# GRAPH-0/JODO

Hardware: AMD Instinct MI355X
Metric: molecules/sec (1000-step ancestral) (higher is better)
Workload: dtype f32

## Files before the change

### include/jodo_hip.h

```cpp
#ifndef JODO_HIP_H
#define JODO_HIP_H
#include <stddef.h>
#include <stdint.h>
#ifdef __cplusplus
extern "C" {
#endif

#define JODO_OK 0
#define JODO_ERR_ARG (-1)
#define JODO_ERR_LAUNCH (-2)
#define JODO_ERR_UNSUPPORTED (-3)

typedef struct {
    int32_t nf;
    int32_t n_layers;
    int32_t n_heads;
    int32_t n_extra;
    int32_t mlp_ratio;
    int32_t in_node_dim;
    int32_t edge_ch;
    int32_t cond_ch;
    float spatial_cut_off;
    float edge_quan_th;
    int32_t layout;
} jodo_cfg;

enum jodo_wslot_global {
    JW_TIME_FREQ = 0, JW_TIME_W1, JW_TIME_B1, JW_TIME_W3, JW_TIME_B3,
    JW_COND_W0, JW_COND_B0, JW_COND_W2, JW_COND_B2, JW_COND_LIN_W, JW_COND_LIN_B,
    JW_MOD_W, JW_MOD_B,
    JW_NODE_EMB_W, JW_NODE_EMB_B, JW_EDGE_EMB_W, JW_EDGE_EMB_B, JW_GBF_TOP,
    JW_NH1_W, JW_NH1_B, JW_NH2_W, JW_NH2_B, JW_NH3_W, JW_NH3_B,
    JW_EH1_W, JW_EH1_B, JW_EH2_W, JW_EH2_B, JW_EH3_W, JW_EH3_B,
    JW_GLOBAL_COUNT
};
enum jodo_wslot_block {
    JB_WQ = 0, JB_BQ, JB_WK, JB_BK, JB_WV, JB_BV,
    JB_EE_W, JB_EE_B, JB_LE0_W, JB_LE1_W, JB_N2E_W, JB_N2E_B,
    JB_FF1_W, JB_FF1_B, JB_FF2_W, JB_FF2_B, JB_FF3_W, JB_FF3_B, JB_FF4_W, JB_FF4_B,
    JB_INE_W, JB_ROW_W, JB_COL_W, JB_IN_B, JB_C0_W, JB_C0_B, JB_C2_W, JB_CSCALE,
    JB_NRO_W, JB_NRO_B, JB_ERO_W, JB_ERO_B, JB_GBF,
    JB_ROWQ_W, JB_COLQ_W, JB_INQ_B, JB_LQ_W, JB_INEC_W, JB_QT_W,
    JB_BLOCK_COUNT
};

typedef struct {
    const char* name;
    const float* data;
    const int64_t* shape;
    int32_t ndim;
} jodo_tensor;
int jodo_dgt_packed_size(const jodo_cfg* cfg, const jodo_tensor* tensors, int n_tensors, size_t* n_floats, int* n_woff);
int jodo_dgt_pack_weights_host(const jodo_cfg* cfg, const jodo_tensor* tensors, int n_tensors, float* packed_host,
                               size_t cap_floats, int64_t* woff_out, int n_woff);
int jodo_dgt_pack_weights(const jodo_cfg* cfg, const jodo_tensor* tensors, int n_tensors, void* packed_dev,
                          size_t cap_floats, int64_t* woff_out, int n_woff, void* stream);

typedef struct jodo_plan jodo_plan;

int jodo_plan_create(const jodo_cfg* cfg, int B, int N, const int32_t* n_nodes_host, int max_chunk,
                     jodo_plan** out);
void jodo_plan_destroy(jodo_plan* plan);
size_t jodo_plan_desc_bytes(const jodo_plan* plan);
size_t jodo_plan_workspace_bytes(const jodo_plan* plan);
int64_t jodo_plan_mod_len(const jodo_plan* plan);
int jodo_plan_upload(jodo_plan* plan, void* desc_dev, void* stream);
int jodo_plan_stats(const jodo_plan* plan, int64_t* out6);

int jodo_dgt_forward(jodo_plan* plan, const void* desc_dev, const float* packed_w, const int64_t* woff,
                     int n_woff, const float* xh, const float* edge_x, const float* cond_x,
                     const float* cond_edge_x, const float* noise_level, const float* context,
                     float* out_xh, float* out_edge, int32_t* flags_dev, void* workspace, void* stream);

int jodo_plan_work(const jodo_plan* plan, int uniform_t, int symmetric, double* mfma_flops_per_class);

enum jodo_plan_option {
    JODO_OPT_FUSE_NEXT_QKV = 0,
    JODO_OPT_DIR_SPLIT = 1,
    JODO_OPT_NODE_POST_WAVES = 2,
    JODO_OPT_ATTN_VARIANT = 3,
    JODO_OPT_PIN_SYMMETRIC = 4,
    JODO_OPT_PIN_UNIFORM_T = 5,
    JODO_OPT_ROT_STATS = 6,
    JODO_OPT_NODE_MIX = 7,
    JODO_OPT_HEADS_MIX = 8,
    JODO_OPT_HALF_ROWS = 9,
    JODO_OPT_PRE_EMBED = 10,
    JODO_OPT_AB_PRE = 11,
    JODO_OPT_Z_SPLIT = 12,
    JODO_OPT_SPLIT_BF16 = 13,
    JODO_OPT_COUNT
};
int jodo_plan_set_option(jodo_plan* plan, int option, int value);

int jodo_debug_attn_schedule(const jodo_plan* plan, int64_t* out8);

int jodo_debug_fetch(jodo_plan* plan, const void* workspace, int what, float* dst_dev, int64_t* count,
                     void* stream);
int jodo_debug_set_max_blocks(jodo_plan* plan, int max_blocks);
int jodo_debug_set_force_directed(jodo_plan* plan, int on);
int jodo_debug_set_timing_buffer(jodo_plan* plan, void* dev16xu64);

enum jodo_prof_class {
    JODO_PROF_PROLOGUE = 0, JODO_PROF_NODE_PRE, JODO_PROF_EDGE_ATTN, JODO_PROF_RESERVED3, JODO_PROF_RESERVED4,
    JODO_PROF_NODE_POST, JODO_PROF_EDGE_UPDATE, JODO_PROF_EPILOGUE, JODO_PROF_COUNT
};
int jodo_profile_enable(jodo_plan* plan, int enable);
int jodo_profile_read(jodo_plan* plan, float* ms_sum, int32_t* launches);

int jodo_sampler_step(int B, int N, int node_feats, int edge_ch, const int32_t* n_nodes_dev, float c_x, float c_pred,
                      float sigma, const float* x, const float* edge_x, const float* pred, const float* edge_pred,
                      const float* eps_pos, const float* eps_feat, const float* eps_edge, float* x_next,
                      float* edge_next, float* x_mean, float* edge_mean, void* stream);
int jodo_sampler_step_tab(int B, int N, int node_feats, int edge_ch, const int32_t* n_nodes_dev, const float* coef_tab_dev,
                          const int32_t* step_dev, const float* x, const float* edge_x, const float* pred,
                          const float* edge_pred, const float* eps_pos, const float* eps_feat, const float* eps_edge,
                          float* x_next, float* edge_next, float* x_mean, float* edge_mean, void* stream);
int jodo_sampler_step_rng(int B, int N, int node_feats, int edge_ch, const int32_t* n_nodes_dev, float c_x, float c_pred,
                          float sigma, const float* coef_tab_dev, const int32_t* step_dev, uint64_t seed, uint32_t draw,
                          const float* x, const float* edge_x, const float* pred, const float* edge_pred, float* x_next,
                          float* edge_next, float* x_mean, float* edge_mean, void* stream);
int jodo_step_begin(int B, const float* coef_tab_dev, const int32_t* step_dev, float* noise_level_out, void* stream);
int jodo_step_end(int32_t* step_dev, void* stream);
int jodo_dpm_update(int B, int N, int node_feats, int edge_ch, const int32_t* n_nodes_dev, const float* coef8_host,
                    const float* coef_tab_dev, const int32_t* step_dev, int tab_stride, int tab_col, const float* x_pos,
                    const float* x_base, const float* edge_base, const float* P, const float* eP, const float* DA, const float* eDA,
                    const float* DB, const float* eDB, const float* PP, const float* eps_pos, float* x_out, float* edge_out,
                    void* stream);
int jodo_dpm_update_rng(int B, int N, int node_feats, int edge_ch, const int32_t* n_nodes_dev, const float* coef8_host,
                        const float* coef_tab_dev, const int32_t* step_dev, int tab_stride, int tab_col, uint64_t seed,
                        uint32_t draw, uint32_t draw_mul, const float* x_pos, const float* x_base, const float* edge_base,
                        const float* P, const float* eP, const float* DA, const float* eDA, const float* DB, const float* eDB,
                        const float* PP, float* x_out, float* edge_out, void* stream);
int jodo_step_begin_at(int B, const float* coef_tab_dev, const int32_t* step_dev, int tab_stride, int tab_col,
                       float* noise_level_out, void* stream);
int jodo_decode(int B, int N, int atom_types, int include_fc, int edge_ch, int compress_edge, int centered,
                float pos_norm, float atom_norm, float fc_norm, float edge_norm, const int32_t* n_nodes_dev,
                const float* xh, const float* edge_x, float* pos_out, uint8_t* atom_type_out, int8_t* fc_out,
                uint8_t* edge_type_out, void* stream);

typedef struct jodo_train jodo_train;
int jodo_train_create(const jodo_cfg* cfg, int B, int N, const int32_t* n_nodes_host, const jodo_tensor* params, int n_params,
                      jodo_train** out);
void jodo_train_destroy(jodo_train* t);
size_t jodo_train_desc_bytes(const jodo_train* t);
size_t jodo_train_workspace_bytes(const jodo_train* t);
int jodo_train_set_option(jodo_train* t, int option, int value);
int jodo_train_debug_locate(const jodo_train* t, int what, int layer, size_t* byte_offset, size_t* count);
int jodo_train_upload(jodo_train* t, void* desc_dev, void* stream);
const void* jodo_train_desc_host(const jodo_train* t);
int jodo_train_forward(jodo_train* t, const void* desc_dev, const float* const* params_dev, int n_params, const float* xh,
                       const float* edge_x, const float* cond_x, const float* cond_edge_x, const float* noise_level,
                       const float* context, float dropout_p, uint64_t seed, float* out_xh, float* out_edge, int32_t* flags_out,
                       void* workspace, void* stream);
int jodo_train_backward(jodo_train* t, const void* desc_dev, const float* const* params_dev, float* const* grads_dev, int n_params,
                        const float* noise_level, const float* d_out_xh, const float* d_out_edge, float dropout_p, uint64_t seed,
                        void* workspace, void* stream);
int jodo_train_gemm(int tA, int tB, int M, int N, int K, const float* A, int lda, const float* B, int ldb, float* C, int ldc,
                    const float* bias, int acc, float* ws, size_t ws_floats, void* stream);
int jodo_train_gemm_ex(int tA, int tB, int M, int N, int K, const float* A, int lda, const float* B, int ldb, float* C, int ldc,
                       const float* bias, int act, float* out2, float* dbias, float* ws, size_t ws_floats, void* stream);

int jodo_adam_step(int64_t n, float* p, const float* g, float* m, float* v, float* vmax, double lr, double beta1, double beta2, double eps,
                   double weight_decay, int64_t step, int decoupled, int amsgrad, void* stream);
int jodo_gradnorm_clip(const float* norm_dev, double* state_dev, double max_grad, float* coef_dev, float* allowed_dev, void* stream);
int jodo_kabsch_rotations(int B, const float* A_dev, float* R_dev, void* stream);

typedef struct {
    int32_t nf, n_layers, n_heads, n_extra, mlp_ratio, in_node_dim, edge_ch;
    float edge_quan_th;
} jodo_cfg2d;
enum jodo2d_wslot_global {
    J2_TIME_FREQ = 0, J2_TIME_W1, J2_TIME_B1, J2_TIME_W3, J2_TIME_B3, J2_MOD_W, J2_MOD_B,
    J2_NODE_EMB_W, J2_NODE_EMB_B, J2_EDGE_EMB_W, J2_EDGE_EMB_B,
    J2_NH1_W, J2_NH1_B, J2_NH2_W, J2_NH2_B, J2_NH3_W, J2_NH3_B,
    J2_EH1_W, J2_EH1_B, J2_EH2_W, J2_EH2_B, J2_EH3_W, J2_EH3_B,
    J2_GLOBAL_COUNT
};
enum jodo2d_wslot_block {
    J2B_QKV_W = 0, J2B_QKV_B, J2B_LE_W, J2B_N2E_W, J2B_N2E_B, J2B_FF1_W, J2B_FF1_B, J2B_FF2_W, J2B_FF2_B,
    J2B_FF3_W, J2B_FF3_B, J2B_FF4_W, J2B_FF4_B, J2B_NRO_W, J2B_NRO_B, J2B_ERO_W, J2B_ERO_B,
    J2B_BLOCK_COUNT
};
int jodo_dgt2d_check_cfg(const jodo_cfg2d* cfg);
int jodo_dgt2d_packed_size(const jodo_cfg2d* cfg, size_t* n_floats, int* n_woff);
int jodo_dgt2d_pack_weights_host(const jodo_cfg2d* cfg, const jodo_tensor* tensors, int n_tensors, float* packed_host,
                                 size_t cap_floats, int64_t* woff_out, int n_woff);
int jodo_dgt2d_layout(const jodo_cfg2d* cfg, int B, int N, const int32_t* n_nodes_host, int64_t* out8);
int jodo_dgt2d_fill_desc(const jodo_cfg2d* cfg, int B, int N, const int32_t* n_nodes_host, int32_t* desc_host, int64_t n_words);
int jodo_dgt2d_forward(const jodo_cfg2d* cfg, int B, int N, const int32_t* n_nodes_host, const void* desc_dev, const float* packed_w,
                       const int64_t* woff, int n_woff, const float* xh, const float* edge_x, const float* cond_x,
                       const float* cond_edge_x, const float* noise_level, float* out_xh, float* out_edge, int32_t* flags_dev,
                       void* workspace, int force_directed, int max_blocks, void* stream);
enum jodo2d_walk { JODO_2D_WALK_DIRECTED = 0, JODO_2D_WALK_PAIR = 1 };
int jodo_dgt2d_pair_layout(const jodo_cfg2d* cfg, int B, int N, const int32_t* n_nodes_host, int64_t* out8);
int jodo_dgt2d_pair_fill_desc(const jodo_cfg2d* cfg, int B, int N, const int32_t* n_nodes_host, int32_t* desc_host, int64_t n_words);
int jodo_dgt2d_forward_walk(const jodo_cfg2d* cfg, int B, int N, const int32_t* n_nodes_host, const void* desc_dev,
                            const void* pair_desc_dev, int walk, const float* packed_w, const int64_t* woff, int n_woff, const float* xh,
                            const float* edge_x, const float* cond_x, const float* cond_edge_x, const float* noise_level, float* out_xh,
                            float* out_edge, int32_t* flags_dev, void* workspace, int force_directed, int max_blocks, void* stream);
int jodo_sampler_step_2d(int B, int N, int node_feats, int edge_ch, const int32_t* n_nodes_dev, float cx, float cp, float sigma,
                         const float* x, const float* edge_x, const float* pred, const float* edge_pred, const float* eps_node,
                         const float* eps_edge, float* x_next, float* edge_next, float* x_mean, float* edge_mean, void* stream);
int jodo_sampler_step_2d_rng(int B, int N, int node_feats, int edge_ch, const int32_t* n_nodes_dev, float c_x, float c_pred, float sigma,
                             const float* coef_tab_dev, const int32_t* step_dev, uint64_t seed, uint32_t draw, const float* x,
                             const float* edge_x, const float* pred, const float* edge_pred, float* x_next, float* edge_next,
                             float* x_mean, float* edge_mean, void* stream);
int jodo_decode_2d(int B, int N, int atom_types, int include_fc, int edge_ch, int compress_edge, int centered, float atom_norm,
                   float fc_norm, float edge_norm, const int32_t* n_nodes_dev, const float* xh, const float* edge_x,
                   uint8_t* atom_type_out, int8_t* fc_out, uint8_t* edge_type_out, void* stream);

typedef struct jodo_train2d jodo_train2d;
int jodo_train2d_create(const jodo_cfg2d* cfg, int B, int N, const int32_t* n_nodes_host, const jodo_tensor* params, int n_params,
                        jodo_train2d** out);
void jodo_train2d_destroy(jodo_train2d* t);
size_t jodo_train2d_desc_bytes(const jodo_train2d* t);
size_t jodo_train2d_workspace_bytes(const jodo_train2d* t);
const void* jodo_train2d_desc_host(const jodo_train2d* t);
int jodo_train2d_upload(jodo_train2d* t, void* desc_dev, void* stream);
int jodo_train2d_set_option(jodo_train2d* t, int option, int value);
int jodo_train2d_debug_locate(const jodo_train2d* t, int what, int layer, size_t* byte_offset, size_t* count);
int jodo_train2d_forward(jodo_train2d* t, const void* desc_dev, const float* const* params_dev, int n_params, const float* xh,
                         const float* edge_x, const float* cond_x, const float* cond_edge_x, const float* noise_level,
                         const float* context, float dropout_p, uint64_t seed, float* out_xh, float* out_edge, int32_t* flags_out,
                         void* workspace, void* stream);
int jodo_train2d_backward(jodo_train2d* t, const void* desc_dev, const float* const* params_dev, float* const* grads_dev, int n_params,
                          const float* noise_level, const float* d_out_xh, const float* d_out_edge, float dropout_p, uint64_t seed,
                          void* workspace, void* stream);

const char* jodo_last_error(void);

int jodo_debug_mfma_peak(int iters, int chains, int waves_per_simd, float* sink_dev, float* tflops_out);

int jodo_debug_mfma_valu(int iters, int nv, int nt, int waves_per_simd, float* sink_dev, float* tflops_out);

int jodo_dgt_split_size(const jodo_cfg* cfg, size_t* total_bytes, size_t* pair_block_bytes, size_t* node_block_bytes, size_t* attn_block_bytes);
int jodo_dgt_pack_split_host(const jodo_cfg* cfg, const jodo_tensor* tensors, int n_tensors, void* host, size_t cap_bytes);
int jodo_plan_set_split_weights(jodo_plan* plan, const void* tape_dev, size_t bytes);
int jodo_dgt_split_cond_size(const jodo_cfg* cfg, size_t* total_bytes, size_t* pair_block_bytes);
int jodo_dgt_pack_split_cond_host(const jodo_cfg* cfg, const jodo_tensor* tensors, int n_tensors, void* host, size_t cap_bytes);

int jodo_debug_mfma_bf16_valu(int iters, int nv, int chains, int waves_per_simd, float* sink_dev, float* tflops_out);
int jodo_debug_pack_split(const float* W, int n_out, int n_in, float* f32_packed_host, void* split_packed_host);
int jodo_debug_chain(int mode, int K, int tiles, const float* x, int rows, const float* wf, const void* wsp, float* y, int iters,
                     float* ms_out, void* stream);

// ... 8 lines not shown
```

### jodo_amd/csrc/dgt_forward.hip

```cpp
#include "dgt_kernels_pre.h"
#include "dgt_kernels_node.h"
#include "dgt_kernels_split_node.h"
#include "dgt_kernels_post.h"
#include "dgt_kernels_wide.h"
#include "jodo_hip_internal.h"
#include "dgt_launch.h"
#include <memory>
#include <utility>

using namespace jd;

namespace {

PlanDev make_plan_dev(const jodo_plan* p, const void* desc_dev) {
    const int* base = static_cast<const int*>(desc_dev);
    PlanDev d;
    d.node_b = base + p->off_node_b; d.node_i = base + p->off_node_i; d.node_n = base + p->off_node_n;
    d.node_noff = base + p->off_node_noff; d.node_eoff = base + p->off_node_eoff;
    d.orig_n = base + p->off_orig_n; d.orig_noff = base + p->off_orig_noff; d.orig_eoff = base + p->off_orig_eoff;
    d.item_strip = base + p->off_item_strip; d.item_t0 = base + p->off_item_t0; d.item_t1 = base + p->off_item_t1;
    d.item_part = base + p->off_item_part; d.strip_parts = base + p->off_strip_parts;
    d.pitem_strip = base + p->off_pitem_strip; d.pitem_t0 = base + p->off_pitem_t0; d.pitem_t1 = base + p->off_pitem_t1;
    d.n_pitems = p->n_pitems;
    d.ag_node = base + p->off_ag_node; d.ai_group = base + p->off_ai_group; d.ai_t0 = base + p->off_ai_t0; d.ai_t1 = base + p->off_ai_t1;
    d.ai_part = base + p->off_ai_part; d.ai_dir = base + p->off_ai_dir; d.ad_group = base + p->off_ad_group; d.ad_t0 = base + p->off_ad_t0; d.ad_t1 = base + p->off_ad_t1;
    d.ad_part = base + p->off_ad_part; d.ad_big = base + p->off_ad_big; d.anode_parts = base + p->off_anode_parts;
    d.aw_off = base + p->off_aw_off; d.a_persist = p->a_persist;
    d.n_agroups = p->n_agroups; d.n_aitems = p->n_aitems; d.n_aditems = p->n_aditems; d.amax_parts = p->amax_parts;
    d.Nn = p->Nn; d.Nn_pad = p->Nn_pad; d.n_strips = p->n_strips; d.n_items = p->n_items; d.B = p->B; d.N = p->N;
    d.max_parts = p->max_parts; d.rows = p->rows;
    d.ut_rows = base + p->off_ut_rows; d.n_ut_pad = p->n_ut_pad;
    d.gt_sa = base + p->off_gt_sa; d.gt_sc = base + p->off_gt_sc; d.n_gtiles = p->n_gtiles;
    return d;
}

template <typename T>
T* ws_ptr(void* ws, size_t off) { return reinterpret_cast<T*>(static_cast<char*>(ws) + off); }

void fill_ws(KArgs& A, const jodo_plan* p, void* ws) {
    const WsLayout& w = p->ws;
    A.hid1 = ws_ptr<float>(ws, w.hid1); A.temb = ws_ptr<float>(ws, w.temb); A.mods = ws_ptr<float>(ws, w.mods);
    A.condh = ws_ptr<float>(ws, w.condh); A.condh2 = ws_ptr<float>(ws, w.condh2);
    A.dpos = ws_ptr<float>(ws, w.dpos); A.cpos = ws_ptr<float>(ws, w.cpos); A.feat = ws_ptr<float>(ws, w.feat);
    A.h = ws_ptr<float>(ws, w.h); A.hhat = ws_ptr<float>(ws, w.hhat); A.astat = ws_ptr<float>(ws, w.astat); A.q = ws_ptr<float>(ws, w.q);
    A.k = ws_ptr<float>(ws, w.k); A.v = ws_ptr<float>(ws, w.v); A.n2e = ws_ptr<float>(ws, w.n2e);
    A.wrow = ws_ptr<float>(ws, w.wrow); A.wcol = ws_ptr<float>(ws, w.wcol); A.ua = ws_ptr<float>(ws, w.ua); A.ub = ws_ptr<float>(ws, w.ub);
    A.rmean = ws_ptr<float>(ws, w.rmean); A.mfold = ws_ptr<float>(ws, w.mfold); A.ffold = ws_ptr<float>(ws, w.ffold); A.ahid = ws_ptr<float>(ws, w.ahid);
    A.apred = ws_ptr<float>(ws, w.apred);
    A.eflag = ws_ptr<int>(ws, w.eflag); A.e = ws_ptr<float>(ws, w.e);
    A.ehid = ws_ptr<float>(ws, w.ehid); A.epred = ws_ptr<float>(ws, w.epred);
    A.e_out = ws_ptr<float>(ws, w.e2);
    A.dposE = ws_ptr<float>(ws, w.dposE); A.gramE = ws_ptr<float>(ws, w.gramE);
    A.wsplit = nullptr; A.wsplit_node = nullptr; A.wsplit_attn = nullptr; A.mfold_s = nullptr; A.ffold_s = nullptr; A.split_cond = 0;
}

int rowgemm(hipStream_t st, const float* X, int64_t ldx, float* Y, int64_t ldy, const float* Wp, const float* bias,
            int rows, int K, int NB, int in_act, int accumulate, const int* uniform_flag, float* Ysilu = nullptr) {
    if (K % 64 != 0) return jodo_set_error(JODO_ERR_ARG, "rowgemm: K=%d not a multiple of 64", K);
    const int nob = (rows <= 64 || uniform_flag) ? 1 : 4;
    const int gx = uniform_flag ? 1 : 0;
    RowGemmArgs G{X, ldx, Y, ldy, Wp, bias, rows, K, NB, in_act, accumulate, uniform_flag, nob, gx, Ysilu};
    dim3 grid((rows + 31) / 32, (NB + nob - 1) / nob);
    if (gx) grid = dim3(grid.y, grid.x);
    hipLaunchKernelGGL(k_rowgemm, grid, dim3(64), 0, st, G);
    return jodo_check_launch("k_rowgemm");
}

struct ProfScope {
    jodo_plan* p; hipStream_t st; int cls; bool on;
    static hipEvent_t get(jodo_plan* p) {
        if (!p->prof_pool.empty()) { hipEvent_t e = (hipEvent_t)p->prof_pool.back(); p->prof_pool.pop_back(); return e; }
        hipEvent_t e; (void)hipEventCreate(&e); return e;
    }
    ProfScope(jodo_plan* p_, hipStream_t st_, int cls_)
        : p(p_), st(st_), cls(cls_), on(p_->prof_enabled == 1 || (p_->prof_enabled == 2 && cls_ == JODO_PROF_EDGE_UPDATE) || p_->prof_enabled == 16 + cls_) {
        if (on) { hipEvent_t e = get(p); (void)hipEventRecord(e, st); p->prof_ev.push_back(e); }
    }
    ~ProfScope() {
        if (on) { hipEvent_t e = get(p); (void)hipEventRecord(e, st); p->prof_ev.push_back(e); p->prof_cls.push_back(cls); }
    }
};

template <int D, int KQ>
int launch_embed_nodes(hipStream_t st, const KArgs& A) {
    LAUNCH((wide::k_embed_nodes<D, KQ>), A.pd.n_strips, 64, A);
    return JODO_OK;
}
template <int D, int NBK>
int launch_edge_head(hipStream_t st, const KArgs& A, bool merged) {
    if (merged) {
        LAUNCH((wide::k_heads_sym<D, NBK>), (unsigned)(A.pd.n_strips + A.pd.n_ut_pad / 32), 64, A);
        return JODO_OK;
    }
    LAUNCH((wide::k_node_head<D>), A.pd.n_strips, 64, A);
    if (A.pd.n_ut_pad > 0 && A.pin_sym != 2) LAUNCH((wide::k_edge_head<D, NBK, true>), (unsigned)(A.pd.n_ut_pad / 32), 64, A);
    if (A.pin_sym != 1) LAUNCH((wide::k_edge_head<D, NBK, false>), (unsigned)((A.pd.rows + 31) / 32), 64, A);
    return JODO_OK;
}

__global__ __launch_bounds__(64, 1) void k_pre_embed(KArgs A) {
    const int npre = A.pd.n_strips * 3;
    if ((int)blockIdx.x < npre) node_pre_body<false>(A, (int)blockIdx.x);
    else wide::embed_edges_body<256>(A, (int)blockIdx.x - npre);
}


__global__ __launch_bounds__(64, 1) void k_node_ab_pre(KArgs A) {
    const int npre = A.mix_nw, nab = A.ab1 - A.ab0;
    const int b = (int)blockIdx.x;
    if (b < npre) node_pre_body<true>(A, b);
    else if (b < npre + nab) wide::node_ab_body<256>(A, A.ab0 + b - npre);
    else wide::node_gram_body<256>(A, A.g0 + b - npre - nab);
}

template <int D>
__global__ __launch_bounds__(64, 1) void k_node_ab_pre_w(KArgs A) {
    const int npre = A.mix_nw, nab = A.ab1 - A.ab0;
    const int b = (int)blockIdx.x;
    if (b < npre) wide::node_pre_body<D, true>(A, b);
    else if (b < npre + nab) wide::node_ab_body<D>(A, A.ab0 + b - npre);
    else wide::node_gram_body<D>(A, A.g0 + b - npre - nab);
}
template <int D>
__global__ __launch_bounds__(64, 1) void k_pre_embed_w(KArgs A) {
    const int npre = A.pd.n_strips * 3;
    if ((int)blockIdx.x < npre) wide::node_pre_body<D, false>(A, (int)blockIdx.x);
    else wide::embed_edges_body<D>(A, (int)blockIdx.x - npre);
}

template <int R, int NW>
__global__ __launch_bounds__(NW * 64, 1) void k_node_mix(KArgs A) {
    __shared__ float4 part[NW * 8 * 4 * 64];
    const int wg = blockIdx.x, wave = threadIdx.x >> 6;
    if (wg < A.mix_nw) { node_postw_body<R, NW>(A, wg + A.strip0, part); return; }
    const int nab = (A.ab1 - A.ab0 + NW - 1) / NW;
    if (wg < A.mix_nw + nab) {
        const int it = A.ab0 + (wg - A.mix_nw) * NW + wave;
        if (it < A.ab1) wide::node_ab_body<256>(A, it);
        return;
    }
    const int t = A.g0 + (wg - A.mix_nw - nab) * NW + wave;
    if (t < A.g1) wide::node_gram_body<256>(A, t);
}

int launch_node_post_256(jodo_plan* p, hipStream_t st, KArgs& A, bool with_ab, bool next_pre) {
    const DgtDims& d = p->dims;
    const int force = p->opt[JODO_OPT_NODE_POST_WAVES];
    const bool rem_only = force >= 10;
    const int full = (force && !rem_only) ? (force == 1 ? p->n_strips : 0) : (p->n_strips / 1024) * 1024;
    const int rem = p->n_strips - full;
    const int nw = rem_only ? force - 10 : (force ? force : (rem <= 256 ? 4 : (rem <= 512 ? 2 : 1)));
    const bool split_node = A.wsplit_node != nullptr && A.rot == 1;
    if (split_node) {
        A.strip0 = 0;
        const int wgs = (p->n_strips + 3) / 4;
        if (d.r == 2) { LAUNCH((split::k_node_post_split<2, 1>), wgs, split::SPLIT_WAVES * 64, A); LAUNCH((split::k_node_post_split<2, 2>), wgs, split::SPLIT_WAVES * 64, A); }
        else { LAUNCH((split::k_node_post_split<4, 1>), wgs, split::SPLIT_WAVES * 64, A); LAUNCH((split::k_node_post_split<4, 2>), wgs, split::SPLIT_WAVES * 64, A); }
    }
    const bool split_ab = split_node && with_ab && A.ffold_s != nullptr && !next_pre;
    if (split_ab) {
        A.ab0 = 0; A.ab1 = 2 * p->n_strips;
        LAUNCH(split::k_node_ab_split, (2 * p->n_strips + split::SPLIT_WAVES - 1) / split::SPLIT_WAVES, split::SPLIT_WAVES * 64, A);
    }
    if (full > 0 && !split_node) {
        A.strip0 = 0;
        if (d.r == 2) LAUNCH(k_node_post<2>, full, 64, A); else LAUNCH(k_node_post<4>, full, 64, A);
    }
    A.ab0 = 0; A.ab1 = 2 * p->n_strips; A.g0 = 0; A.g1 = A.rot ? p->n_gtiles : 0; A.mix_nw = 0;
    const bool mix = !split_node && with_ab && full > 0 && rem > 0 && nw >= 2 && p->opt[JODO_OPT_NODE_MIX] != 0;
    if (mix) {
        if (p->gt_cache_full != full) {
            const int32_t* sa = p->desc.data() + p->off_gt_sa, *sc = p->desc.data() + p->off_gt_sc;
            int c = 0;
            while (c < p->n_gtiles && sa[c] < full && sc[c] < full) ++c;
            p->gt_cache_full = full; p->gt_cache_count = c;
        }
        const int gpre = A.rot ? p->gt_cache_count : 0;
        A.strip0 = full; A.mix_nw = rem; A.ab0 = 0; A.ab1 = 2 * full; A.g0 = 0; A.g1 = gpre;
        const int g1 = rem + (A.ab1 - A.ab0 + nw - 1) / nw + (A.g1 - A.g0 + nw - 1) / nw;
        if (nw == 2) { if (d.r == 2) LAUNCH((k_node_mix<2, 2>), g1, 128, A); else LAUNCH((k_node_mix<4, 2>), g1, 128, A); }
        else { if (d.r == 2) LAUNCH((k_node_mix<2, 4>), g1, 256, A); else LAUNCH((k_node_mix<4, 4>), g1, 256, A); }
        A.strip0 = 0; A.mix_nw = 0; A.ab0 = 2 * full; A.ab1 = 2 * p->n_strips; A.g0 = gpre; A.g1 = A.rot ? p->n_gtiles : 0;
        const int g2 = (A.ab1 - A.ab0 + 1) / 2 + (A.g1 - A.g0 + 1) / 2;
        if (d.r == 2) LAUNCH((k_node_mix<2, 2>), g2, 128, A); else LAUNCH((k_node_mix<4, 2>), g2, 128, A);
        A.ab0 = 0; A.g0 = 0;
        return JODO_OK;
    }
    if (rem > 0 && !split_node) {
        A.strip0 = full;
        if (nw == 1) { if (d.r == 2) LAUNCH(k_node_post<2>, rem, 64, A); else LAUNCH(k_node_post<4>, rem, 64, A); }
        else if (nw == 2) { if (d.r == 2) LAUNCH((k_node_postw<2, 2>), rem, 128, A); else LAUNCH((k_node_postw<4, 2>), rem, 128, A); }
        else { if (d.r == 2) LAUNCH((k_node_postw<2, 4>), rem, 256, A); else LAUNCH((k_node_postw<4, 4>), rem, 256, A); }
    }
    A.strip0 = 0;
    if (next_pre) {
        A.mix_nw = 3 * p->n_strips;
        if (!with_ab) { A.ab1 = A.ab0; A.g1 = A.g0; }
        LAUNCH(k_node_ab_pre, A.mix_nw + (A.ab1 - A.ab0) + (A.g1 - A.g0), 64, A);
        A.mix_nw = 0;
        return JODO_OK;
    }
    if (with_ab) {
        if (!split_ab) LAUNCH((wide::k_node_ab<256>), p->n_strips * 2, 64, A);
        if (A.rot && p->n_gtiles > 0) LAUNCH((wide::k_node_gram<256>), p->n_gtiles, 64, A);
    }
    return JODO_OK;
}

template <int D, bool TUNED>
int forward_blocks(jodo_plan* p, hipStream_t st, KArgs& A, const int64_t* woff, float* const posbuf[2], std::unique_ptr<ProfScope>& pro) {
    const DgtDims& d = p->dims;
    int rc = JODO_OK;
    LAUNCH(k_pack_nodes, (p->Nn_pad + 255) / 256, 256, A);
    switch (d.ndp / 8) {
        case 1: rc = launch_embed_nodes<D, 1>(st, A); break;
        case 2: rc = launch_embed_nodes<D, 2>(st, A); break;
        case 3: rc = launch_embed_nodes<D, 3>(st, A); break;
        case 4: rc = launch_embed_nodes<D, 4>(st, A); break;
        case 5: rc = launch_embed_nodes<D, 5>(st, A); break;
        case 6: rc = launch_embed_nodes<D, 6>(st, A); break;
        case 7: rc = launch_embed_nodes<D, 7>(st, A); break;
        case 8: rc = launch_embed_nodes<D, 8>(st, A); break;
        default: return jodo_set_error(JODO_ERR_UNSUPPORTED, "node input width %d", d.ndp);
    }
    if (rc) return rc;
    const bool embed_merged = p->n_items > 0 && p->opt[JODO_OPT_PRE_EMBED] != 0 && ((p->max_blocks >= 0 && p->max_blocks < d.L) ? p->max_blocks : d.L) > 0;
    if (p->n_items > 0 && !embed_merged) LAUNCH((wide::k_embed_edges<D>), p->n_items, 64, A);
    const bool pin_pair = p->opt[JODO_OPT_PIN_SYMMETRIC] == 1 && !p->force_directed, pin_dir = p->opt[JODO_OPT_PIN_SYMMETRIC] == 2 || p->force_directed;
    const bool can_fold = p->n_pitems > 0 && !pin_dir && p->opt[JODO_OPT_PIN_UNIFORM_T] != 2 && d.cond_ch == 0;
    A.rot = can_fold ? p->opt[JODO_OPT_ROT_STATS] : 0;
    if (can_fold) {
        if (d.L > 16) return jodo_set_error(JODO_ERR_UNSUPPORTED, "more than 16 blocks");
        FoldOffs F;
        for (int l = 0; l < 16; ++l) {
            F.c0[l] = l < d.L ? woff[JW_GLOBAL_COUNT + l * JB_BLOCK_COUNT + JB_C0_W] : 0;
            F.ine[l] = l < d.L ? woff[JW_GLOBAL_COUNT + l * JB_BLOCK_COUNT + (A.rot ? JB_INEC_W : JB_INE_W)] : 0;
        }
        LAUNCH((wide::k_fold_coord<D, D / 16>), d.L * (D / 32) * (d.De / 4), 64, A, F, A.mfold, 0, A.mfold_s);
        if (A.rot) {
            for (int l = 0; l < d.L; ++l) F.ine[l] = woff[JW_GLOBAL_COUNT + l * JB_BLOCK_COUNT + JB_QT_W];
            LAUNCH((wide::k_fold_coord<D, D / 8>), d.L * (D / 32) * (D / 8), 64, A, F, A.ffold, 1, A.ffold_s);
        }
    }
    pro.reset();
    const int nblocks = (p->max_blocks >= 0 && p->max_blocks < d.L) ? p->max_blocks : d.L;
    const bool fuse_pre = TUNED && p->opt[JODO_OPT_FUSE_NEXT_QKV] != 0 && nblocks > 1 && p->n_strips >= 1024;
    const bool ab_pre = !fuse_pre && p->opt[JODO_OPT_AB_PRE] != 0 && nblocks > 1 && (!TUNED || (p->n_strips < 1024 && p->opt[JODO_OPT_NODE_POST_WAVES] == 0));
    int cur = 0;
    for (int l = 0; l < nblocks; ++l) {
        A.layer = l;
        A.mod_base = 32 + (int64_t)l * d.MB;
        for (int i = 0; i < JB_BLOCK_COUNT; ++i) A.wb[i] = woff[JW_GLOBAL_COUNT + l * JB_BLOCK_COUNT + i];
        A.wsplit = nullptr; A.wsplit_node = nullptr; A.wsplit_attn = nullptr;
        if (A.mfold_s) {
            size_t total = 0, pair_block = 0, node_block = 0, attn_block = 0;
            (void)jodo_dgt_split_size(&p->cfg, &total, &pair_block, &node_block, &attn_block);
            const char* base = static_cast<const char*>(p->split_w);
            A.wsplit = reinterpret_cast<const unsigned short*>(base + (size_t)l * pair_block);
            if (node_block > 0) A.wsplit_node = reinterpret_cast<const unsigned short*>(base + (size_t)d.L * pair_block + (size_t)l * node_block);
            if (attn_block > 0 && p->opt[JODO_OPT_SPLIT_BF16] == 2) A.wsplit_attn = reinterpret_cast<const unsigned short*>(base + (size_t)d.L * (pair_block + node_block) + (size_t)l * attn_block);
        } else if (A.split_cond) {
            size_t total = 0, pair_block = 0;
            (void)jodo_dgt_split_cond_size(&p->cfg, &total, &pair_block);
            A.wsplit = reinterpret_cast<const unsigned short*>(static_cast<const char*>(p->split_w) + (size_t)l * pair_block);
        }
        A.pos_in = posbuf[cur]; A.pos_out = posbuf[cur ^ 1];
        {
            ProfScope ps(p, st, JODO_PROF_NODE_PRE);
            if constexpr (TUNED) {
                if (!fuse_pre && !ab_pre) {
                    A.pre_mode = 0;
                    if (l == 0 && embed_merged) LAUNCH(k_pre_embed, p->n_strips * 3 + p->n_items, 64, A);
                    else LAUNCH(k_node_pre, p->n_strips * 3, 64, A);
                } else {
                    LAUNCH(k_pos_final, (p->Nn_pad + 255) / 256, 256, A);
                    if (l == 0) {
                        A.pre_mode = 1;
                        if (embed_merged) LAUNCH(k_pre_embed, p->n_strips * 3 + p->n_items, 64, A);
                        else LAUNCH(k_node_pre, p->n_strips * 3, 64, A);
                    }
                }
            } else if (!ab_pre) {
                A.pre_mode = 0;
                if (l == 0 && embed_merged) LAUNCH((k_pre_embed_w<D>), p->n_strips * 3 + p->n_items, 64, A);
                else LAUNCH((wide::k_node_pre<D>), p->n_strips * 3, 64, A);
            } else {
                LAUNCH(k_pos_final, (p->Nn_pad + 255) / 256, 256, A);
                if (l == 0) {
                    A.pre_mode = 1;
                    if (embed_merged) LAUNCH((k_pre_embed_w<D>), p->n_strips * 3 + p->n_items, 64, A);
                    else LAUNCH((wide::k_node_pre<D>), p->n_strips * 3, 64, A);
                }
            }
        }
        cur ^= 1;
        {
            ProfScope ps(p, st, JODO_PROF_EDGE_ATTN);
            rc = jd_launch_edge_attn(p, st, A, D, TUNED, pin_pair, pin_dir);
            if (rc) return rc;
        }
        {
            ProfScope ps(p, st, JODO_PROF_NODE_POST);
            if constexpr (TUNED) {
                A.fuse_next = (fuse_pre && l + 1 < nblocks) ? 1 : 0;
                const bool next_pre = ab_pre && l + 1 < nblocks;
                if (A.fuse_next || next_pre) {
                    static const int slots[6] = {JB_WQ, JB_BQ, JB_WK, JB_BK, JB_WV, JB_BV};
                    for (int i = 0; i < 6; ++i) A.wbn[i] = woff[JW_GLOBAL_COUNT + (l + 1) * JB_BLOCK_COUNT + slots[i]];
                    A.mod_base_next = 32 + (int64_t)(l + 1) * d.MB;
                }
                rc = launch_node_post_256(p, st, A, p->n_pitems > 0 && !pin_dir, next_pre);
                if (rc) return rc;
            } else {
                if (d.r == 2) LAUNCH((wide::k_node_post<D, 2>), p->n_strips, 64, A); else LAUNCH((wide::k_node_post<D, 4>), p->n_strips, 64, A);
                A.ab0 = 0; A.g0 = 0;
                const bool with_ab = p->n_pitems > 0 && !pin_dir;
                if (ab_pre && l + 1 < nblocks) {
                    static const int slots[6] = {JB_WQ, JB_BQ, JB_WK, JB_BK, JB_WV, JB_BV};
                    for (int i = 0; i < 6; ++i) A.wbn[i] = woff[JW_GLOBAL_COUNT + (l + 1) * JB_BLOCK_COUNT + slots[i]];
                    A.mod_base_next = 32 + (int64_t)(l + 1) * d.MB;
                    A.mix_nw = 3 * p->n_strips;
                    A.ab1 = with_ab ? 2 * p->n_strips : 0;
                    A.g1 = (with_ab && A.rot) ? p->n_gtiles : 0;
                    LAUNCH((k_node_ab_pre_w<D>), A.mix_nw + A.ab1 + A.g1, 64, A);
                    A.mix_nw = 0;
                } else {
                    if (with_ab) LAUNCH((wide::k_node_ab<D>), p->n_strips * 2, 64, A);
                    if (A.rot && p->n_gtiles > 0) LAUNCH((wide::k_node_gram<D>), p->n_gtiles, 64, A);
                }
            }
        }
        if (p->n_items > 0) {
            ProfScope ps(p, st, JODO_PROF_EDGE_UPDATE);
            rc = jd_launch_edge_update(p, st, A, D, pin_pair, pin_dir);
            if (rc) return rc;
            std::swap(A.e, A.e_out);
            p->last_e_buf ^= 1;
        }
    }
    ProfScope epi(p, st, JODO_PROF_EPILOGUE);
    A.pos_in = posbuf[cur]; A.pos_out = posbuf[cur ^ 1];
    A.layer = nblocks;
    LAUNCH(k_pos_final, (p->Nn_pad + 255) / 256, 256, A);
    p->last_pos_buf = cur ^ 1;
    const bool heads_mix = A.pin_sym == 1 && A.pd.n_ut_pad > 0 && p->opt[JODO_OPT_HEADS_MIX] != 0;
    switch (d.KEH / 32) {
        case 3: rc = launch_edge_head<D, 3>(st, A, heads_mix); break;
        case 4: rc = launch_edge_head<D, 4>(st, A, heads_mix); break;
        case 5: rc = launch_edge_head<D, 5>(st, A, heads_mix); break;
        case 6: rc = launch_edge_head<D, 6>(st, A, heads_mix); break;
        case 7: rc = launch_edge_head<D, 7>(st, A, heads_mix); break;
        case 8: rc = launch_edge_head<D, 8>(st, A, heads_mix); break;
        case 9: rc = launch_edge_head<D, 9>(st, A, heads_mix); break;
        case 10: rc = launch_edge_head<D, 10>(st, A, heads_mix); break;
        case 11: rc = launch_edge_head<D, 11>(st, A, heads_mix); break;
        case 12: rc = launch_edge_head<D, 12>(st, A, heads_mix); break;
        case 13: rc = launch_edge_head<D, 13>(st, A, heads_mix); break;
        case 15: rc = launch_edge_head<D, 15>(st, A, heads_mix); break;
        default: return jodo_set_error(JODO_ERR_UNSUPPORTED, "edge head width %d", d.KEH);
    }
    if (rc) return rc;
    LAUNCH(k_finalize_nodes, (p->B * p->N + 255) / 256, 256, A);
    {
        const size_t tot = (size_t)p->B * p->N * p->N;
        LAUNCH(k_finalize_edges, (unsigned)((tot + 255) / 256), 256, A);
    }
    return JODO_OK;
}

}

extern "C" int jodo_dgt_forward(jodo_plan* p, const void* desc_dev, const float* packed_w, const int64_t* woff,
                                int n_woff, const float* xh, const float* edge_x, const float* cond_x,
                                const float* cond_edge_x, const float* noise_level, const float* context,
                                float* out_xh, float* out_edge, int32_t* flags_dev, void* workspace, void* stream) {
    if (!p || !desc_dev || !packed_w || !woff || !xh || !edge_x || !noise_level || !out_xh || !out_edge || !flags_dev ||
        !workspace)
        return jodo_set_error(JODO_ERR_ARG, "dgt_forward: null argument");
    const DgtDims& d = p->dims;
    if (n_woff != JW_GLOBAL_COUNT + d.L * JB_BLOCK_COUNT)
        return jodo_set_error(JODO_ERR_ARG, "dgt_forward: weight table has %d slots, expected %d", n_woff,
                              JW_GLOBAL_COUNT + d.L * JB_BLOCK_COUNT);
    if ((cond_x == nullptr) != (cond_edge_x == nullptr))
        return jodo_set_error(JODO_ERR_ARG, "dgt_forward: cond_x and cond_edge_x must both be given or both NULL");
    if (d.cond_ch > 0 && !context) return jodo_set_error(JODO_ERR_ARG, "dgt_forward: conditional model needs context");
    hipStream_t st = (hipStream_t)stream;

    KArgs A;
    A.pd = make_plan_dev(p, desc_dev);
    A.d = d;
    A.W = packed_w;
    for (int i = 0; i < JW_GLOBAL_COUNT; ++i) A.wg[i] = woff[i];
    for (int i = 0; i < JB_BLOCK_COUNT; ++i) A.wb[i] = 0;
    A.mod_base = 0; A.layer = 0; A.force_directed = p->force_directed; A.pin_sym = p->force_directed ? 0 : p->opt[JODO_OPT_PIN_SYMMETRIC];
    A.half_rows = (A.pin_sym == 1 && p->n_pitems > 0 && p->opt[JODO_OPT_HALF_ROWS] != 0) ? 1 : 0;
    A.pin_uni = p->opt[JODO_OPT_PIN_UNIFORM_T]; A.pre_mode = 0; A.strip0 = 0; A.item0 = 0; A.dir_split = 0; A.rot = 0; A.mix_nw = 0; A.ab0 = 0; A.ab1 = 0; A.g0 = 0; A.g1 = 0; A.fuse_next = 0; A.mod_base_next = 0;
    for (int i = 0; i < 6; ++i) A.wbn[i] = 0;
    fill_ws(A, p, workspace);
    if (p->opt[JODO_OPT_SPLIT_BF16] >= 1 && p->split_w && (d.D == 256 || d.D == 384) && d.cond_ch == 0 && !p->force_directed && p->n_pitems > 0 && p->pitems_single &&
        p->opt[JODO_OPT_PIN_SYMMETRIC] == 1 && p->opt[JODO_OPT_PIN_UNIFORM_T] == 1 && p->opt[JODO_OPT_ROT_STATS] == 1) {
        size_t total = 0, per_block = 0, node_block = 0, attn_block = 0;
        if (jodo_dgt_split_size(&p->cfg, &total, &per_block, &node_block, &attn_block) == JODO_OK && total == p->split_bytes)
            A.mfold_s = ws_ptr<unsigned short>(workspace, p->ws.mfold_s);
        if (A.mfold_s && node_block > 0) A.ffold_s = ws_ptr<unsigned short>(workspace, p->ws.ffold_s);
    }
    if (p->opt[JODO_OPT_SPLIT_BF16] >= 1 && p->split_w && d.D == 256 && d.cond_ch > 0 && !p->force_directed && p->n_pitems > 0 && p->pitems_single &&
        p->opt[JODO_OPT_PIN_SYMMETRIC] == 1 && p->opt[JODO_OPT_PIN_UNIFORM_T] == 2) {
        size_t total = 0, per_block = 0;
        if (jodo_dgt_split_cond_size(&p->cfg, &total, &per_block) == JODO_OK && total == p->split_bytes) A.split_cond = 1;
    }
    float* posbuf[2] = {ws_ptr<float>(workspace, p->ws.pos0), ws_ptr<float>(workspace, p->ws.pos1)};
    A.pos_in = posbuf[0]; A.pos_out = posbuf[1];
    A.flags = flags_dev;
    A.dbgt = static_cast<unsigned long long*>(p->dbg_timing);
    A.xh = xh; A.edge_x = edge_x; A.cond_x = cond_x; A.cond_edge_x = cond_edge_x; A.noise = noise_level; A.context = context;
    A.out_xh = out_xh; A.out_edge = out_edge;
    const float* W = packed_w;
    int rc;

    p->last_e_buf = 0;
    std::unique_ptr<ProfScope> pro(new ProfScope(p, st, JODO_PROF_PROLOGUE));
    LAUNCH(k_flags_init, 1, 256, A);
    { const size_t tot = (size_t)p->B * p->N * p->N; LAUNCH(k_check_sym, (unsigned)((tot + 255) / 256), 256, A); }
    LAUNCH(k_time1, p->B, 256, A);
    const int* uflag = d.cond_ch > 0 ? nullptr : flags_dev + FLAG_UNIFORM_T;
    float* tembs = ws_ptr<float>(workspace, p->ws.tembs);
    rc = rowgemm(st, A.hid1, d.T, A.temb, d.T, W + A.wg[JW_TIME_W3], W + A.wg[JW_TIME_B3], p->B, d.T, d.T / 32, 0, 0, uflag,
                 d.cond_ch > 0 ? nullptr : tembs);
    if (rc) return rc;
    if (d.cond_ch > 0) {
        LAUNCH(k_cond1, p->B * d.cond_ch, 256, A);
        rc = rowgemm(st, A.condh, d.D, A.condh2, d.D, W + A.wg[JW_COND_W2], W + A.wg[JW_COND_B2], p->B * d.cond_ch, d.D,
                     d.D / 32, 0, 0, nullptr);
        if (rc) return rc;
        rc = rowgemm(st, A.condh2, (int64_t)d.cond_ch * d.D, A.temb, d.T, W + A.wg[JW_COND_LIN_W], W + A.wg[JW_COND_LIN_B],
                     p->B, d.cond_ch * d.D, d.T / 32, 0, 1, nullptr, tembs);
        if (rc) return rc;
    }
    rc = rowgemm(st, tembs, d.T, A.mods, d.Mtot, W + A.wg[JW_MOD_W], W + A.wg[JW_MOD_B], p->B, d.T, (int)(d.Mtot / 32), 0, 0,
                 uflag);
    if (rc) return rc;
    if (!d.wide) return forward_blocks<256, true>(p, st, A, woff, posbuf, pro);
    if (d.D == 128) return forward_blocks<128, false>(p, st, A, woff, posbuf, pro);
    return d.D == 256 ? forward_blocks<256, false>(p, st, A, woff, posbuf, pro) : forward_blocks<384, false>(p, st, A, woff, posbuf, pro);
}

extern "C" int jodo_debug_fetch(jodo_plan* p, const void* workspace, int what, float* dst, int64_t* count, void* stream) {
    if (!p || !workspace || !dst || !count) return jodo_set_error(JODO_ERR_ARG, "debug_fetch: null");
    const char* ws = static_cast<const char*>(workspace);
    const void* src = nullptr;
    int64_t n = 0;
    switch (what) {
        case 0: src = ws + p->ws.h; n = (int64_t)p->Nn * p->dims.D; break;
        case 1: src = ws + (p->last_e_buf ? p->ws.e2 : p->ws.e); n = p->rows * p->dims.De; break;
        case 2: src = ws + (p->last_pos_buf ? p->ws.pos1 : p->ws.pos0); n = (int64_t)p->Nn * 4; break;
        case 3: src = ws + p->ws.hhat; n = (int64_t)p->Nn * p->amax_parts * p->dims.D; break;
        case 5: src = ws + p->ws.mods; n = p->dims.Mtot; break;
        case 6: src = ws + p->ws.q; n = (int64_t)p->Nn * p->dims.QKP; break;
        default: return jodo_set_error(JODO_ERR_ARG, "debug_fetch: unknown selector %d", what);
    }
    hipError_t e = hipMemcpyAsync(dst, src, (size_t)n * sizeof(float), hipMemcpyDeviceToDevice, (hipStream_t)stream);
    if (e != hipSuccess) return jodo_set_error(JODO_ERR_LAUNCH, "debug_fetch: %s", hipGetErrorString(e));
    *count = n;
    return JODO_OK;
}
```

### jodo_amd/csrc/dgt_kernels_common.h

```cpp
#pragma once
#include "dgt_device.h"
#include "dgt_plan.h"

enum { FLAG_NAN = 0, FLAG_FIRST = 1, FLAG_UNIFORM_T = 2, FLAG_COND_NONZERO = 3, FLAG_ASYM = 4, FLAG_NAN_COUNT = 5, FLAG_PIN_VIOLATED = 6 };

struct KArgs {
    PlanDev pd;
    DgtDims d;
    const float* W;
    int64_t wg[JW_GLOBAL_COUNT];
    int64_t wb[JB_BLOCK_COUNT];
    int64_t mod_base;
    int layer;
    int force_directed;
    int pin_sym, pin_uni;
    int strip0;
    int half_rows;
    int item0, dir_split;
    int mix_nw, ab0, ab1, g0, g1;
    int rot;
    int fuse_next;
    int64_t wbn[6];
    int64_t mod_base_next;
    int pre_mode;
    float *hid1, *temb, *mods, *condh, *condh2;
    float *pos_in, *pos_out, *dpos, *cpos, *feat, *h, *hhat, *astat, *q, *k, *v, *n2e, *wrow, *wcol, *ua, *ub, *rmean, *mfold, *ffold, *ahid, *apred;
    int* eflag;
    float *e, *ehid, *epred, *dposE, *gramE;
    float* e_out;
    const unsigned short* wsplit;
    const unsigned short* wsplit_attn;
    const unsigned short* wsplit_node;
    unsigned short* mfold_s;
    unsigned short* ffold_s;
    int split_cond;
    int* flags;
    unsigned long long* dbgt;
    const float *xh, *edge_x, *cond_x, *cond_edge_x, *noise, *context;
    float *out_xh, *out_edge;
};

struct FoldOffs { int64_t c0[16], ine[16]; };

namespace jd {

constexpr int PAIR_GROUP_LANES = 128;

__device__ __forceinline__ bool rot_active(const KArgs& A) { return A.rot && A.flags[FLAG_UNIFORM_T] && !A.flags[FLAG_ASYM]; }
}

namespace jd {

__device__ __forceinline__ const float4* wq(const KArgs& A, int64_t off, int lane) {
    return reinterpret_cast<const float4*>(A.W + off) + lane;
}

__device__ __forceinline__ const float* mod_row(const KArgs& A, int node_b) {
    const int trow = A.flags[FLAG_UNIFORM_T] ? 0 : node_b;
    return A.mods + (size_t)trow * A.d.Mtot;
}

struct LaneNode {
    int v, b, i, n, noff, eoff;
    bool valid;
};

__device__ __forceinline__ LaneNode lane_node(const KArgs& A, int strip, int j) {
    LaneNode L;
    L.v = strip * 32 + j;
    L.b = A.pd.node_b[L.v];
    L.i = A.pd.node_i[L.v];
    L.n = A.pd.node_n[L.v];
    L.noff = A.pd.node_noff[L.v];
    L.eoff = A.pd.node_eoff[L.v];
    L.valid = L.n > 0;
    return L;
}

__device__ __forceinline__ float4 advance_position(const KArgs& A, float4 p, int v, int strip, int n, int i, int eoff) {
    double sx = 0., sy = 0., sz = 0.;
    if (A.flags[FLAG_ASYM]) {
        const int parts = A.pd.strip_parts[strip];
        for (int q = 0; q < parts; ++q) {
            const float4 dp = reinterpret_cast<const float4*>(A.dpos)[(size_t)v * A.pd.max_parts + q];
            sx += dp.x; sy += dp.y; sz += dp.z;
        }
    } else {
        const float4* row = reinterpret_cast<const float4*>(A.dposE) + (size_t)eoff + (size_t)i * n;
        int c = 0;
        for (; c + 8 <= n; c += 8) {
            float4 d[8];
#pragma unroll
            for (int u = 0; u < 8; ++u) d[u] = row[c + u];
#pragma unroll
            for (int u = 0; u < 8; ++u)
                if (c + u != i) { sx += d[u].x; sy += d[u].y; sz += d[u].z; }
        }
        for (; c + 4 <= n; c += 4) {
            const float4 d0 = row[c], d1 = row[c + 1], d2 = row[c + 2], d3 = row[c + 3];
            if (c != i) { sx += d0.x; sy += d0.y; sz += d0.z; }
            if (c + 1 != i) { sx += d1.x; sy += d1.y; sz += d1.z; }
            if (c + 2 != i) { sx += d2.x; sy += d2.y; sz += d2.z; }
            if (c + 3 != i) { sx += d3.x; sy += d3.y; sz += d3.z; }
        }
        for (; c < n; ++c) {
            if (c == i) continue;
            const float4 dp = row[c];
            sx += dp.x; sy += dp.y; sz += dp.z;
        }
    }
    p.x += (float)sx; p.y += (float)sy; p.z += (float)sz;
    return p;
}

__device__ __forceinline__ float gelu_erf(float x) { return 0.5f * x * (1.f + erff(x * 0.70710678118654752f)); }

}
```

### jodo_amd/csrc/dgt_kernels_node.h

```cpp
#pragma once
#include "dgt_kernels_attn.h"

namespace jd {

template <bool NEXT = false>
__device__ __forceinline__ void node_pre_body(const KArgs& A, int blk) {
    const int lane = threadIdx.x & 63, j = lane & 31, half = lane >> 5;
    const int strip = blk / 3, piece = blk % 3;
    const LaneNode L = lane_node(A, strip, j);
    if (!NEXT && piece == 0 && A.pre_mode == 0) {
        float4 p = reinterpret_cast<const float4*>(A.pos_in)[L.v];
        if (A.layer > 0) p = advance_position(A, p, L.v, strip, L.n, L.i, L.eoff);
        if (half == 0) reinterpret_cast<float4*>(A.pos_out)[L.v] = p;
    }
    const float* mr = mod_row(A, L.b) + (NEXT ? A.mod_base_next : A.mod_base);
    float hx[128];
    load_nat<8>(A.h + (size_t)L.v * 256, half, hx);
    layer_norm<128>(hx);
    modulate<8>(hx, mr, mr + 256, half);
    const WSrc ws = make_wsrc(A.W, lane);
    const unsigned woff = (unsigned)((NEXT ? A.wbn[2 * piece] : A.wb[piece == 0 ? JB_WQ : (piece == 1 ? JB_WK : JB_WV)]) * 4);
    const float* bias = A.W + (NEXT ? A.wbn[2 * piece + 1] : A.wb[piece == 0 ? JB_BQ : (piece == 1 ? JB_BK : JB_BV)]);
    float* outp = piece == 0 ? A.q : (piece == 1 ? A.k : A.v);
    WPipe<8> wp;
    wpipe_prime(wp, ws, woff);
#pragma unroll 1
    for (int b = 0; b < 8; ++b) {
        const unsigned cur = woff + (unsigned)b * 32 * 1024;
        const unsigned nxt = b < 7 ? cur + 32 * 1024 : woff;
        float bb[16], r[16];
        load16(bias + b * 32 + half * 16, bb);
        f32x16 acc = mfma_block_p<32>(wp, ws, cur, nxt, hx, zero16());
#pragma unroll
        for (int s = 0; s < 16; ++s) r[s] = acc[s] + bb[s];
        store16T(outp, 8, L.v, half, b, r);
    }
}
__global__ __launch_bounds__(64, 1) void k_node_pre(KArgs A) { node_pre_body<false>(A, (int)blockIdx.x); }
__device__ __forceinline__ void node_load_hh(const KArgs& A, const LaneNode& L, int half, float (&hh)[128]) {
    attn_merge<256>(A, L.v, half, hh);
}

__device__ __forceinline__ void node_residual_ln(const KArgs& A, const LaneNode& L, int half, const float* mr, float (&x)[128]) {
    const float* ng1 = mr + 2 * 256, *ns2 = mr + 3 * 256, *nc2 = mr + 4 * 256;
    const float* hrow = A.h + (size_t)L.v * 256;
#pragma unroll
    for (int b = 0; b < 8; ++b) {
        float g[16], h0[16];
        load16(ng1 + b * 32 + half * 16, g);
        load16(hrow + b * 32 + half * 16, h0);
#pragma unroll
        for (int s = 0; s < 16; ++s) x[b * 16 + s] = fmaf(g[s], x[b * 16 + s], h0[s]);
    }
    layer_norm<128>(x);
    modulate<8>(x, ns2, nc2, half);
}

__device__ __forceinline__ void node_next_ln(const KArgs& A, const LaneNode& L, int half, float (&x)[128]) {
    const float* mr = mod_row(A, L.b) + A.mod_base_next;
    layer_norm<128>(x);
    modulate<8>(x, mr, mr + 256, half);
}
__device__ __forceinline__ void node_next_qkv(const KArgs& A, const LaneNode& L, int half, const float (&x)[128], const WSrc& ws,
                                              WPipe<8>& wp, int g0, int g1) {
#pragma unroll 1
    for (int g = g0; g < g1; ++g) {
        const int piece = g >> 3, b = g & 7;
        const unsigned cur = (unsigned)(A.wbn[2 * piece] * 4) + (unsigned)b * 32 * 1024;
        const int gn = g + 1 < g1 ? g + 1 : g0;
        const unsigned nxt = (unsigned)(A.wbn[2 * (gn >> 3)] * 4) + (unsigned)(gn & 7) * 32 * 1024;
        const float* bias = A.W + A.wbn[2 * piece + 1];
        float* outp = piece == 0 ? A.q : (piece == 1 ? A.k : A.v);
        float bb[16], r[16];
        load16(bias + b * 32 + half * 16, bb);
        f32x16 acc = mfma_block_p<32>(wp, ws, cur, nxt, x, zero16());
#pragma unroll
        for (int s = 0; s < 16; ++s) r[s] = acc[s] + bb[s];
        store16T(outp, 8, L.v, half, b, r);
    }
}

template <int R>
__global__ __launch_bounds__(64, 1) void k_node_post(KArgs A) {
    const int lane = threadIdx.x & 63, j = lane & 31, half = lane >> 5;
    const int strip = blockIdx.x + A.strip0;
    const LaneNode L = lane_node(A, strip, j);
    const float* mr = mod_row(A, L.b) + A.mod_base;
    const float* ng2 = mr + 5 * 256;
    const WSrc ws = make_wsrc(A.W, lane);
    const unsigned oN2E = (unsigned)(A.wb[JB_N2E_W] * 4), oF1 = (unsigned)(A.wb[JB_FF1_W] * 4), oF2 = (unsigned)(A.wb[JB_FF2_W] * 4);
    const bool rot = rot_active(A);
    const unsigned oRow = (unsigned)(A.wb[rot ? JB_ROWQ_W : JB_ROW_W] * 4), oCol = (unsigned)(A.wb[rot ? JB_COLQ_W : JB_COL_W] * 4), oNro = (unsigned)(A.wb[JB_NRO_W] * 4);
    WPipe<8> wp;
    wpipe_prime(wp, ws, oN2E);
    float hx[128];
    node_load_hh(A, L, half, hx);
#pragma unroll
    for (int b = 0; b < 2; ++b) {
        const unsigned cur = oN2E + (unsigned)b * 32 * 1024;
        f32x16 acc = mfma_block_p<32>(wp, ws, cur, b == 0 ? cur + 32 * 1024 : oF1, hx, zero16());
        float r[16];
#pragma unroll
        for (int s = 0; s < 16; ++s) r[s] = acc[s];
        store16T(A.n2e, 2, L.v, half, b, r);
    }
    node_residual_ln(A, L, half, mr, hx);
    f32x16 o[8];
#pragma unroll
    for (int b = 0; b < 8; ++b) o[b] = zero16();
    {
        const float* b1 = A.W + A.wb[JB_FF1_B];
        constexpr int KQ2 = R * 256 / 8;
#pragma unroll 1
        for (int c = 0; c < R * 4; ++c) {
            float hid[32];
#pragma unroll
            for (int b2 = 0; b2 < 2; ++b2) {
                const unsigned cur = oF1 + (unsigned)(c * 2 + b2) * 32 * 1024;
                const unsigned nxt = b2 == 0 ? cur + 32 * 1024 : oF2 + (unsigned)(c * 8) * 1024;
                float bb[16];
                load16(b1 + (c * 2 + b2) * 32 + half * 16, bb);
                f32x16 acc = mfma_block_p<32>(wp, ws, cur, nxt, hx, zero16());
                silu_bias16(acc, bb, hid + b2 * 16);
            }
#pragma unroll
            for (int ob = 0; ob < 8; ++ob) {
                const unsigned cur = oF2 + (unsigned)(ob * KQ2 + c * 8) * 1024;
                const unsigned nxt = ob < 7 ? oF2 + (unsigned)((ob + 1) * KQ2 + c * 8) * 1024
                                            : (c + 1 < R * 4 ? oF1 + (unsigned)((c + 1) * 2) * 32 * 1024 : oRow);
                o[ob] = mfma_block_p<8>(wp, ws, cur, nxt, hid, o[ob]);
            }
        }
    }
    {
        const float* b2 = A.W + A.wb[JB_FF2_B];
#pragma unroll
        for (int b = 0; b < 8; ++b) {
            float bb[16], g[16];
            load16(b2 + b * 32 + half * 16, bb);
            load16(ng2 + b * 32 + half * 16, g);
#pragma unroll
            for (int s = 0; s < 16; ++s) hx[b * 16 + s] = fmaf(g[s], o[b][s] + bb[s], hx[b * 16 + s]);
        }
    }
    store_nat<8>(A.h + (size_t)L.v * 256, half, hx);
    {
        const float* bin = A.W + A.wb[rot ? JB_INQ_B : JB_IN_B];
#pragma unroll 1
        for (int b = 0; b < 8; ++b) {
            const unsigned cr = oRow + (unsigned)b * 32 * 1024, cc = oCol + (unsigned)b * 32 * 1024;
            float bb[16], r[16];
            load16(bin + b * 32 + half * 16, bb);
            f32x16 acc = mfma_block_p<32>(wp, ws, cr, cc, hx, zero16());
#pragma unroll
            for (int s = 0; s < 16; ++s) r[s] = acc[s] + bb[s];
            store16T(A.wrow, 8, L.v, half, b, r);
            acc = mfma_block_p<32>(wp, ws, cc, b < 7 ? cr + 32 * 1024 : oNro, hx, zero16());
#pragma unroll
            for (int s = 0; s < 16; ++s) r[s] = acc[s];
            store16T(A.wcol, 8, L.v, half, b, r);
        }
    }
    {
        const float* bias = A.W + A.wb[JB_NRO_B];
#pragma unroll
        for (int b = 0; b < 2; ++b) {
            const unsigned cur = oNro + (unsigned)b * 32 * 1024;
            float bb[16], r[16];
            load16(bias + b * 32 + half * 16, bb);
            f32x16 acc = mfma_block_p<32>(wp, ws, cur, b == 0 ? cur + 32 * 1024 : (A.fuse_next ? (unsigned)(A.wbn[0] * 4) : oNro), hx, zero16());
// ... 162 lines not shown
```

### jodo_amd/csrc/dgt_kernels_post.h

```cpp
#pragma once
#include "dgt_kernels_common.h"

namespace jd {

__global__ void k_pos_final(KArgs A) {
    const int v = blockIdx.x * blockDim.x + threadIdx.x;
    if (v >= A.pd.Nn_pad) return;
    float4 p = reinterpret_cast<const float4*>(A.pos_in)[v];
    if (v < A.pd.Nn) {
        if (A.layer > 0)
            p = advance_position(A, p, v, v >> 5, A.pd.node_n[v], A.pd.node_i[v], A.pd.node_eoff[v]);
        if (isnan(p.x) || isnan(p.y) || isnan(p.z)) atomicOr(&A.flags[FLAG_NAN], 1);
    }
    reinterpret_cast<float4*>(A.pos_out)[v] = p;
}

__global__ void k_finalize_nodes(KArgs A) {
    const int idx = blockIdx.x * blockDim.x + threadIdx.x;
    if (idx >= A.pd.B * A.pd.N) return;
    if (idx == 0 && A.flags[FLAG_NAN] != 0) A.flags[FLAG_NAN_COUNT] += 1;
    if (idx == 0) {
        int bad = 0;
        if (A.pin_sym == 1 && A.flags[FLAG_ASYM]) bad |= 1;
        if ((A.pin_uni == 1 && !A.flags[FLAG_UNIFORM_T]) || (A.pin_uni == 2 && A.flags[FLAG_UNIFORM_T])) bad |= 2;
        if (bad) A.flags[FLAG_PIN_VIOLATED] |= bad;
    }
    const int b = idx / A.pd.N, i = idx % A.pd.N;
    const int n = A.pd.orig_n[b], nd = A.d.nd;
    float* o = A.out_xh + (size_t)idx * (3 + nd);
    if (i >= n) {
        for (int f = 0; f < 3 + nd; ++f) o[f] = 0.f;
        return;
    }
    const int v0 = A.pd.orig_noff[b];
    const bool nan = A.flags[FLAG_NAN] != 0;
    double mx = 0., my = 0., mz = 0.;
    for (int k = 0; k < n; ++k) {
        const float4 p = reinterpret_cast<const float4*>(A.pos_out)[v0 + k];
        mx += p.x; my += p.y; mz += p.z;
    }
    const float4 p = reinterpret_cast<const float4*>(A.pos_out)[v0 + i];
    const double inv = 1.0 / (double)n;
    o[0] = nan ? 0.f : p.x - (float)(mx * inv);
    o[1] = nan ? 0.f : p.y - (float)(my * inv);
    o[2] = nan ? 0.f : p.z - (float)(mz * inv);
    const float* ap = A.apred + (size_t)(v0 + i) * 32;
    for (int f = 0; f < nd; ++f) o[3 + f] = ap[f];
}

__global__ void k_finalize_edges(KArgs A) {
    const size_t idx = (size_t)blockIdx.x * blockDim.x + threadIdx.x;
    const size_t NN = (size_t)A.pd.N * A.pd.N;
    if (idx >= (size_t)A.pd.B * NN) return;
    const int b = (int)(idx / NN);
    const int a = (int)((idx % NN) / A.pd.N), c = (int)(idx % A.pd.N);
    const int n = A.pd.orig_n[b], ch = A.d.ch;
    float* o = A.out_edge + idx * ch;
    if (a >= n || c >= n || a == c) {
        for (int f = 0; f < ch; ++f) o[f] = 0.f;
        return;
    }
    const size_t e0 = (size_t)A.pd.orig_eoff[b];
    const float4 p = reinterpret_cast<const float4*>(A.epred)[e0 + (size_t)a * n + c];
    const float4 q = reinterpret_cast<const float4*>(A.epred)[e0 + (size_t)c * n + a];
    const float pp[4] = {p.x, p.y, p.z, p.w}, qq[4] = {q.x, q.y, q.z, q.w};
    for (int f = 0; f < ch; ++f) o[f] = 0.5f * (pp[f] + qq[f]);
}

}
```

### jodo_amd/csrc/dgt_kernels_pre.h

```cpp
#pragma once
#include "dgt_kernels_common.h"

namespace jd {

__global__ void k_flags_init(KArgs A) {
    __shared__ int differs;
    if (threadIdx.x == 0) differs = 0;
    __syncthreads();
    const float x0 = A.noise[0];
    int d = 0;
    for (int b = threadIdx.x; b < A.pd.B; b += blockDim.x) d |= (A.noise[b] != x0);
    if (d) atomicOr(&differs, 1);
    __syncthreads();
    if (threadIdx.x == 0) {
        A.flags[FLAG_NAN] = 0;
        A.flags[FLAG_FIRST] = 0;
        A.flags[FLAG_COND_NONZERO] = 0;
        A.flags[FLAG_ASYM] = (A.force_directed || A.pin_sym == 2) ? 1 : 0;
        A.flags[FLAG_UNIFORM_T] = (A.d.cond_ch == 0 && !differs) ? 1 : 0;
    }
}

__global__ void k_check_sym(KArgs A) {
    const size_t idx = (size_t)blockIdx.x * blockDim.x + threadIdx.x;
    const size_t NN = (size_t)A.pd.N * A.pd.N;
    if (idx >= (size_t)A.pd.B * NN) return;
    const int b = (int)(idx / NN);
    const int a = (int)((idx % NN) / A.pd.N), c = (int)(idx % A.pd.N);
    const int n = A.pd.orig_n[b], ch = A.d.ch;
    if (a >= n || c >= n || a >= c) return;
    const size_t r1 = idx * ch, r2 = ((size_t)b * NN + (size_t)c * A.pd.N + a) * ch;
    bool diff = false;
    for (int f = 0; f < ch; ++f) {
        const float x1 = A.edge_x[r1 + f], x2 = A.edge_x[r2 + f];
        diff |= !(x1 == x2 || (x1 != x1 && x2 != x2));
        if (A.cond_edge_x) {
            const float c1 = A.cond_edge_x[r1 + f], c2 = A.cond_edge_x[r2 + f];
            diff |= !(c1 == c2 || (c1 != c1 && c2 != c2));
        }
    }
    if (diff) atomicOr(&A.flags[FLAG_ASYM], 1);
}

__global__ void k_time1(KArgs A) {
    const int b = blockIdx.x;
    if (A.flags[FLAG_UNIFORM_T] && b > 0) return;
    __shared__ float ft[17];
    const float x = A.noise[b];
    if (threadIdx.x < 8) {
        const float fr = x * A.W[A.wg[JW_TIME_FREQ] + threadIdx.x] * 2.f * 3.14159265358979323846f;
        ft[1 + threadIdx.x] = sinf(fr);
        ft[9 + threadIdx.x] = cosf(fr);
    }
    if (threadIdx.x == 0) ft[0] = x;
    __syncthreads();
    const float* W1 = A.W + A.wg[JW_TIME_W1];
    const float* b1 = A.W + A.wg[JW_TIME_B1];
    for (int f = threadIdx.x; f < A.d.T; f += blockDim.x) {
        float acc = b1[f];
#pragma unroll
        for (int k = 0; k < 17; ++k) acc = fmaf(W1[f * 17 + k], ft[k], acc);
        A.hid1[(size_t)b * A.d.T + f] = gelu_erf(acc);
    }
}

__global__ void k_cond1(KArgs A) {
    const int row = blockIdx.x;
    const float x = A.context[row];
    const float* w0 = A.W + A.wg[JW_COND_W0];
    const float* b0 = A.W + A.wg[JW_COND_B0];
    for (int f = threadIdx.x; f < A.d.D; f += blockDim.x)
        A.condh[(size_t)row * A.d.D + f] = gelu_erf(fmaf(w0[f], x, b0[f]));
}

struct RowGemmArgs {
    const float* X; int64_t ldx;
    float* Y; int64_t ldy;
    const float* Wp; const float* bias;
    int rows, K, NB;
    int in_act;
    int accumulate;
    const int* uniform_flag;
    int nob;
    int groups_in_x;
    float* Ysilu;
};

__global__ __launch_bounds__(64) __attribute__((amdgpu_waves_per_eu(2))) void k_rowgemm(RowGemmArgs G) {
    const int lane = threadIdx.x & 63, j = lane & 31, half = lane >> 5;
    const int rows = (G.uniform_flag && *G.uniform_flag) ? 1 : G.rows;
    const int r0 = (G.groups_in_x ? blockIdx.y : blockIdx.x) * 32;
    if (r0 >= rows) return;
    const int row = r0 + j;
    const int rowc = row < rows ? row : rows - 1;
    const int ob0 = (G.groups_in_x ? blockIdx.x : blockIdx.y) * G.nob;
    const int nv = G.NB - ob0 < G.nob ? G.NB - ob0 : G.nob;
    const int kq = G.K / 8, nch = G.K / 64;
    f32x16 acc[4];
#pragma unroll
    for (int o = 0; o < 4; ++o) acc[o] = zero16();
    const WSrc ws = make_wsrc(G.Wp, lane);
    auto woff = [&](int o, int c) { return (unsigned)(((size_t)(ob0 + o) * kq + (size_t)c * 8) * 1024); };
    WPipe<8> wp;
    wpipe_prime(wp, ws, woff(0, 0));
    const float* xrow = G.X + (size_t)rowc * G.ldx;
    float xn[32];
    load_nat<2>(xrow, half, xn);
    for (int c = 0; c < nch; ++c) {
        float x[32];
#pragma unroll
        for (int s = 0; s < 32; ++s) x[s] = xn[s];
        if (c + 1 < nch) load_nat<2>(xrow + (c + 1) * 64, half, xn);
        if (G.in_act == 1) {
#pragma unroll
            for (int s = 0; s < 32; ++s) x[s] = silu_f(x[s]);
        }
#pragma unroll
        for (int o = 0; o < 4; ++o) {
            if (o < nv) {
                const bool last_o = o + 1 >= nv;
                const unsigned nxt = !last_o ? woff(o + 1, c) : (c + 1 < nch ? woff(0, c + 1) : woff(0, 0));
                acc[o] = mfma_block_p<8>(wp, ws, woff(o, c), nxt, x, acc[o]);
            }
        }
    }
    if (row >= rows) return;
#pragma unroll
    for (int o = 0; o < 4; ++o) {
        if (o < nv) {
            float r[16];
            acc_bias(acc[o], G.bias + (ob0 + o) * 32 + half * 16, r);
            float* yp = G.Y + (size_t)row * G.ldy + (ob0 + o) * 32 + half * 16;
            if (G.accumulate) {
                float old[16];
                load16(yp, old);
#pragma unroll
                for (int s = 0; s < 16; ++s) r[s] += old[s];
            }
            store16(yp, r);
            if (G.Ysilu) {
#pragma unroll
                for (int s = 0; s < 16; ++s) r[s] = silu_f(r[s]);
                store16(G.Ysilu + (size_t)row * G.ldy + (ob0 + o) * 32 + half * 16, r);
            }
        }
    }
}

__global__ void k_pack_nodes(KArgs A) {
    const int v = blockIdx.x * blockDim.x + threadIdx.x;
    if (v >= A.pd.Nn_pad) return;
    const int nd = A.d.nd, ndp = A.d.ndp, dims = 3 + nd;
    float4 p = make_float4(0.f, 0.f, 0.f, 0.f), cp = p;
    float* ft = A.feat + (size_t)v * ndp;
    for (int f = 0; f < ndp; ++f) ft[f] = 0.f;
    if (v < A.pd.Nn) {
        const int b = A.pd.node_b[v], i = A.pd.node_i[v];
        const float* x = A.xh + ((size_t)b * A.pd.N + i) * dims;
        p = make_float4(x[0], x[1], x[2], 0.f);
        for (int f = 0; f < nd; ++f) ft[f] = x[3 + f];
        if (A.cond_x) {
            const float* c = A.cond_x + ((size_t)b * A.pd.N + i) * dims;
            cp = make_float4(c[0], c[1], c[2], 0.f);
            for (int f = 0; f < nd; ++f) ft[nd + f] = c[3 + f];
            const float* c0 = A.cond_x + ((size_t)b * A.pd.N) * dims;
            if (c[0] != c0[0] || c[1] != c0[1] || c[2] != c0[2]) atomicOr(&A.flags[FLAG_COND_NONZERO], 1);
        }
    }
    reinterpret_cast<float4*>(A.pos_in)[v] = p;
    reinterpret_cast<float4*>(A.cpos)[v] = cp;
}

}
```

### jodo_amd/csrc/dgt_kernels_wide.h

```cpp
#pragma once
#include "dgt_kernels_common.h"
#include "dgt_kernels_attn.h"

namespace jd {
namespace wide {

constexpr int NHEAD_BLOCKS = 14;

template <int D_>
struct Dim {
    static constexpr int D = D_, De = D_ / 4, ND = D_ / 32, NE = D_ / 128;
    static constexpr int HD = D_ / 2, HE = D_ / 8;
    static constexpr int KQD = D_ / 8, KQE = D_ / 32;
    static constexpr int PG = (D_ % 256 == 0) ? 8 : 4;
    static constexpr int C = D_ / 16;
    static constexpr float INV_SQRT_C = D_ == 256 ? 0.25f : (D_ == 384 ? 0.20412414523193150f : (D_ == 128 ? 0.35355339059327379f : 0.f));
    static constexpr int M_EDGE = 6 * D_, M_EQUI = 6 * D_ + 6 * (D_ / 4), M_GBF = 6 * D_ + 6 * (D_ / 4) + 2 * D_;
    static constexpr int M_WG = M_GBF + 32, M_BS = M_WG + D_;
};

template <int D, int KQ>
__global__ __launch_bounds__(64) void k_embed_nodes(KArgs A) {
    using X = Dim<D>;
    const int lane = threadIdx.x & 63, j = lane & 31, half = lane >> 5;
    const int v = blockIdx.x * 32 + j;
    float x[KQ * 4];
    const float4* src = reinterpret_cast<const float4*>(A.feat + (size_t)v * (KQ * 8) + half * (KQ * 4));
#pragma unroll
    for (int q = 0; q < KQ; ++q) {
        const float4 t = src[q];
        x[q * 4 + 0] = t.x; x[q * 4 + 1] = t.y; x[q * 4 + 2] = t.z; x[q * 4 + 3] = t.w;
    }
    const float4* w = wq(A, A.wg[JW_NODE_EMB_W], lane);
    const float* bias = A.W + A.wg[JW_NODE_EMB_B];
#pragma unroll
    for (int b = 0; b < X::ND; ++b) {
        f32x16 acc = mfma_block<KQ>(w + (size_t)b * KQ * 64, x, zero16());
        float r[16];
        acc_bias(acc, bias + b * 32 + half * 16, r);
        store16(A.h + (size_t)v * D + b * 32 + half * 16, r);
        store16(A.ahid + (size_t)v * A.d.KNH + b * 32 + half * 16, r);
    }
}

template <int D>
__device__ __forceinline__ void embed_edges_body(const KArgs& A, int it) {
    using X = Dim<D>;
    const int lane = threadIdx.x & 63, j = lane & 31, half = lane >> 5;
    const int strip = A.pd.item_strip[it], t0 = A.pd.item_t0[it], t1 = A.pd.item_t1[it];
    const LaneNode L = lane_node(A, strip, j);
    const int ch = A.d.ch;
    const bool first = A.flags[FLAG_COND_NONZERO] == 0;
    const float* mr = mod_row(A, L.b);
    const float gscale = mr[0], gshift = mr[1];
    const float4 pc = reinterpret_cast<const float4*>(A.cpos)[L.v];
    const float* tab = A.W + A.wg[JW_GBF_TOP];
    const float4* w = wq(A, A.wg[JW_EDGE_EMB_W], lane);
    const float* bias = A.W + A.wg[JW_EDGE_EMB_B];
    for (int t = t0; t < t1; ++t) {
        const bool ok = L.valid && t < L.n;
        const int tc = ok ? t : 0;
        const int u = L.noff + tc;
        const size_t r = (size_t)L.eoff + (size_t)L.i * L.n + tc;
        int dd = tc - L.i;
        if (dd < 0) dd += L.n;
        const bool wr = ok && (!A.half_rows || L.n > PAIR_GROUP_LANES || (dd != 0 && (2 * dd < L.n || (2 * dd == L.n && 2 * L.i < L.n))));
        const float4 pu = reinterpret_cast<const float4*>(A.cpos)[u];
        const float dx = pc.x - pu.x, dy = pc.y - pu.y, dz = pc.z - pu.z;
        const float d2c = dx * dx + dy * dy + dz * dz;
        const size_t din = (((size_t)L.b * A.pd.N + L.i) * A.pd.N + tc) * ch;
        float ein[4];
#pragma unroll
        for (int s = 0; s < 4; ++s) {
            const int f = half * 4 + s;
            float val = 0.f;
            if (f < ch) val = A.edge_x[din + f];
            else if (f < 2 * ch && A.cond_edge_x) val = A.cond_edge_x[din + (f - ch)];
            ein[s] = val;
        }
        int adj2d = 1;
        if (A.cond_edge_x) adj2d = A.cond_edge_x[din] >= A.d.edge_th ? 1 : 0;
        const int adjsp = d2c <= A.d.cutoff ? 1 : 0;
        float G[X::HE];
        if (first) {
#pragma unroll
            for (int s = 0; s < X::HE; ++s) G[s] = 0.f;
        } else {
            gbf_n<X::NE>(d2c, gscale, gshift, tab, half, G);
        }
#pragma unroll
        for (int b = 0; b < X::NE; ++b) {
            f32x16 acc = mfma_block<X::KQE>(w + (size_t)(b * (X::KQE + 1)) * 64, G, zero16());
            acc = mfma_block<1>(w + (size_t)(b * (X::KQE + 1) + X::KQE) * 64, ein, acc);
            float rr[16];
            acc_bias(acc, bias + b * 32 + half * 16, rr);
            if (wr) {
                store16(A.e + r * X::De + b * 32 + half * 16, rr);
                store16(A.ehid + r * A.d.KEH + b * 32 + half * 16, rr);
            }
        }
        if (ok && half == 0) A.eflag[r] = adj2d | (adjsp << 1);
    }
}
template <int D>
__global__ __launch_bounds__(64) void k_embed_edges(KArgs A) { embed_edges_body<D>(A, (int)blockIdx.x); }

template <int D, bool NEXT = false>
__device__ __forceinline__ void node_pre_body(const KArgs& A, int blk) {
    using X = Dim<D>;
    const int lane = threadIdx.x & 63, j = lane & 31, half = lane >> 5;
    const int strip = blk / 3, piece = blk % 3;
    const LaneNode L = lane_node(A, strip, j);
    if (!NEXT && piece == 0 && A.pre_mode == 0) {
        float4 p = reinterpret_cast<const float4*>(A.pos_in)[L.v];
        if (A.layer > 0) p = advance_position(A, p, L.v, strip, L.n, L.i, L.eoff);
        if (half == 0) reinterpret_cast<float4*>(A.pos_out)[L.v] = p;
    }
    const float* mr = mod_row(A, L.b) + (NEXT ? A.mod_base_next : A.mod_base);
    float hx[X::HD];
    load_nat<X::ND>(A.h + (size_t)L.v * D, half, hx);
    layer_norm<X::HD>(hx);
    modulate<X::ND>(hx, mr, mr + D, half);
    const WSrc ws = make_wsrc(A.W, lane);
    const unsigned woff = (unsigned)((NEXT ? A.wbn[2 * piece] : A.wb[piece == 0 ? JB_WQ : (piece == 1 ? JB_WK : JB_WV)]) * 4);
    const float* bias = A.W + (NEXT ? A.wbn[2 * piece + 1] : A.wb[piece == 0 ? JB_BQ : (piece == 1 ? JB_BK : JB_BV)]);
    float* outp = piece == 0 ? A.q : (piece == 1 ? A.k : A.v);
    const int nb = piece == 2 ? X::ND : NHEAD_BLOCKS;
    WPipe<X::PG> wp;
    wpipe_prime(wp, ws, woff);
#pragma unroll 1
    for (int b = 0; b < nb; ++b) {
        const unsigned cur = woff + (unsigned)b * X::KQD * 1024;
        const unsigned nxt = b + 1 < nb ? cur + X::KQD * 1024 : woff;
        float bb[16], r[16];
        load16(bias + b * 32 + half * 16, bb);
        f32x16 acc = mfma_block_p<X::KQD>(wp, ws, cur, nxt, hx, zero16());
#pragma unroll
        for (int s = 0; s < 16; ++s) r[s] = acc[s] + bb[s];
        store16T(outp, nb, L.v, half, b, r);
    }
}
template <int D>
__global__ __launch_bounds__(64, 1) void k_node_pre(KArgs A) { node_pre_body<D, false>(A, (int)blockIdx.x); }

template <int D, int R>
__global__ __launch_bounds__(64, 1) void k_node_post(KArgs A) {
    using X = Dim<D>;
    constexpr int NPASS = 1, NOB = X::ND / NPASS;
    constexpr int NCH = R * D / 64;
    constexpr int KQ2 = R * D / 8;
    const int lane = threadIdx.x & 63, j = lane & 31, half = lane >> 5;
    const int strip = blockIdx.x;
    const LaneNode L = lane_node(A, strip, j);
    const float* mr = mod_row(A, L.b) + A.mod_base;
    const float* ng1 = mr + 2 * D, *ns2 = mr + 3 * D, *nc2 = mr + 4 * D, *ng2 = mr + 5 * D;
    const WSrc ws = make_wsrc(A.W, lane);
    const unsigned oN2E = (unsigned)(A.wb[JB_N2E_W] * 4), oF1 = (unsigned)(A.wb[JB_FF1_W] * 4), oF2 = (unsigned)(A.wb[JB_FF2_W] * 4);
    const bool rot = rot_active(A);
    const unsigned oRow = (unsigned)(A.wb[rot ? JB_ROWQ_W : JB_ROW_W] * 4), oCol = (unsigned)(A.wb[rot ? JB_COLQ_W : JB_COL_W] * 4), oNro = (unsigned)(A.wb[JB_NRO_W] * 4);
    WPipe<X::PG> wp;
    wpipe_prime(wp, ws, oN2E);
    float hx[X::HD];
    attn_merge<D>(A, L.v, half, hx);
#pragma unroll
    for (int b = 0; b < X::NE; ++b) {
        const unsigned cur = oN2E + (unsigned)b * X::KQD * 1024;
        f32x16 acc = mfma_block_p<X::KQD>(wp, ws, cur, b + 1 < X::NE ? cur + X::KQD * 1024 : oF1, hx, zero16());
        float r[16];
#pragma unroll
        for (int s = 0; s < 16; ++s) r[s] = acc[s];
        store16T(A.n2e, X::NE, L.v, half, b, r);
    }
    {
        const float* hrow = A.h + (size_t)L.v * D;
#pragma unroll
        for (int b = 0; b < X::ND; ++b) {
            float g[16], h0[16];
            load16(ng1 + b * 32 + half * 16, g);
            load16(hrow + b * 32 + half * 16, h0);
#pragma unroll
            for (int s = 0; s < 16; ++s) hx[b * 16 + s] = fmaf(g[s], hx[b * 16 + s], h0[s]);
        }
        layer_norm<X::HD>(hx);
        modulate<X::ND>(hx, ns2, nc2, half);
    }
    {
        const float* b1 = A.W + A.wb[JB_FF1_B];
        const float* b2 = A.W + A.wb[JB_FF2_B];
        float* hrow = A.h + (size_t)L.v * D;
#pragma unroll
        for (int ps = 0; ps < NPASS; ++ps) {
            f32x16 o[NOB];
#pragma unroll
            for (int b = 0; b < NOB; ++b) o[b] = zero16();
#pragma unroll 1
// ... 12 lines not shown
                for (int ob = 0; ob < NOB; ++ob) {
                    const unsigned cur = oF2 + (unsigned)((ps * NOB + ob) * KQ2 + c * 8) * 1024;
                    const unsigned nxt = ob + 1 < NOB ? oF2 + (unsigned)((ps * NOB + ob + 1) * KQ2 + c * 8) * 1024
                                                      : (c + 1 < NCH ? oF1 + (unsigned)((c + 1) * 2) * X::KQD * 1024
                                                                     : (ps + 1 < NPASS ? oF1 : oRow));
                    o[ob] = mfma_block_p<8>(wp, ws, cur, nxt, hid, o[ob]);
                }
            }
#pragma unroll
            for (int ob = 0; ob < NOB; ++ob) {
                const int b = ps * NOB + ob;
                float bb[16], g[16], r[16];
                load16(b2 + b * 32 + half * 16, bb);
                load16(ng2 + b * 32 + half * 16, g);
#pragma unroll
                for (int s = 0; s < 16; ++s) r[s] = fmaf(g[s], o[ob][s] + bb[s], hx[b * 16 + s]);
                store16(hrow + b * 32 + half * 16, r);
            }
        }
        load_nat<X::ND>(hrow, half, hx);
    }
    {
        const float* bin = A.W + A.wb[rot ? JB_INQ_B : JB_IN_B];
#pragma unroll 1
        for (int b = 0; b < X::ND; ++b) {
            const unsigned cr = oRow + (unsigned)b * X::KQD * 1024, cc = oCol + (unsigned)b * X::KQD * 1024;
            float bb[16], r[16];
            load16(bin + b * 32 + half * 16, bb);
            f32x16 acc = mfma_block_p<X::KQD>(wp, ws, cr, cc, hx, zero16());
#pragma unroll
            for (int s = 0; s < 16; ++s) r[s] = acc[s] + bb[s];
            store16T(A.wrow, X::ND, L.v, half, b, r);
            acc = mfma_block_p<X::KQD>(wp, ws, cc, b + 1 < X::ND ? cr + X::KQD * 1024 : oNro, hx, zero16());
#pragma unroll
            for (int s = 0; s < 16; ++s) r[s] = acc[s];
            store16T(A.wcol, X::ND, L.v, half, b, r);
        }
    }
    {
        const float* bias = A.W + A.wb[JB_NRO_B];
        const int nro = A.d.cnp / 32;
#pragma unroll 1
        for (int b = 0; b < nro; ++b) {
            const unsigned cur = oNro + (unsigned)b * X::KQD * 1024;
            float bb[16], r[16];
            load16(bias + b * 32 + half * 16, bb);
            f32x16 acc = mfma_block_p<X::KQD>(wp, ws, cur, b + 1 < nro ? cur + X::KQD * 1024 : oNro, hx, zero16());
#pragma unroll
            for (int s = 0; s < 16; ++s) r[s] = acc[s] + bb[s];
            store16(A.ahid + (size_t)L.v * A.d.KNH + D + A.layer * A.d.cnp + b * 32 + half * 16, r);
        }
    }
}

template <int D>
__device__ __forceinline__ void node_ab_body(const KArgs& A, int item) {
    if (D != 256 && !A.flags[FLAG_UNIFORM_T]) return;
    using X = Dim<D>;
    const int lane = threadIdx.x & 63, j = lane & 31, half = lane >> 5;
    const int strip = item >> 1, piece = item & 1;
    const LaneNode L = lane_node(A, strip, j);
    const bool rot = rot_active(A);
    const float* qsc = mod_row(A, L.b) + A.mod_base + X::M_EQUI + D;
    const TRow src = trow(piece == 0 ? A.wrow : A.wcol, X::ND, L.v, half);
    float x[X::HD];
    float sum = 0.f;
    if (rot) {
#pragma unroll
        for (int b = 0; b < X::ND; ++b) {
            float t[16];
            load16T(src, b, t);
#pragma unroll
            for (int s = 0; s < 16; ++s) x[b * 16 + s] = t[s];
        }
    } else {
#pragma unroll
        for (int b = 0; b < X::ND; ++b) {
            float t[16], g[16];
            load16T(src, b, t);
            load16(qsc + b * 32 + half * 16, g);
#pragma unroll
            for (int s = 0; s < 16; ++s) { sum += t[s]; x[b * 16 + s] = t[s] * (1.f + g[s]); }
        }
    }
    if (!rot) {
        const float red = pair_sum(sum);
        if (half == 0) A.rmean[(size_t)L.v * 2 + piece] = red * (1.f / D);
    }
    const float* wbase = rot ? A.ffold + (size_t)A.layer * D * D : A.W;
    const WSrc ws = make_wsrc(wbase, lane);
    const unsigned o0 = rot ? 0u : (unsigned)(A.wb[JB_C0_W] * 4);
    WPipe<X::PG> wp;
    wpipe_prime(wp, ws, o0);
    float* dst = piece == 0 ? A.ua : A.ub;
#pragma unroll 1
    for (int b = 0; b < X::ND; ++b) {
        const unsigned cur = o0 + (unsigned)b * X::KQD * 1024;
        f32x16 acc = mfma_block_p<X::KQD>(wp, ws, cur, b + 1 < X::ND ? cur + X::KQD * 1024 : o0, x, zero16());
        float r[16];
#pragma unroll
        for (int s = 0; s < 16; ++s) r[s] = acc[s];
        store16T(dst, X::ND, L.v, half, b, r);
    }
}
template <int D>
__global__ __launch_bounds__(64, 1) void k_node_ab(KArgs A) { node_ab_body<D>(A, A.ab0 + (int)blockIdx.x); }

template <int D>
__device__ __forceinline__ void node_gram_body(const KArgs& A, int tile) {
    if (!rot_active(A)) return;
    using X = Dim<D>;
    const int lane = threadIdx.x & 63, j = lane & 31, half = lane >> 5;
    const int sa = A.pd.gt_sa[tile], sc = A.pd.gt_sc[tile];
    const float4* ra = reinterpret_cast<const float4*>(A.wrow) + (size_t)sa * X::ND * 256 + lane;
    const float4* cc = reinterpret_cast<const float4*>(A.wcol) + (size_t)sc * X::ND * 256 + lane;
    const int vc = sc * 32 + j, val = sa * 32 + j;
    const int nc = A.pd.node_n[vc], noffc = A.pd.node_noff[vc], ic = A.pd.node_i[vc];
    const bool centre = A.rot != 2;
    const int refa = (centre && A.pd.node_n[val] > 0) ? A.pd.node_noff[val] : val, refc = (centre && nc > 0) ? noffc : vc;
    const float4* ma = reinterpret_cast<const float4*>(A.wcol) + (size_t)(refa >> 5) * X::ND * 256 + (refa & 31) + 32 * half;
    const float4* mc = reinterpret_cast<const float4*>(A.wcol) + (size_t)(refc >> 5) * X::ND * 256 + (refc & 31) + 32 * half;
    const float sgn = centre ? 1.f : 0.f;
    f32x16 acc = zero16();
    float na[4] = {0.f, 0.f, 0.f, 0.f}, nc4[4] = {0.f, 0.f, 0.f, 0.f};
#pragma unroll
    for (int b = 2 * X::NE; b < X::ND; ++b)
#pragma unroll
        for (int q = 0; q < 4; ++q) {
            const float4 a0 = ra[(b * 4 + q) * 64], c0 = cc[(b * 4 + q) * 64], pa = ma[(b * 4 + q) * 64], pc = mc[(b * 4 + q) * 64];
            const float4 a = make_float4(fmaf(sgn, pa.x, a0.x), fmaf(sgn, pa.y, a0.y), fmaf(sgn, pa.z, a0.z), fmaf(sgn, pa.w, a0.w));
            const float4 c = make_float4(fmaf(-sgn, pc.x, c0.x), fmaf(-sgn, pc.y, c0.y), fmaf(-sgn, pc.z, c0.z), fmaf(-sgn, pc.w, c0.w));
            acc = __builtin_amdgcn_mfma_f32_32x32x2f32(a.x, c.x, acc, 0, 0, 0);
            acc = __builtin_amdgcn_mfma_f32_32x32x2f32(a.y, c.y, acc, 0, 0, 0);
            acc = __builtin_amdgcn_mfma_f32_32x32x2f32(a.z, c.z, acc, 0, 0, 0);
            acc = __builtin_amdgcn_mfma_f32_32x32x2f32(a.w, c.w, acc, 0, 0, 0);
            na[0] = fmaf(a.x, a.x, na[0]); na[1] = fmaf(a.y, a.y, na[1]); na[2] = fmaf(a.z, a.z, na[2]); na[3] = fmaf(a.w, a.w, na[3]);
            nc4[0] = fmaf(c.x, c.x, nc4[0]); nc4[1] = fmaf(c.y, c.y, nc4[1]); nc4[2] = fmaf(c.z, c.z, nc4[2]); nc4[3] = fmaf(c.w, c.w, nc4[3]);
        }
    const float nR = pair_sum((na[0] + na[1]) + (na[2] + na[3]));
    const float nC = pair_sum((nc4[0] + nc4[1]) + (nc4[2] + nc4[3]));
    const size_t eoffc = (size_t)A.pd.node_eoff[vc];
#pragma unroll
    for (int s = 0; s < 16; ++s) {
        const int m = 8 * (s >> 2) + 4 * half + (s & 3), va = sa * 32 + m;
        const float nRa = __shfl(nR, m);
        if (nc > 0 && A.pd.node_n[va] > 0 && A.pd.node_noff[va] == noffc)
            A.gramE[eoffc + (size_t)A.pd.node_i[va] * nc + ic] = nRa + nC + 2.f * acc[s];
    }
}
template <int D>
__global__ __launch_bounds__(64) void k_node_gram(KArgs A) { node_gram_body<D>(A, A.g0 + (int)blockIdx.x); }

template <int D, int KQI>
__global__ __launch_bounds__(64) void k_fold_coord(KArgs A, FoldOffs F, float* out, int need_rot, unsigned short* out_s = nullptr) {
    if (!A.flags[FLAG_UNIFORM_T] || (need_rot && !rot_active(A))) return;
    using X = Dim<D>;
    constexpr int PER_L = X::ND * KQI;
    const int l = blockIdx.x / PER_L, r = blockIdx.x % PER_L, nb = r / KQI, q = r % KQI;
    const int lane = threadIdx.x & 63, i = lane & 31, kh = lane >> 5;
    const float* sc = A.mods + 32 + (size_t)l * A.d.MB + X::M_EQUI + D;
    const float4* c0 = reinterpret_cast<const float4*>(A.W + F.c0[l]) + (size_t)nb * X::KQD * 64;
    const float4* ine = reinterpret_cast<const float4*>(A.W + F.ine[l]);
    double a0 = 0., a1 = 0., a2 = 0., a3 = 0.;
#pragma unroll 2
    for (int qj = 0; qj < X::KQD; ++qj) {
#pragma unroll
        for (int khj = 0; khj < 2; ++khj) {
            const float4 w = c0[qj * 64 + i + 32 * khj];
            const float wv[4] = {w.x, w.y, w.z, w.w};
#pragma unroll
            for (int cj = 0; cj < 4; ++cj) {
                const int m = 4 * qj + cj, j = (m >> 4) * 32 + khj * 16 + (m & 15);
                const int s_ = j & 15, h_ = (j >> 4) & 1, ij = (s_ & 3) + 4 * h_ + 8 * (s_ >> 2);
                const float4 v = ine[((size_t)(j >> 5) * KQI + q) * 64 + ij + 32 * kh];
                const double f = (double)wv[cj] * (1.0 + (double)sc[j]);
                a0 += f * v.x; a1 += f * v.y; a2 += f * v.z; a3 += f * v.w;
            }
        }
    }
    const float m4[4] = {(float)a0, (float)a1, (float)a2, (float)a3};
    reinterpret_cast<float4*>(out)[((size_t)l * PER_L + r) * 64 + lane] = make_float4(m4[0], m4[1], m4[2], m4[3]);
    if (out_s) {
        unsigned short t[3][4];
#pragma unroll
        for (int c = 0; c < 4; ++c) {
            const __bf16 h = (__bf16)m4[c];
            const float r1 = m4[c] - (float)h;
            const __bf16 m = (__bf16)r1;
            const __bf16 lo = (__bf16)(r1 - (float)m);
            t[0][c] = __builtin_bit_cast(unsigned short, h); t[1][c] = __builtin_bit_cast(unsigned short, m); t[2][c] = __builtin_bit_cast(unsigned short, lo);
        }
        constexpr int NS = KQI / 2;
        const size_t stepbase = (((size_t)l * X::ND + nb) * NS + (q >> 1)) * 3;
#pragma unroll
        for (int term = 0; term < 3; ++term) {
            unsigned short* dst = out_s + ((stepbase + term) * 64 + lane) * 8 + 4 * (q & 1);
            *reinterpret_cast<uint2*>(dst) = make_uint2((unsigned)t[term][0] | ((unsigned)t[term][1] << 16), (unsigned)t[term][2] | ((unsigned)t[term][3] << 16));
        }
    }
}

template <int D, int R>
__global__ __launch_bounds__(64, 1) void k_edge_update(KArgs A) {
    if (!A.flags[FLAG_ASYM]) return;
    using X = Dim<D>;
    constexpr int NCH = R * X::De / 64;
    constexpr int KQ4 = R * X::De / 8;
    const int lane = threadIdx.x & 63, j = lane & 31, half = lane >> 5;
    const int it = blockIdx.x;
    const int strip = A.pd.item_strip[it], t0 = A.pd.item_t0[it], t1 = A.pd.item_t1[it], part = A.pd.item_part[it];
    const LaneNode L = lane_node(A, strip, j);
    const float* mrow = mod_row(A, L.b) + A.mod_base;
    const float* eg1 = mrow + X::M_EDGE + 2 * X::De;
    const float* qsh = mrow + X::M_EQUI;
    const float gscale = mrow[X::M_GBF + 0], gshift = mrow[X::M_GBF + 1];
    const float4 pv = reinterpret_cast<const float4*>(A.pos_out)[L.v];
    const float cscale = A.W[A.wb[JB_CSCALE]];
    const WSrc ws = make_wsrc(A.W, lane);
    const unsigned o3 = (unsigned)(A.wb[JB_FF3_W] * 4), o4 = (unsigned)(A.wb[JB_FF4_W] * 4);
    const unsigned oro = (unsigned)(A.wb[JB_ERO_W] * 4), oi = (unsigned)(A.wb[JB_INE_W] * 4), o0 = (unsigned)(A.wb[JB_C0_W] * 4);
    WPipe<X::PG> wp;
    wpipe_prime(wp, ws, o3);
    float dax = 0.f, day = 0.f, daz = 0.f;
    for (int t = t0; t < t1; ++t) {
        const bool inr = L.valid && t < L.n;
        const bool ok = inr && t != L.i;
        const int tc = inr ? t : 0;
        const int u = L.noff + tc;
        const size_t r = (size_t)L.eoff + (size_t)L.i * L.n + tc;
        const float* eg1_ = launder(eg1);
        const float* es2_ = eg1_ + X::De, *ec2_ = es2_ + X::De, *eg2_ = ec2_ + X::De;
        const float* qsh_ = launder(qsh);
        const float* qsc_ = qsh_ + D;
        const float* cst = launder(A.W);
        const float* n2bias_ = cst + A.wb[JB_N2E_B], *b3_ = cst + A.wb[JB_FF3_B], *b4_ = cst + A.wb[JB_FF4_B];
        const float* b0_ = cst + A.wb[JB_C0_B], *w2_ = cst + A.wb[JB_C2_W], *tab_ = cst + A.wb[JB_GBF];
        const float* bro_ = cst + A.wb[JB_ERO_B];
        TRow wrow = trow(A.wrow, X::ND, L.v, half);
        wrow.p = launder(wrow.p);
        const TRow wcol = trow(A.wcol, X::ND, u, half);
        const float4 pu = reinterpret_cast<const float4*>(A.pos_out)[u];
        const float dx = pv.x - pu.x, dy = pv.y - pu.y, dz = pv.z - pu.z;
        const float d2 = dx * dx + dy * dy + dz * dz;
        float G[X::HE];
        gbf_n<X::NE>(d2, gscale, gshift, tab_, half, G);
        float en[X::HE];
        {
            const TRow ra = trow(A.n2e, X::NE, L.v, half), rc = trow(A.n2e, X::NE, u, half);
#pragma unroll
            for (int b = 0; b < X::NE; ++b) {
                float e[16], ta[16], tc2[16], g[16], bb[16];
                load16(A.e + r * X::De + b * 32 + half * 16, e);
                load16T(ra, b, ta);
                load16T(rc, b, tc2);
                load16(eg1_ + b * 32 + half * 16, g);
                load16(n2bias_ + b * 32 + half * 16, bb);
#pragma unroll
                for (int s = 0; s < 16; ++s) en[b * 16 + s] = fmaf(g[s], ta[s] + tc2[s] + bb[s], e[s]);
            }
        }
        layer_norm<X::HE>(en);
        modulate<X::NE>(en, es2_, ec2_, half);
        {
            f32x16 o[X::NE];
#pragma unroll
            for (int b = 0; b < X::NE; ++b) o[b] = zero16();
#pragma unroll
            for (int c = 0; c < NCH; ++c) {
                float hid[32];
#pragma unroll
                for (int b2 = 0; b2 < 2; ++b2) {
                    const unsigned wcur = o3 + (unsigned)(c * 2 + b2) * X::KQE * 1024;
                    const unsigned wnx = b2 == 0 ? wcur + X::KQE * 1024 : o4 + (unsigned)(c * 8) * 1024;
                    float bb[16];
                    load16(b3_ + (c * 2 + b2) * 32 + half * 16, bb);
                    f32x16 acc = mfma_block_p<X::KQE>(wp, ws, wcur, wnx, en, zero16());
                    silu_bias16(acc, bb, hid + b2 * 16);
                }
#pragma unroll
                for (int ob = 0; ob < X::NE; ++ob) {
                    const unsigned wcur = o4 + (unsigned)(ob * KQ4 + c * 8) * 1024;
                    const unsigned wnx = ob + 1 < X::NE ? o4 + (unsigned)((ob + 1) * KQ4 + c * 8) * 1024
                                                        : (c + 1 < NCH ? o3 + (unsigned)((c + 1) * 2) * X::KQE * 1024 : oro);
                    o[ob] = mfma_block_p<8>(wp, ws, wcur, wnx, hid, o[ob]);
                }
            }
#pragma unroll
            for (int b = 0; b < X::NE; ++b) {
                float ob4[16], og2[16];
                load16(b4_ + b * 32 + half * 16, ob4);
                load16(eg2_ + b * 32 + half * 16, og2);
#pragma unroll
                for (int s = 0; s < 16; ++s) en[b * 16 + s] = fmaf(og2[s], o[b][s] + ob4[s], en[b * 16 + s]);
            }
        }
        if (inr) store_nat<X::NE>(A.e_out + r * X::De, half, en);
        {
            float bb[16];
            load16(bro_ + half * 16, bb);
            f32x16 acc = mfma_block_p<X::KQE>(wp, ws, oro, oi, en, zero16());
            float rr[16];
#pragma unroll
            for (int s = 0; s < 16; ++s) rr[s] = acc[s] + bb[s];
            if (inr && (half == 0 || A.d.cep == 32)) store16(A.ehid + r * A.d.KEH + X::De + A.layer * A.d.cep + half * 16, rr);
        }
        float uu[X::HD];
#pragma unroll
        for (int b = 0; b < X::ND; ++b) {
            const unsigned we = oi + (unsigned)(b * 2 * X::KQE) * 1024, wg_ = we + X::KQE * 1024;
            float a1[16], a2[16];
            load16T(wrow, b, a1);
            load16T(wcol, b, a2);
            f32x16 acc = mfma_block_p<X::KQE>(wp, ws, we, wg_, en, zero16());
            acc = mfma_block_p<X::KQE>(wp, ws, wg_, b + 1 < X::ND ? wg_ + X::KQE * 1024 : o0, G, acc);
#pragma unroll
            for (int s = 0; s < 16; ++s) uu[b * 16 + s] = acc[s] + a1[s] + a2[s];
        }
        layer_norm<X::HD>(uu);
        modulate<X::ND>(uu, qsh_, qsc_, half);
        float c0 = 0.f, c1 = 0.f, c2 = 0.f;
#pragma unroll 1
        for (int b = 0; b < X::ND; ++b) {
            const unsigned wcur = o0 + (unsigned)b * X::KQD * 1024;
            const unsigned wnx = b + 1 < X::ND ? wcur + X::KQD * 1024 : o3;
            float bb[16], k0[16], k1[16], k2[16];
            load16(b0_ + b * 32 + half * 16, bb);
            load16(w2_ + b * 32 + half * 16, k0);
            load16(w2_ + D + b * 32 + half * 16, k1);
            load16(w2_ + 2 * D + b * 32 + half * 16, k2);
            f32x16 acc = mfma_block_p<X::KQD>(wp, ws, wcur, wnx, uu, zero16());
#pragma unroll
            for (int s = 0; s < 16; ++s) {
                const float ys = silu_f(acc[s] + bb[s]);
                c0 = fmaf(ys, k0[s], c0);
                c1 = fmaf(ys, k1[s], c1);
                c2 = fmaf(ys, k2[s], c2);
            }
        }
        c0 = tanh_f(pair_sum(c0));
        c1 = tanh_f(pair_sum(c1));
        c2 = tanh_f(pair_sum(c2));
        const int fl = A.eflag[r];
        const float iota = (c0 + ((fl & 1) ? c1 : 0.f) + ((fl & 2) ? c2 : 0.f)) * (1.f / 3.f);
        const float nrm = fmaxf(sqrtf(d2), 1e-8f);
        const float f = ok ? cscale * iota / nrm : 0.f;
        dax = fmaf(dx, f, dax);
        day = fmaf(dy, f, day);
        daz = fmaf(dz, f, daz);
    }
    if (half == 0)
        reinterpret_cast<float4*>(A.dpos)[(size_t)L.v * A.pd.max_parts + part] = make_float4(dax, day, daz, 0.f);
}
// ... 336 lines not shown
                const unsigned we = oi + (unsigned)(b * 2 * X::KQE) * 1024, wg_ = we + X::KQE * 1024;
                f32x16 acc = mfma_block_p<X::KQE>(wp, ws, we, wg_, en, zero16());
                acc = mfma_block_p<X::KQE>(wp, ws, wg_, b + 1 < X::ND ? wg_ + X::KQE * 1024 : o0, G, acc);
    #pragma unroll
                for (int s = 0; s < 16; ++s) {
                    if (b < X::ND - PLB) park[(b < X::ND - PLB ? b : 0) * 16 + s] = acc[s];
                }
                if (b >= X::ND - PLB) {
    #pragma unroll
                    for (int q = 0; q < 4; ++q)
                        pl[((b - (X::ND - PLB)) * 4 + q) * 64 + lane] = make_float4(acc[q * 4 + 0], acc[q * 4 + 1], acc[q * 4 + 2], acc[q * 4 + 3]);
                }
            }
            PT(3);
    #pragma unroll 1
            for (int dir = 0; dir < 2; ++dir) {
                if (dsel >= 0 && dir != dsel) continue;
                BRow ra = wrow_i, rc = wcol_j;
                if (dir == 1) { ra.voff = wrow_j.voff; rc.voff = wcol_i.voff; }
                float uu[X::HD];
                constexpr int GB = D == 256 ? 4 : 2;
    #pragma unroll
                for (int g = 0; g < X::ND / GB; ++g) {
                    float a1[GB * 16], a2[GB * 16];
    #pragma unroll
                    for (int k = 0; k < GB; ++k) {
                        float t1[16], t2[16];
                        bload16(ra, g * GB + k, t1);
                        bload16(rc, g * GB + k, t2);
    #pragma unroll
                        for (int s = 0; s < 16; ++s) { a1[k * 16 + s] = t1[s]; a2[k * 16 + s] = t2[s]; }
                    }
                    pipeline_fence();
    #pragma unroll
                    for (int k = 0; k < GB; ++k) {
                        const int b = g * GB + k;
                        float pk[16];
                        if (b < X::ND - PLB) {
    #pragma unroll
                            for (int s = 0; s < 16; ++s) pk[s] = park[(b < X::ND - PLB ? b : 0) * 16 + s];
                        } else {
    #pragma unroll
                            for (int q = 0; q < 4; ++q) {
                                const float4 t = pl[((b - (X::ND - PLB)) * 4 + q) * 64 + lane];
                                pk[q * 4 + 0] = t.x; pk[q * 4 + 1] = t.y; pk[q * 4 + 2] = t.z; pk[q * 4 + 3] = t.w;
                            }
                        }
    #pragma unroll
                        for (int s = 0; s < 16; ++s) uu[b * 16 + s] = pk[s] + (a1[k * 16 + s] + a2[k * 16 + s]);
                    }
                }
                PT(6);
                layer_norm<X::HD>(uu);
                modulate<X::ND>(uu, qsh_, qsc_, half);
                PT(4);
                float c0 = 0.f, c1 = 0.f, c2 = 0.f;
    #pragma unroll 1
                for (int b = 0; b < X::ND; ++b) {
                    const unsigned wcur = o0 + (unsigned)b * X::KQD * 1024;
                    const unsigned wnx = b + 1 < X::ND ? wcur + X::KQD * 1024 : ((dir == 0 && dsel < 0) ? o0 : o3);
                    float bb[16], k0[16], k1[16], k2[16];
                    load16(b0_ + b * 32 + half * 16, bb);
                    load16(w2_ + b * 32 + half * 16, k0);
                    load16(w2_ + D + b * 32 + half * 16, k1);
                    load16(w2_ + 2 * D + b * 32 + half * 16, k2);
                    f32x16 acc = mfma_block_p<X::KQD>(wp, ws, wcur, wnx, uu, zero16());
    #pragma unroll
                    for (int s = 0; s < 16; ++s) {
                        const float ys = silu_f(acc[s] + bb[s]);
                        c0 = fmaf(ys, k0[s], c0);
                        c1 = fmaf(ys, k1[s], c1);
                        c2 = fmaf(ys, k2[s], c2);
                    }
                }
                PT(dir == 0 ? 5 : 7);
                c0 = tanh_f(pair_sum(c0));
                c1 = tanh_f(pair_sum(c1));
                c2 = tanh_f(pair_sum(c2));
                const size_t rr = dir == 0 ? P.rij : P.rji;
                const int fl = A.eflag[rr];
                const float iota = (c0 + ((fl & 1) ? c1 : 0.f) + ((fl & 2) ? c2 : 0.f)) * (1.f / 3.f);
                const float nrm = fmaxf(sqrtf(d2), 1e-8f);
                const float f = cscale * iota / nrm;
                const float sgn = dir == 0 ? 1.f : -1.f;
                if (P.ok && half == 0)
                    reinterpret_cast<float4*>(A.dposE)[rr] = make_float4(sgn * dx * f, sgn * dy * f, sgn * dz * f, 0.f);
                PT(6);
            }
        }
    }
    PT_FLUSH;
}

template <int D>
__device__ __forceinline__ void node_head_body(const KArgs& A, int strip) {
    using X = Dim<D>;
    const int lane = threadIdx.x & 63, j = lane & 31, half = lane >> 5;
    const int v = strip * 32 + j;
    const int KNH = A.d.KNH;
    const WSrc ws = make_wsrc(A.W, lane);
    const unsigned o1 = (unsigned)(A.wg[JW_NH1_W] * 4), o2 = (unsigned)(A.wg[JW_NH2_W] * 4), o3 = (unsigned)(A.wg[JW_NH3_W] * 4);
    WPipe<4> wp;
    wpipe_prime(wp, ws, o1);
    f32x16 o[X::ND];
#pragma unroll
    for (int b = 0; b < X::ND; ++b) o[b] = zero16();
    {
        const int kq = KNH / 8, nch = KNH / 64;
#pragma unroll 1
        for (int c = 0; c < nch; ++c) {
            float x[32];
            load_nat<2>(A.ahid + (size_t)v * KNH + c * 64, half, x);
#pragma unroll
            for (int ob = 0; ob < X::ND; ++ob) {
                const unsigned cur = o1 + (unsigned)(ob * kq + c * 8) * 1024;
                const unsigned nxt = ob + 1 < X::ND ? o1 + (unsigned)((ob + 1) * kq + c * 8) * 1024
                                                    : (c + 1 < nch ? o1 + (unsigned)((c + 1) * 8) * 1024 : o2);
                o[ob] = mfma_block_p<8>(wp, ws, cur, nxt, x, o[ob]);
            }
        }
    }
    float a1[X::HD];
    {
        const float* bias = A.W + A.wg[JW_NH1_B];
#pragma unroll
        for (int b = 0; b < X::ND; ++b) {
            float r[16];
            acc_bias(o[b], bias + b * 32 + half * 16, r);
#pragma unroll
            for (int s = 0; s < 16; ++s) a1[b * 16 + s] = silu_f(r[s]);
        }
    }
    float a2[X::HD / 2];
    {
        const float* bias = A.W + A.wg[JW_NH2_B];
#pragma unroll
        for (int b = 0; b < X::ND / 2; ++b) {
            const unsigned cur = o2 + (unsigned)(b * X::KQD) * 1024;
            f32x16 acc = mfma_block_p<X::KQD>(wp, ws, cur, b + 1 < X::ND / 2 ? cur + X::KQD * 1024 : o3, a1, zero16());
            float r[16];
            acc_bias(acc, bias + b * 32 + half * 16, r);
#pragma unroll
            for (int s = 0; s < 16; ++s) a2[b * 16 + s] = silu_f(r[s]);
        }
    }
    {
        f32x16 acc = mfma_block_p<X::KQD / 2>(wp, ws, o3, o3, a2, zero16());
        float r[16];
        acc_bias(acc, A.W + A.wg[JW_NH3_B] + half * 16, r);
        store16(A.apred + (size_t)v * 32 + half * 16, r);
    }
}
template <int D>
__global__ __launch_bounds__(64, 1) void k_node_head(KArgs A) { node_head_body<D>(A, (int)blockIdx.x); }

template <int D, int NBK, bool SYM>
__device__ __forceinline__ void edge_head_body(const KArgs& A, int blk) {
    if ((A.flags[FLAG_ASYM] != 0) == SYM) return;
    using X = Dim<D>;
    const int lane = threadIdx.x & 63, j = lane & 31, half = lane >> 5;
    const int ur = SYM ? A.pd.ut_rows[((size_t)blk * 32 + j) * 2] : 0, um = SYM ? A.pd.ut_rows[((size_t)blk * 32 + j) * 2 + 1] : 0;
    const size_t r = SYM ? (size_t)(ur < 0 ? 0 : ur) : (size_t)blk * 32 + j;
    const WSrc ws = make_wsrc(A.W, lane);
    const unsigned o1 = (unsigned)(A.wg[JW_EH1_W] * 4), o2 = (unsigned)(A.wg[JW_EH2_W] * 4), o3 = (unsigned)(A.wg[JW_EH3_W] * 4);
    WPipe<4> wp;
    wpipe_prime(wp, ws, o1);
    float x[NBK * 16];
    load_nat<NBK>(A.ehid + r * (NBK * 32), half, x);
    float a1[X::De];
    {
        const float* bias = A.W + A.wg[JW_EH1_B];
#pragma unroll
        for (int b = 0; b < 2 * X::NE; ++b) {
            const unsigned cur = o1 + (unsigned)(b * NBK * 4) * 1024;
            f32x16 acc = mfma_block_p<NBK * 4>(wp, ws, cur, b + 1 < 2 * X::NE ? cur + (unsigned)(NBK * 4) * 1024 : o2, x, zero16());
            float rr[16];
            acc_bias(acc, bias + b * 32 + half * 16, rr);
#pragma unroll
            for (int s = 0; s < 16; ++s) a1[b * 16 + s] = silu_f(rr[s]);
        }
    }
    float a2[X::De / 2];
    {
        const float* bias = A.W + A.wg[JW_EH2_B];
#pragma unroll
        for (int b = 0; b < X::NE; ++b) {
            const unsigned cur = o2 + (unsigned)(b * (X::De / 4)) * 1024;
            f32x16 acc = mfma_block_p<X::De / 4>(wp, ws, cur, b + 1 < X::NE ? cur + (unsigned)(X::De / 4) * 1024 : o3, a1, zero16());
            float rr[16];
            acc_bias(acc, bias + b * 32 + half * 16, rr);
#pragma unroll
            for (int s = 0; s < 16; ++s) a2[b * 16 + s] = silu_f(rr[s]);
        }
    }
    {
        f32x16 acc = mfma_block_p<X::De / 8>(wp, ws, o3, o3, a2, zero16());
        float rr[16];
        acc_bias(acc, A.W + A.wg[JW_EH3_B] + half * 16, rr);
        if (SYM) {
            if (half == 0 && ur >= 0) {
                reinterpret_cast<float4*>(A.epred)[ur] = make_float4(rr[0], rr[1], rr[2], rr[3]);
                reinterpret_cast<float4*>(A.epred)[um] = make_float4(rr[0], rr[1], rr[2], rr[3]);
            }
        } else if (half == 0 && r < (size_t)A.pd.rows) {
            reinterpret_cast<float4*>(A.epred)[r] = make_float4(rr[0], rr[1], rr[2], rr[3]);
        }
    }
}
template <int D, int NBK, bool SYM>
__global__ __launch_bounds__(64, 1) void k_edge_head(KArgs A) { edge_head_body<D, NBK, SYM>(A, (int)blockIdx.x); }

template <int D, int NBK>
__global__ __launch_bounds__(64, 1) void k_heads_sym(KArgs A) {
    const int ns = A.pd.n_strips;
    if ((int)blockIdx.x < ns) node_head_body<D>(A, (int)blockIdx.x);
    else edge_head_body<D, NBK, true>(A, (int)blockIdx.x - ns);
}

}
}
```

### jodo_amd/csrc/dgt_plan.cpp

```cpp
#include <algorithm>
#include <numeric>
#include <utility>
#include <new>
#include "dgt_plan.h"
#include "jodo_hip_internal.h"

static size_t align_up(size_t x, size_t a) { return (x + a - 1) / a * a; }

static std::vector<int> xcd_order(const std::vector<int32_t>& strip, int group) {
    const int n = (int)strip.size();
    std::vector<std::vector<int>> q(8);
    for (int i = 0; i < n; ++i) q[strip[i] & 7].push_back(i);
    size_t pos[8] = {0, 0, 0, 0, 0, 0, 0, 0};
    std::vector<int> out;
    out.reserve(n);
    int wg = 0;
    while ((int)out.size() < n) {
        int c = wg & 7, tries = 0;
        while (pos[c] >= q[c].size() && tries < 8) { c = (c + 1) & 7; ++tries; }
        for (int k = 0; k < group && pos[c] < q[c].size(); ++k) out.push_back(q[c][pos[c]++]);
        ++wg;
    }
    return out;
}

static void permute(std::vector<int32_t>& a, const std::vector<int>& ord) {
    std::vector<int32_t> b(a.size());
    for (size_t i = 0; i < ord.size(); ++i) b[i] = a[ord[i]];
    a.swap(b);
}

int dgt_dims_from_cfg(const jodo_cfg* c, DgtDims* d) {
    if (c->nf != 128 && c->nf != 256 && c->nf != 384)
        return jodo_set_error(JODO_ERR_UNSUPPORTED, "nf=%d: kernels are built for nf=128, nf=256 and nf=384", c->nf);
    if (c->layout != 0 && c->layout != 1) return jodo_set_error(JODO_ERR_ARG, "layout=%d (0 or 1)", c->layout);
    if (c->n_heads != 16 || c->n_extra != 2)
        return jodo_set_error(JODO_ERR_UNSUPPORTED, "n_heads=%d n_extra_heads=%d: kernels are built for 16/2", c->n_heads, c->n_extra);
    if (c->mlp_ratio != 2 && c->mlp_ratio != 4)
        return jodo_set_error(JODO_ERR_UNSUPPORTED, "mlp_ratio=%d: supported 2, 4", c->mlp_ratio);
    if (c->n_layers < 1 || c->n_layers > 32) return jodo_set_error(JODO_ERR_ARG, "n_layers=%d", c->n_layers);
    if (c->in_node_dim < 1 || 2 * c->in_node_dim > 64) return jodo_set_error(JODO_ERR_ARG, "in_node_dim=%d", c->in_node_dim);
    if (c->edge_ch < 1 || c->edge_ch > 4) return jodo_set_error(JODO_ERR_ARG, "edge_ch=%d (1..4)", c->edge_ch);
    if (c->cond_ch < 0 || c->cond_ch > 8) return jodo_set_error(JODO_ERR_ARG, "cond_ch=%d", c->cond_ch);
    d->D = c->nf; d->De = c->nf / 4; d->T = c->nf * 4; d->L = c->n_layers; d->H = c->n_heads; d->XH = c->n_extra;
    d->SH = d->H - d->XH; d->C = d->D / d->H; d->SC = (d->H * d->C) / d->SH; d->r = c->mlp_ratio;
    d->nd = c->in_node_dim; d->ch = c->edge_ch; d->cond_ch = c->cond_ch;
    const int cn = (2 * d->D) / d->L, ce = (2 * d->De) / d->L;
    d->cnp = std::max(d->D / 4, (cn + 31) / 32 * 32);
    d->cep = std::max((d->D / 16 + 15) / 16 * 16, (ce + 15) / 16 * 16);
    if (d->cep > 32) return jodo_set_error(JODO_ERR_UNSUPPORTED, "n_layers=%d at nf=%d: edge readout width %d beyond one 32-row block", d->L, d->D, ce);
    d->wide = (c->nf != 256 || c->layout == 1 || d->cnp != 64) ? 1 : 0;
    int tail = d->SC - 16;
    d->QKP = d->wide ? d->SH * 32 : (d->SH / 2 + (tail + 1) / 2) * 32;
    d->ndp = (2 * d->nd + 7) / 8 * 8;
    d->einp = (2 * d->ch + 7) / 8 * 8;
    d->KNH = d->D + d->L * d->cnp; d->KEH = d->De + d->L * d->cep;
    if (d->KEH % 32 != 0) return jodo_set_error(JODO_ERR_UNSUPPORTED, "edge head width %d not a multiple of 32", d->KEH);
    d->MB = 6 * d->D + 6 * d->De + 2 * d->D + 32 + 2 * d->D;
    d->Mtot = 32 + (int64_t)d->L * d->MB;
    d->cutoff = c->spatial_cut_off; d->edge_th = c->edge_quan_th;
    return JODO_OK;
}

extern "C" int jodo_plan_create(const jodo_cfg* cfg, int B, int N, const int32_t* n_nodes, int max_chunk,
                                jodo_plan** out) {
    if (!cfg || !n_nodes || !out || B <= 0 || N <= 0) return jodo_set_error(JODO_ERR_ARG, "plan_create: bad argument");
    jodo_plan* p = new (std::nothrow) jodo_plan();
    if (!p) return jodo_set_error(JODO_ERR_ARG, "plan_create: out of host memory");
    p->cfg = *cfg;
    int rc = dgt_dims_from_cfg(cfg, &p->dims);
    if (rc != JODO_OK) { delete p; return rc; }
    for (int b = 0; b < B; ++b)
        if (n_nodes[b] < 1 || n_nodes[b] > N) {
            delete p;
            return jodo_set_error(JODO_ERR_ARG, "plan_create: n_nodes[%d]=%d outside [1,%d]", b, n_nodes[b], N);
        }
    int pair_chunk = (max_chunk >> 16) & 0xff, spair_chunk = (max_chunk >> 24) & 0xff;
    max_chunk &= 0xffff;
    if (max_chunk <= 0) {
        int64_t strip_nmax_sum = 0;
        {
            std::vector<int> sorted(n_nodes, n_nodes + B);
            std::sort(sorted.begin(), sorted.end(), [](int a, int b) { return a > b; });
            int64_t v = 0;
            int strip = -1;
            for (int m = 0; m < B; ++m) {
                const int first = (int)(v / 32), last = (int)((v + sorted[m] - 1) / 32);
                for (int s = std::max(first, strip + 1); s <= last; ++s) strip_nmax_sum += sorted[m];
                strip = std::max(strip, last);
                v += sorted[m];
            }
        }
        max_chunk = 8;
        while (max_chunk > 2 && strip_nmax_sum / max_chunk < 2048) --max_chunk;
    }
    if (pair_chunk <= 0) pair_chunk = 1;
    const bool spair_auto = spair_chunk <= 0;
    p->B = B; p->N = N; p->max_blocks = -1; p->last_pos_buf = 0; p->last_e_buf = 0;
    p->opt[JODO_OPT_FUSE_NEXT_QKV] = 1; p->opt[JODO_OPT_DIR_SPLIT] = 1; p->opt[JODO_OPT_NODE_POST_WAVES] = 0; p->opt[JODO_OPT_ATTN_VARIANT] = 0; p->opt[JODO_OPT_HEADS_MIX] = 1; p->opt[JODO_OPT_HALF_ROWS] = 1; p->opt[JODO_OPT_PRE_EMBED] = 1; p->opt[JODO_OPT_AB_PRE] = 1; p->opt[JODO_OPT_Z_SPLIT] = 1;
    p->opt[JODO_OPT_PIN_SYMMETRIC] = 0; p->opt[JODO_OPT_PIN_UNIFORM_T] = 0; p->opt[JODO_OPT_ROT_STATS] = 1; p->opt[JODO_OPT_NODE_MIX] = 1;
    p->opt[JODO_OPT_SPLIT_BF16] = 0; p->split_w = nullptr; p->split_bytes = 0;
    p->prof_enabled = 0; p->force_directed = 0; p->dbg_timing = nullptr;

    std::vector<int> order(B);
    std::iota(order.begin(), order.end(), 0);
    std::stable_sort(order.begin(), order.end(), [&](int a, int b) { return n_nodes[a] > n_nodes[b]; });

    int64_t Nn = 0, rows = 0, dir = 0;
    for (int b = 0; b < B; ++b) { Nn += n_nodes[b]; rows += (int64_t)n_nodes[b] * n_nodes[b]; dir += (int64_t)n_nodes[b] * (n_nodes[b] - 1); }
    if (rows >= (int64_t)1 << 31) { delete p; return jodo_set_error(JODO_ERR_UNSUPPORTED, "batch too large: %lld dense edge rows", (long long)rows); }
    p->Nn = (int)Nn; p->Nn_pad = (int)align_up((size_t)Nn, 32); p->n_strips = p->Nn_pad / 32;
    p->rows = rows; p->dir_edges = dir;

    std::vector<int32_t> node_b(p->Nn_pad, 0), node_i(p->Nn_pad, 0), node_n(p->Nn_pad, 0), node_noff(p->Nn_pad, 0),
        node_eoff(p->Nn_pad, 0), orig_n(B), orig_noff(B), orig_eoff(B);
    int v = 0; int64_t eoff = 0;
    for (int m = 0; m < B; ++m) {
        int b = order[m], n = n_nodes[b];
        orig_n[b] = n; orig_noff[b] = v; orig_eoff[b] = (int32_t)eoff;
        for (int i = 0; i < n; ++i) {
            node_b[v + i] = b; node_i[v + i] = i; node_n[v + i] = n; node_noff[v + i] = v; node_eoff[v + i] = (int32_t)eoff;
        }
        v += n; eoff += (int64_t)n * n;
    }
    std::vector<int32_t> it_strip, it_t0, it_t1, it_part, strip_parts(p->n_strips, 0);
    int max_parts = 1;
    for (int s = 0; s < p->n_strips; ++s) {
        int nmax = 0;
        for (int j = 0; j < 32; ++j) nmax = std::max(nmax, (int)node_n[s * 32 + j]);
        if (nmax == 0) continue;
        int parts = (nmax + max_chunk - 1) / max_chunk;
        int chunk = (nmax + parts - 1) / parts;
        parts = (nmax + chunk - 1) / chunk;
        max_parts = std::max(max_parts, parts);
        strip_parts[s] = parts;
        for (int q = 0; q < parts; ++q) {
            it_strip.push_back(s); it_t0.push_back(q * chunk); it_t1.push_back(std::min(nmax, (q + 1) * chunk)); it_part.push_back(q);
        }
    }
    p->n_items = (int)it_strip.size(); p->max_parts = max_parts;
    {
        const std::vector<int> ord = xcd_order(it_strip, 4);
        permute(it_strip, ord); permute(it_t0, ord); permute(it_t1, ord); permute(it_part, ord);
    }
    std::vector<int32_t> pi_strip, pi_t0, pi_t1;
    for (int s = 0; s < p->n_strips; ++s) {
        int nmax = 0;
        for (int j = 0; j < 32; ++j) nmax = std::max(nmax, (int)node_n[s * 32 + j]);
        const int dmax = nmax / 2;
        if (dmax == 0) continue;
        int parts = (dmax + pair_chunk - 1) / pair_chunk;
        int chunk = (dmax + parts - 1) / parts;
        parts = (dmax + chunk - 1) / chunk;
        for (int q = 0; q < parts; ++q) { pi_strip.push_back(s); pi_t0.push_back(q * chunk); pi_t1.push_back(std::min(dmax, (q + 1) * chunk)); }
    }
    p->n_pitems = (int)pi_strip.size();
    p->pitems_single = 1;
    for (size_t i = 0; i < pi_strip.size(); ++i) if (pi_t1[i] - pi_t0[i] != 1) p->pitems_single = 0;
    {
        const std::vector<int> ord = xcd_order(pi_strip, 1);
        permute(pi_strip, ord); permute(pi_t0, ord); permute(pi_t1, ord);
    }
    std::vector<int32_t> ag_node, ai_group, ai_t0, ai_t1, ai_part, ai_dir, ad_group, ad_t0, ad_t1, ad_part, ad_big, anode_parts(p->Nn_pad, 0), aw_off;
    int amax_parts = 1;
    {
        constexpr int G = 128;
        const bool persist = spair_auto;
        int achunk = (spair_auto || spair_chunk == 255) ? 0 : spair_chunk;
        std::vector<int> mol_n(B), mol_noff(B);
        for (int m = 0; m < B; ++m) { mol_n[m] = n_nodes[order[m]]; mol_noff[m] = orig_noff[order[m]]; }
        std::vector<char> used(B, 0);
        std::vector<int> g_nmax, g_big;
        int head = 0;
        while (head < B) {
            if (used[head]) { ++head; continue; }
            if (mol_n[head] > G) {
                for (int o = 0; o < mol_n[head]; o += G) {
                    for (int k = 0; k < G; ++k) ag_node.push_back(o + k < mol_n[head] ? mol_noff[head] + o + k : -1);
                    g_nmax.push_back(mol_n[head]); g_big.push_back(1);
                }
                used[head++] = 1;
                continue;
            }
            int fill = 0, nmax = mol_n[head];
            std::vector<int32_t> lanes;
            for (int m = head; m < B && fill < G; ++m) {
                if (used[m] || mol_n[m] > G - fill) continue;
                for (int k = 0; k < mol_n[m]; ++k) lanes.push_back(mol_noff[m] + k);
                fill += mol_n[m]; used[m] = 1;
            }
            lanes.resize(G, -1);
            ag_node.insert(ag_node.end(), lanes.begin(), lanes.end());
            g_nmax.push_back(nmax); g_big.push_back(0);
        }
        const int ng = (int)g_nmax.size();
        p->n_agroups = ng;
        if (persist) achunk = 6;
        if (achunk <= 0 && p->dims.wide) {
            int64_t iters = 0;
            for (int g = 0; g < ng; ++g) iters += std::max(1, g_nmax[g] / 2);
            achunk = 6;
            while (achunk > 1 && iters / achunk < 2 * 256) --achunk;
        }
        if (achunk <= 0) {
            std::vector<double> slot(256);
            double best = 0.0;
            for (int c = 1; c <= 16; ++c) {
                std::vector<int> len;
                for (int g = 0; g < ng; ++g) {
                    if (g_big[g]) { len.push_back(g_nmax[g]); continue; }
                    const int dmax = g_nmax[g] / 2, parts = std::max(1, (dmax + c - 1) / c), cp = dmax > 0 ? (dmax + parts - 1) / parts : 0;
                    for (int q = 0; q < parts; ++q) len.push_back(std::min(dmax, (q + 1) * cp) - std::min(dmax, q * cp));
                }
                std::stable_sort(len.begin(), len.end(), [](int a, int b) { return a > b; });
                std::fill(slot.begin(), slot.end(), 0.0);
                for (int l : len) { auto it = std::min_element(slot.begin(), slot.end()); *it += 0.8 + (double)l; }
                const double mk = *std::max_element(slot.begin(), slot.end());
                if (achunk <= 0 || mk <= best) { best = mk; achunk = c; }
            }
        }
        struct It { int g, t0, t1, part, big; };
        std::vector<It> pit, dit;
        std::vector<int> g_parts(ng, 1), pit_dir;
        if (persist) {
            const double a_item = 0.3;
            const double w_dir = 0.9;
            auto g_len = [&](int g) { return g_big[g] ? g_nmax[g] : g_nmax[g] / 2; };
            auto g_wgt = [&](int g) { return g_big[g] ? w_dir : 1.0; };
            double total = 0.0;
            for (int g = 0; g < ng; ++g) total += a_item + g_wgt(g) * (double)g_len(g);
            double T = std::max(total / JODO_ATT_SLOTS, a_item + 1.0);
            aw_off.assign(JODO_ATT_SLOTS + 1, 0);
            for (int attempt = 0; attempt < 400; ++attempt, T *= 1.004) {
                pit.clear();
                int slot = 0;
                double load = 0.0;
                auto next_slot = [&]() { if (slot + 1 < JODO_ATT_SLOTS) { ++slot; load = 0.0; } };
                for (int g = 0; g < ng; ++g) {
                    const int len = g_len(g);
                    const double wg = g_wgt(g);
                    int t = 0, part = 0;
                    do {
                        double room = T - load - a_item;
                        if (room < 0.75 && load > 0.0 && slot + 1 < JODO_ATT_SLOTS) { next_slot(); room = T - a_item; }
                        int take = std::min(len - t, std::max(1, (int)(room / wg + 0.5)));
                        take = std::max(take, 0);
                        pit.push_back({g, t, t + take, part++, slot});
                        load += a_item + wg * (double)take;
                        t += take;
                        if (load >= T - 0.5) next_slot();
                    } while (t < len);
                    g_parts[g] = part;
                }
// ... 4 lines not shown
            for (It& it : pit) { it.big = 0; pit_dir.push_back(g_big[it.g]); }
        }
        for (int g = 0; g < ng; ++g) {
            const int nmax = g_nmax[g], dmax = nmax / 2;
            int parts;
            if (persist) parts = g_parts[g];
            else if (g_big[g]) parts = std::max(1, (nmax + 2 * achunk - 1) / (2 * achunk));
            else parts = std::max(1, (dmax + achunk - 1) / achunk);
            amax_parts = std::max(amax_parts, parts);
            const int cp = dmax > 0 ? (dmax + parts - 1) / parts : 0, cd = (nmax + parts - 1) / parts;
            for (int q = 0; q < parts; ++q) {
                if (!g_big[g] && !persist) pit.push_back({g, std::min(dmax, q * cp), std::min(dmax, (q + 1) * cp), q, 0});
                dit.push_back({g, std::min(nmax, q * cd), std::min(nmax, (q + 1) * cd), q, (g_big[g] && !persist) ? 1 : 0});
            }
            for (int k = 0; k < G; ++k) { const int v = ag_node[(size_t)g * G + k]; if (v >= 0) anode_parts[v] = parts; }
        }
        auto lpt = [](const It& a, const It& b) { return (a.t1 - a.t0) > (b.t1 - b.t0); };
        if (!persist) std::stable_sort(pit.begin(), pit.end(), lpt);
        std::stable_sort(dit.begin(), dit.end(), lpt);
        for (const It& it : pit) { ai_group.push_back(it.g); ai_t0.push_back(it.t0); ai_t1.push_back(it.t1); ai_part.push_back(it.part); }
        ai_dir.assign(pit.size(), 0);
        for (size_t i = 0; i < pit_dir.size(); ++i) ai_dir[i] = pit_dir[i];
        p->n_ai_dir = 0;
        for (size_t i = 0; i < ai_dir.size(); ++i) p->n_ai_dir += ai_dir[i] ? 1 : 0;
        for (const It& it : dit) { ad_group.push_back(it.g); ad_t0.push_back(it.t0); ad_t1.push_back(it.t1); ad_part.push_back(it.part); ad_big.push_back(it.big); }
        p->n_aitems = (int)pit.size(); p->n_aditems = (int)dit.size(); p->amax_parts = amax_parts;
        p->a_persist = persist ? 1 : 0;
        if (!persist) aw_off.assign(1, 0);
        p->has_big = 0;
        for (int g = 0; g < ng; ++g) p->has_big |= (g_big[g] && !persist) ? 1 : 0;
    }

    auto put = [&](const std::vector<int32_t>& a, size_t* off) {
        *off = p->desc.size();
        p->desc.insert(p->desc.end(), a.begin(), a.end());
        while (p->desc.size() % 64) p->desc.push_back(0);
    };
    put(node_b, &p->off_node_b); put(node_i, &p->off_node_i); put(node_n, &p->off_node_n);
    put(node_noff, &p->off_node_noff); put(node_eoff, &p->off_node_eoff);
    put(orig_n, &p->off_orig_n); put(orig_noff, &p->off_orig_noff); put(orig_eoff, &p->off_orig_eoff);
    put(it_strip, &p->off_item_strip); put(it_t0, &p->off_item_t0); put(it_t1, &p->off_item_t1); put(it_part, &p->off_item_part); put(strip_parts, &p->off_strip_parts);
    put(pi_strip, &p->off_pitem_strip); put(pi_t0, &p->off_pitem_t0); put(pi_t1, &p->off_pitem_t1);
    put(ag_node, &p->off_ag_node); put(ai_group, &p->off_ai_group); put(ai_t0, &p->off_ai_t0); put(ai_t1, &p->off_ai_t1); put(ai_part, &p->off_ai_part); put(ai_dir, &p->off_ai_dir);
    put(ad_group, &p->off_ad_group); put(ad_t0, &p->off_ad_t0); put(ad_t1, &p->off_ad_t1); put(ad_part, &p->off_ad_part); put(ad_big, &p->off_ad_big);
    put(anode_parts, &p->off_anode_parts); put(aw_off, &p->off_aw_off);
    {
        std::vector<int32_t> ut;
        for (int b = 0; b < B; ++b) {
            const int n = orig_n[b];
            const int64_t e0 = orig_eoff[b];
            for (int i = 0; i < n; ++i)
                for (int d = 1; 2 * d <= n; ++d) {
                    if (2 * d == n && 2 * i >= n) continue;
                    const int j = (i + d) % n;
                    ut.push_back((int32_t)(e0 + (int64_t)i * n + j)); ut.push_back((int32_t)(e0 + (int64_t)j * n + i));
                }
        }
        while ((ut.size() / 2) % 32) { ut.push_back(-1); ut.push_back(-1); }
        p->n_ut_pad = (int)(ut.size() / 2);
        put(ut, &p->off_ut_rows);
    }
    {
        std::vector<int32_t> gsa, gsc;
        for (int s = 0; s < p->n_strips; ++s) {
            int lo = s, hi = s;
            for (int j = 0; j < 32; ++j) {
                const int v0 = s * 32 + j;
                if (node_n[v0] <= 0) continue;
                lo = std::min(lo, (int)node_noff[v0] / 32);
                hi = std::max(hi, (int)(node_noff[v0] + node_n[v0] - 1) / 32);
            }
            for (int c = lo; c <= hi; ++c) { gsa.push_back(s); gsc.push_back(c); }
        }
        {
            std::vector<int> ord(gsa.size());
            std::iota(ord.begin(), ord.end(), 0);
            std::stable_sort(ord.begin(), ord.end(), [&](int a, int b) { return std::max(gsa[a], gsc[a]) < std::max(gsa[b], gsc[b]); });
            permute(gsa, ord); permute(gsc, ord);
        }
        p->n_gtiles = (int)gsa.size(); p->gt_cache_full = -1; p->gt_cache_count = 0;
        put(gsa, &p->off_gt_sa); put(gsc, &p->off_gt_sc);
    }

    const DgtDims& d = p->dims;
    size_t o = 0;
    auto take = [&](size_t bytes) { size_t at = o; o = align_up(o + bytes, 256); return at; };
    const size_t f = sizeof(float), NP = (size_t)p->Nn_pad, R = (size_t)rows + 32, Bp = align_up((size_t)B, 32);
    WsLayout& w = p->ws;
    w.hid1 = take(Bp * d.T * f); w.temb = take(Bp * d.T * f); w.tembs = take(Bp * d.T * f); w.mods = take(Bp * (size_t)d.Mtot * f);
    w.condh = take(Bp * (size_t)std::max(1, d.cond_ch) * d.D * f); w.condh2 = take(Bp * (size_t)std::max(1, d.cond_ch) * d.D * f);
    w.pos0 = take(NP * 4 * f); w.pos1 = take(NP * 4 * f); w.dpos = take(NP * max_parts * 4 * f); w.cpos = take(NP * 4 * f);
    w.feat = take(NP * d.ndp * f); w.h = take(NP * d.D * f); w.hhat = take(NP * amax_parts * d.D * f);
    w.astat = take(NP * amax_parts * 32 * f);
    w.q = take(NP * d.QKP * f); w.k = take(NP * d.QKP * f); w.v = take(NP * d.D * f); w.n2e = take(NP * d.De * f);
    w.wrow = take(NP * d.D * f); w.wcol = take(NP * d.D * f); w.ua = take(NP * d.D * f); w.ub = take(NP * d.D * f); w.rmean = take(NP * 2 * f); w.mfold = take((size_t)d.L * d.D * 2 * d.De * f); w.mfold_s = take((size_t)d.L * d.D * 2 * d.De * 6); w.ffold_s = take((size_t)d.L * d.D * d.D * 6); w.ffold = take((size_t)d.L * d.D * d.D * f); w.ahid = take(NP * d.KNH * f);
    w.apred = take(NP * 32 * f);
    w.eflag = take(R * sizeof(int32_t)); w.e = take(R * d.De * f); w.e2 = take(R * d.De * f);
    w.ehid = take(R * d.KEH * f); w.epred = take(R * 4 * f); w.dposE = take(R * 4 * f); w.gramE = take(R * f);
    w.total = o;
    *out = p;
    return JODO_OK;
}

extern "C" void jodo_plan_destroy(jodo_plan* p) {
    if (!p) return;
    for (void* e : p->prof_ev) (void)hipEventDestroy((hipEvent_t)e);
    for (void* e : p->prof_pool) (void)hipEventDestroy((hipEvent_t)e);
    delete p;
}
extern "C" int jodo_profile_enable(jodo_plan* p, int enable) {
    if (!p) return jodo_set_error(JODO_ERR_ARG, "null plan");
    p->prof_enabled = enable;
    return JODO_OK;
}
extern "C" int jodo_profile_read(jodo_plan* p, float* ms_sum, int32_t* launches) {
    if (!p || !ms_sum || !launches) return jodo_set_error(JODO_ERR_ARG, "profile_read: null");
    for (int c = 0; c < JODO_PROF_COUNT; ++c) { ms_sum[c] = 0.f; launches[c] = 0; }
    for (size_t i = 0; i + 1 < p->prof_ev.size(); i += 2) {
        hipEvent_t a = (hipEvent_t)p->prof_ev[i], b = (hipEvent_t)p->prof_ev[i + 1];
        hipError_t e = hipEventSynchronize(b);
        float ms = 0.f;
        if (e == hipSuccess) e = hipEventElapsedTime(&ms, a, b);
        if (e != hipSuccess) return jodo_set_error(JODO_ERR_LAUNCH, "profile_read: %s", hipGetErrorString(e));
        const int c = p->prof_cls[i / 2];
        ms_sum[c] += ms; launches[c] += 1;
        p->prof_pool.push_back(p->prof_ev[i]); p->prof_pool.push_back(p->prof_ev[i + 1]);
    }
    p->prof_ev.clear(); p->prof_cls.clear();
    return JODO_OK;
}
extern "C" size_t jodo_plan_desc_bytes(const jodo_plan* p) { return p ? p->desc.size() * sizeof(int32_t) : 0; }
extern "C" size_t jodo_plan_workspace_bytes(const jodo_plan* p) { return p ? p->ws.total : 0; }
extern "C" int64_t jodo_plan_mod_len(const jodo_plan* p) { return p ? p->dims.Mtot : 0; }
extern "C" int jodo_plan_stats(const jodo_plan* p, int64_t* o) {
    if (!p || !o) return jodo_set_error(JODO_ERR_ARG, "plan_stats: null");
    o[0] = p->Nn; o[1] = p->rows; o[2] = p->dir_edges; o[3] = p->n_strips; o[4] = p->n_items; o[5] = p->max_parts;
    return JODO_OK;
}

namespace {
inline double proj(int out, int K) { return (double)((out + 31) / 32) * (double)((K + 7) / 8 * 4); }
}
extern "C" int jodo_plan_work(const jodo_plan* p, int uniform_t, int symmetric, double* mfma_flops) {
    if (!p || !mfma_flops) return jodo_set_error(JODO_ERR_ARG, "plan_work: null");
    const DgtDims& d = p->dims;
    const bool tuned = !d.wide, sym = symmetric && !p->force_directed && p->n_pitems > 0;
    const int D = d.D, De = d.De, L = d.L, r = d.r;
    const int32_t* dsc = p->desc.data();
    double cls[JODO_PROF_COUNT] = {0, 0, 0, 0, 0, 0, 0, 0};
    const double strips = p->n_strips;
    const double rowgroups = (uniform_t && d.cond_ch == 0) ? 1.0 : (double)((p->B + 31) / 32);
    cls[JODO_PROF_PROLOGUE] += rowgroups * (proj(d.T, d.T) + proj((int)d.Mtot, d.T));
    if (d.cond_ch > 0) cls[JODO_PROF_PROLOGUE] += (double)((p->B * d.cond_ch + 31) / 32) * proj(D, D) + (double)((p->B + 31) / 32) * proj(d.T, d.cond_ch * D);
    cls[JODO_PROF_PROLOGUE] += strips * proj(D, d.ndp);
    double dir_iters = 0, pair_iters = 0;
    for (int i = 0; i < p->n_items; ++i) dir_iters += dsc[p->off_item_t1 + i] - dsc[p->off_item_t0 + i];
    for (int i = 0; i < p->n_pitems; ++i) pair_iters += dsc[p->off_pitem_t1 + i] - dsc[p->off_pitem_t0 + i];
    cls[(p->opt[JODO_OPT_PRE_EMBED] != 0 && L > 0) ? JODO_PROF_NODE_PRE : JODO_PROF_PROLOGUE] += dir_iters * proj(De, d.einp + De);
    const int nqb = tuned ? 8 : d.SH;
    const double qkv = 2.0 * nqb * (D / 2) + proj(D, D);
    const bool fuse_pre = tuned && p->opt[JODO_OPT_FUSE_NEXT_QKV] != 0 && L > 1 && p->n_strips >= 1024;
    const bool ab_pre = !fuse_pre && p->opt[JODO_OPT_AB_PRE] != 0 && L > 1 && (!tuned || (p->n_strips < 1024 && p->opt[JODO_OPT_NODE_POST_WAVES] == 0));
    cls[JODO_PROF_NODE_PRE] += strips * qkv * ((fuse_pre || ab_pre) ? 1 : L);
    if (fuse_pre || ab_pre) cls[JODO_PROF_NODE_POST] += strips * qkv * (L - 1);
    cls[JODO_PROF_NODE_POST] += L * strips * (proj(De, D) + proj(r * D, D) + proj(D, r * D) + 2 * proj(D, D) + proj(d.cnp, D));
    const bool hoist = sym && (D == 256 || uniform_t);
    if (p->n_pitems > 0 && (D == 256 || uniform_t)) cls[JODO_PROF_NODE_POST] += L * strips * 2 * proj(D, D);
    const double att_iter = proj(De, 2 * De) + nqb * (double)(De / 2) + proj(D, De);
    double att_iters = 0;
    for (int i = 0; i < p->n_aitems; ++i) if (sym) att_iters += 4.0 * (dsc[p->off_ai_t1 + i] - dsc[p->off_ai_t0 + i]);
    for (int i = 0; i < p->n_aditems; ++i)
        if (!sym || dsc[p->off_ad_big + i]) att_iters += 4.0 * (dsc[p->off_ad_t1 + i] - dsc[p->off_ad_t0 + i]);
    cls[JODO_PROF_EDGE_ATTN] += L * att_iters * att_iter;
    const double trunk = proj(r * De, De) + proj(De, r * De) + proj(d.cep, De) + proj(D, 2 * De);
    if (sym) {
        const bool fold = uniform_t && d.cond_ch == 0;
        const double c0 = fold ? proj(D, 2 * De) : (hoist ? proj(D, D) : 2 * proj(D, D));
        double tr = trunk;
        if (fold && p->opt[JODO_OPT_ROT_STATS]) {
            tr -= proj(D, 2 * De);
            for (int b = 0; b < 2 * De / 32; ++b) tr += (double)(2 * De - 32 * b) / 2;
            cls[JODO_PROF_NODE_POST] += L * (double)p->n_gtiles * (double)(D - 2 * De) / 2;
        }
        cls[JODO_PROF_EDGE_UPDATE] += L * pair_iters * (tr + c0);
        if (p->opt[JODO_OPT_Z_SPLIT] != 0 && hoist && p->opt[JODO_OPT_PIN_UNIFORM_T] != (fold ? 2 : 1)) {
            const int rem = p->n_pitems % 1024;
            const int zw = rem > 0 ? (rem <= 256 ? 4 : ((p->opt[JODO_OPT_Z_SPLIT] == 2 && rem <= 512) ? 2 : 1)) : 1;
            cls[JODO_PROF_EDGE_UPDATE] += L * (double)rem * (zw - 1) * tr;
        }
    } else {
        cls[JODO_PROF_EDGE_UPDATE] += L * dir_iters * (trunk + proj(D, D));
    }
    cls[JODO_PROF_EPILOGUE] += strips * (proj(D, d.KNH) + proj(D / 2, D) + proj(d.nd, D / 2));
    const double eh = 2 * proj(De, d.KEH) + proj(De, 2 * De) + proj(32, De);
    cls[JODO_PROF_EPILOGUE] += (sym ? (double)(p->n_ut_pad / 32) : (double)((p->rows + 31) / 32)) * eh;
    for (int c = 0; c < JODO_PROF_COUNT; ++c) mfma_flops[c] = cls[c] * 4096.0;
    return JODO_OK;
}

extern "C" int jodo_plan_upload(jodo_plan* p, void* desc_dev, void* stream) {
    if (!p || !desc_dev) return jodo_set_error(JODO_ERR_ARG, "plan_upload: null");
    hipError_t e = hipMemcpyAsync(desc_dev, p->desc.data(), p->desc.size() * sizeof(int32_t), hipMemcpyHostToDevice,
                                  (hipStream_t)stream);
    if (e != hipSuccess) return jodo_set_error(JODO_ERR_LAUNCH, "plan_upload: %s", hipGetErrorString(e));
    return JODO_OK;
}
extern "C" int jodo_debug_set_timing_buffer(jodo_plan* p, void* dev16xu64) {
    if (!p) return jodo_set_error(JODO_ERR_ARG, "null plan");
    p->dbg_timing = dev16xu64;
    return JODO_OK;
}
extern "C" int jodo_debug_set_force_directed(jodo_plan* p, int on) {
    if (!p) return jodo_set_error(JODO_ERR_ARG, "null plan");
    if (on && p->opt[JODO_OPT_PIN_SYMMETRIC] == 1)
        return jodo_set_error(JODO_ERR_ARG, "set_force_directed: the plan is pinned to the symmetric path");
    p->force_directed = on;
    return JODO_OK;
}
extern "C" int jodo_plan_set_option(jodo_plan* p, int option, int value) {
    if (!p) return jodo_set_error(JODO_ERR_ARG, "null plan");
    if (option < 0 || option >= JODO_OPT_COUNT) return jodo_set_error(JODO_ERR_ARG, "plan_set_option: unknown option %d", option);
    if (option == JODO_OPT_NODE_POST_WAVES && value != 0 && value != 1 && value != 2 && value != 4 && value != 12 && value != 14)
        return jodo_set_error(JODO_ERR_ARG, "plan_set_option: node-post waves per strip must be 0 (auto), 1, 2 or 4");
    if (option == JODO_OPT_SPLIT_BF16 && (value < 0 || value > 2))
        return jodo_set_error(JODO_ERR_ARG, "plan_set_option: the split-bf16 form is 0 (off), 1 (pair update + node kernel) or 2 (also the attention kernel: experiments, measured slower), got %d", value);
    if ((option == JODO_OPT_FUSE_NEXT_QKV || option == JODO_OPT_DIR_SPLIT || option == JODO_OPT_NODE_MIX || option == JODO_OPT_HEADS_MIX || option == JODO_OPT_HALF_ROWS || option == JODO_OPT_PRE_EMBED || option == JODO_OPT_AB_PRE) && value != 0 && value != 1)
        return jodo_set_error(JODO_ERR_ARG, "plan_set_option: option %d is a switch (0 or 1), got %d", option, value);
    if (option == JODO_OPT_Z_SPLIT && (value < 0 || value > 2))
        return jodo_set_error(JODO_ERR_ARG, "plan_set_option: the Z split is 0 (off), 1 (four waves for a last round of <= 256 items) or 2 (also two waves up to 512), got %d", value);
    if (option == JODO_OPT_ROT_STATS && (value < 0 || value > 2))
        return jodo_set_error(JODO_ERR_ARG, "plan_set_option: rotated statistics are 0 (off), 1 (on) or 2 (on, uncentred Gram tiles: tests), got %d", value);
    if (option == JODO_OPT_PIN_SYMMETRIC && value == 1 && p->force_directed)
        return jodo_set_error(JODO_ERR_ARG, "plan_set_option: the symmetric pin contradicts jodo_debug_set_force_directed");
    if ((option == JODO_OPT_PIN_SYMMETRIC || option == JODO_OPT_PIN_UNIFORM_T) && (value < 0 || value > 2))
        return jodo_set_error(JODO_ERR_ARG, "plan_set_option: a pin is 0 (none), 1 or 2, got %d", value);
    if (option == JODO_OPT_ATTN_VARIANT && (value < 0 || value > 3))
        return jodo_set_error(JODO_ERR_ARG, "plan_set_option: attention variant must be 0..3, got %d", value);
    p->opt[option] = value;
    return JODO_OK;
}
extern "C" int jodo_debug_attn_schedule(const jodo_plan* p, int64_t* o) {
    if (!p || !o) return jodo_set_error(JODO_ERR_ARG, "attn_schedule: null");
    const int32_t* d = p->desc.data();
    int64_t iters = 0;
    for (int i = 0; i < p->n_aitems; ++i) iters += d[p->off_ai_t1 + i] - d[p->off_ai_t0 + i];
    o[0] = p->n_aitems; o[1] = iters; o[2] = p->amax_parts; o[3] = p->a_persist; o[4] = o[5] = o[6] = o[7] = 0;
    {
        std::vector<std::vector<std::pair<int, int>>> per((size_t)p->n_agroups);
        std::vector<std::vector<int>> parts((size_t)p->n_agroups);
        for (int i = 0; i < p->n_aitems; ++i) {
            const int g = d[p->off_ai_group + i];
            if (g < 0 || g >= p->n_agroups) return jodo_set_error(JODO_ERR_ARG, "attn_schedule: item %d names group %d", i, g);
            per[g].push_back({d[p->off_ai_t0 + i], d[p->off_ai_t1 + i]});
            parts[g].push_back(d[p->off_ai_part + i]);
        }
        for (int g = 0; g < p->n_agroups; ++g) {
            int nmax = 0, want_parts = 0;
            for (int k = 0; k < 128; ++k) {
                const int v = d[p->off_ag_node + (size_t)g * 128 + k];
                if (v >= 0) { nmax = std::max(nmax, (int)d[p->off_node_n + v]); want_parts = d[p->off_anode_parts + v]; }
            }
            const bool bigg = nmax > 128;
            if (bigg && !p->a_persist) { if (!per[g].empty()) return jodo_set_error(JODO_ERR_ARG, "attn_schedule: pair items for the big group %d", g); continue; }
            for (int i = 0; i < p->n_aitems; ++i)
                if (d[p->off_ai_group + i] == g && d[p->off_ai_dir + i] != (bigg ? 1 : 0)) return jodo_set_error(JODO_ERR_ARG, "attn_schedule: item %d of group %d has the wrong mode", i, g);
            std::sort(per[g].begin(), per[g].end());
            std::sort(parts[g].begin(), parts[g].end());
            int at = 0;
            for (const auto& it : per[g]) {
                if (it.first != at || it.second < it.first) return jodo_set_error(JODO_ERR_ARG, "attn_schedule: group %d offsets not tiled at %d", g, at);
                at = it.second;
            }
            const int want_len = bigg ? nmax : nmax / 2;
            if (at != want_len || per[g].empty()) return jodo_set_error(JODO_ERR_ARG, "attn_schedule: group %d covers %d of %d offsets", g, at, want_len);
            for (size_t q = 0; q < parts[g].size(); ++q)
                if (parts[g][q] != (int)q) return jodo_set_error(JODO_ERR_ARG, "attn_schedule: group %d partial indices are not 0..%d", g, (int)parts[g].size() - 1);
            if ((int)parts[g].size() != want_parts) return jodo_set_error(JODO_ERR_ARG, "attn_schedule: group %d has %d items, its atoms expect %d partials", g, (int)parts[g].size(), want_parts);
        }
    }
    if (p->a_persist) {
        int64_t lo = INT64_MAX, hi = 0, mi = 0, idle = 0;
        for (int s = 0; s < JODO_ATT_SLOTS; ++s) {
            const int k0 = d[p->off_aw_off + s], k1 = d[p->off_aw_off + s + 1];
            int64_t l = 0;
            for (int k = k0; k < k1; ++k) l += d[p->off_ai_t1 + k] - d[p->off_ai_t0 + k];
            lo = std::min(lo, l); hi = std::max(hi, l); mi = std::max<int64_t>(mi, k1 - k0); idle += (k1 == k0);
        }
        o[4] = lo; o[5] = hi; o[6] = mi; o[7] = idle;
    }
    return JODO_OK;
}
extern "C" int jodo_plan_set_split_weights(jodo_plan* p, const void* tape_dev, size_t bytes) {
    if (!p) return jodo_set_error(JODO_ERR_ARG, "null plan");
    if (tape_dev) {
        size_t total = 0, per_block = 0, node_block = 0, attn_block = 0;
        const int rc = p->dims.cond_ch > 0 ? jodo_dgt_split_cond_size(&p->cfg, &total, &per_block)
                                           : jodo_dgt_split_size(&p->cfg, &total, &per_block, &node_block, &attn_block);
        if (rc != JODO_OK) return rc;
        if (bytes != total) return jodo_set_error(JODO_ERR_ARG, "set_split_weights: %zu bytes, this configuration's tape has %zu", bytes, total);
    }
    p->split_w = tape_dev; p->split_bytes = tape_dev ? bytes : 0;
    return JODO_OK;
}
extern "C" int jodo_debug_set_max_blocks(jodo_plan* p, int mb) {
    if (!p) return jodo_set_error(JODO_ERR_ARG, "null plan");
    p->max_blocks = mb;
    return JODO_OK;
}
```

### jodo_amd/csrc/dgt_plan.h

```cpp
#pragma once
#include <stdint.h>
#include <stddef.h>
#include <vector>
#include "../../include/jodo_hip.h"

constexpr int JODO_ATT_SLOTS = 256;

struct DgtDims {
    int D, De, T, L, H, XH, SH, SC, C, r, nd, ch, cond_ch;
    int QKP;
    int ndp;
    int einp;
    int cnp, cep;
    int KNH, KEH;
    int MB;
    int64_t Mtot;
    float cutoff, edge_th;
    int wide;
};

struct PlanDev {
    const int* node_b;
    const int* node_i;
    const int* node_n;
    const int* node_noff;
    const int* node_eoff;
    const int* orig_n;
    const int* orig_noff;
    const int* orig_eoff;
    const int* item_strip;
    const int* item_t0;
    const int* item_t1;
    const int* item_part;
    const int* strip_parts;
    const int* pitem_strip;
    const int* pitem_t0;
    const int* pitem_t1;
    const int* ag_node;
    const int* ai_group;
    const int* ai_t0;
    const int* ai_t1;
    const int* ai_part;
    const int* ai_dir;
    const int* ad_group;
    const int* ad_t0;
    const int* ad_t1;
    const int* ad_part;
    const int* ad_big;
    const int* anode_parts;
    const int* aw_off;
    int a_persist;
    const int* ut_rows;
    int n_ut_pad;
    const int* gt_sa;
    const int* gt_sc;
    int n_gtiles;
    int n_agroups, n_aitems, n_aditems, amax_parts;
    int Nn, Nn_pad, n_strips, n_items, n_pitems, B, N, max_parts;
    int64_t rows;
};

struct WsLayout {
    size_t hid1, temb, tembs, mods, condh, condh2;
    size_t pos0, pos1, dpos, cpos, feat, h, hhat, astat, q, k, v, n2e, wrow, wcol, ua, ub, rmean, mfold, ffold, ahid, apred;
    size_t eflag, e, e2, ehid, epred, dposE, gramE;
    size_t ffold_s;
    size_t mfold_s;
    size_t total;
};

struct jodo_plan {
    jodo_cfg cfg;
    DgtDims dims;
    int B, N, Nn, Nn_pad, n_strips, n_items, n_pitems, max_parts;
    int n_agroups, n_aitems, n_aditems, amax_parts, n_ut_pad, n_gtiles;
    int a_persist;
    size_t off_aw_off;
    int has_big;
    size_t off_ag_node, off_ai_group, off_ai_t0, off_ai_t1, off_ai_part, off_ai_dir, off_ad_group, off_ad_t0, off_ad_t1, off_ad_part, off_ad_big, off_anode_parts, off_ut_rows, off_gt_sa, off_gt_sc;
    int64_t rows, dir_edges;
    std::vector<int32_t> desc;
    size_t off_node_b, off_node_i, off_node_n, off_node_noff, off_node_eoff, off_orig_n, off_orig_noff,
        off_orig_eoff, off_item_strip, off_item_t0, off_item_t1, off_item_part, off_strip_parts, off_pitem_strip, off_pitem_t0, off_pitem_t1;
    WsLayout ws;
    int prof_enabled;
    std::vector<void*> prof_ev;
    std::vector<int> prof_cls;
    std::vector<void*> prof_pool;
    int force_directed;
    void* dbg_timing;
    int max_blocks;
    int last_pos_buf;
    int last_e_buf;
    int opt[JODO_OPT_COUNT];
    const void* split_w;
    size_t split_bytes;
    int n_ai_dir;
    int pitems_single;
    int gt_cache_full, gt_cache_count;
};

int dgt_dims_from_cfg(const jodo_cfg* cfg, DgtDims* d);
```

Measured before the change: 173.9.

## Merge prologue/epilogue frame kernels and fold node embedding into pre-attention items

```diff
diff --git a/include/jodo_hip.h b/include/jodo_hip.h
--- a/include/jodo_hip.h
+++ b/include/jodo_hip.h
@@ -89,9 +89,12 @@
     JODO_OPT_AB_PRE = 11,
     JODO_OPT_Z_SPLIT = 12,
     JODO_OPT_SPLIT_BF16 = 13,
+    JODO_OPT_FRAME_MIX = 14,
     JODO_OPT_COUNT
 };
 int jodo_plan_set_option(jodo_plan* plan, int option, int value);
+
+int jodo_debug_frame_mix_map(int n_strips, int n_items, int32_t* out);
 
 int jodo_debug_attn_schedule(const jodo_plan* plan, int64_t* out8);
 
diff --git a/jodo_amd/csrc/dgt_forward.hip b/jodo_amd/csrc/dgt_forward.hip
--- a/jodo_amd/csrc/dgt_forward.hip
+++ b/jodo_amd/csrc/dgt_forward.hip
@@ -89,19 +89,38 @@
 template <int D, int NBK>
 int launch_edge_head(hipStream_t st, const KArgs& A, bool merged) {
     if (merged) {
-        LAUNCH((wide::k_heads_sym<D, NBK>), (unsigned)(A.pd.n_strips + A.pd.n_ut_pad / 32), 64, A);
+        LAUNCH((wide::k_heads_sym<D, NBK>), (unsigned)(A.pd.n_strips + A.pos_items + A.pd.n_ut_pad / 32), 64, A);
         return JODO_OK;
     }
-    LAUNCH((wide::k_node_head<D>), A.pd.n_strips, 64, A);
+    LAUNCH((wide::k_node_head<D>), A.pd.n_strips + A.pos_items, 64, A);
     if (A.pd.n_ut_pad > 0 && A.pin_sym != 2) LAUNCH((wide::k_edge_head<D, NBK, true>), (unsigned)(A.pd.n_ut_pad / 32), 64, A);
     if (A.pin_sym != 1) LAUNCH((wide::k_edge_head<D, NBK, false>), (unsigned)((A.pd.rows + 31) / 32), 64, A);
     return JODO_OK;
 }
 
-__global__ __launch_bounds__(64, 1) void k_pre_embed(KArgs A) {
-    const int npre = A.pd.n_strips * 3;
-    if ((int)blockIdx.x < npre) node_pre_body<false>(A, (int)blockIdx.x);
-    else wide::embed_edges_body<256>(A, (int)blockIdx.x - npre);
+template <int EKQ>
+__global__ __launch_bounds__(64, 1) void k_pre_embed(KArgs A, int interleave) {
+    const int npre = A.pd.n_strips * 3, ne = A.pd.n_items, b = (int)blockIdx.x;
+    int emb = b >= npre, idx = emb ? b - npre : b;
+    if (interleave) idx = jodo_frame_mix_map(b, npre, ne, &emb);
+    if (!emb) node_pre_body<false, EKQ>(A, idx);
+    else wide::embed_edges_body<256>(A, idx);
+}
+int launch_pre_embed(hipStream_t st, const KArgs& A, int M, int ekq) {
+    const unsigned grid = (unsigned)(A.pd.n_strips * 3 + A.pd.n_items);
+    switch (ekq) {
+        case 0: LAUNCH(k_pre_embed<0>, grid, 64, A, M); break;
+        case 1: LAUNCH(k_pre_embed<1>, grid, 64, A, M); break;
+        case 2: LAUNCH(k_pre_embed<2>, grid, 64, A, M); break;
+        case 3: LAUNCH(k_pre_embed<3>, grid, 64, A, M); break;
+        case 4: LAUNCH(k_pre_embed<4>, grid, 64, A, M); break;
+        case 5: LAUNCH(k_pre_embed<5>, grid, 64, A, M); break;
+        case 6: LAUNCH(k_pre_embed<6>, grid, 64, A, M); break;
+        case 7: LAUNCH(k_pre_embed<7>, grid, 64, A, M); break;
+        case 8: LAUNCH(k_pre_embed<8>, grid, 64, A, M); break;
+        default: return jodo_set_error(JODO_ERR_UNSUPPORTED, "node input width %d", 8 * ekq);
+    }
+    return JODO_OK;
 }
 
 
@@ -211,8 +230,12 @@
 int forward_blocks(jodo_plan* p, hipStream_t st, KArgs& A, const int64_t* woff, float* const posbuf[2], std::unique_ptr<ProfScope>& pro) {
     const DgtDims& d = p->dims;
     int rc = JODO_OK;
-    LAUNCH(k_pack_nodes, (p->Nn_pad + 255) / 256, 256, A);
-    switch (d.ndp / 8) {
+    const int fm = p->opt[JODO_OPT_FRAME_MIX], mix = fm & 1;
+    const int nblocks = (p->max_blocks >= 0 && p->max_blocks < d.L) ? p->max_blocks : d.L;
+    const bool embed_merged = p->n_items > 0 && p->opt[JODO_OPT_PRE_EMBED] != 0 && nblocks > 0;
+    const int pre_ekq = (TUNED && mix && (fm & 2) && embed_merged) ? d.ndp / 8 : 0;
+    if (!mix) LAUNCH(k_pack_nodes, (p->Nn_pad + 255) / 256, 256, A);
+    if (!pre_ekq) switch (d.ndp / 8) {
         case 1: rc = launch_embed_nodes<D, 1>(st, A); break;
         case 2: rc = launch_embed_nodes<D, 2>(st, A); break;
         case 3: rc = launch_embed_nodes<D, 3>(st, A); break;
@@ -224,28 +247,35 @@
         default: return jodo_set_error(JODO_ERR_UNSUPPORTED, "node input width %d", d.ndp);
     }
     if (rc) return rc;
-    const bool embed_merged = p->n_items > 0 && p->opt[JODO_OPT_PRE_EMBED] != 0 && ((p->max_blocks >= 0 && p->max_blocks < d.L) ? p->max_blocks : d.L) > 0;
     if (p->n_items > 0 && !embed_merged) LAUNCH((wide::k_embed_edges<D>), p->n_items, 64, A);
     const bool pin_pair = p->opt[JODO_OPT_PIN_SYMMETRIC] == 1 && !p->force_directed, pin_dir = p->opt[JODO_OPT_PIN_SYMMETRIC] == 2 || p->force_directed;
     const bool can_fold = p->n_pitems > 0 && !pin_dir && p->opt[JODO_OPT_PIN_UNIFORM_T] != 2 && d.cond_ch == 0;
     A.rot = can_fold ? p->opt[JODO_OPT_ROT_STATS] : 0;
+    const bool fuse_pre = TUNED && p->opt[JODO_OPT_FUSE_NEXT_QKV] != 0 && nblocks > 1 && p->n_strips >= 1024;
+    const bool ab_pre = !fuse_pre && p->opt[JODO_OPT_AB_PRE] != 0 && nblocks > 1 && (!TUNED || (p->n_strips < 1024 && p->opt[JODO_OPT_NODE_POST_WAVES] == 0));
+    const int pmix = (mix && (fm & 4)) ? 1 : 0;
+    bool pos0_done = false;
     if (can_fold) {
         if (d.L > 16) return jodo_set_error(JODO_ERR_UNSUPPORTED, "more than 16 blocks");
-        FoldOffs F;
+        FoldPair F;
         for (int l = 0; l < 16; ++l) {
-            F.c0[l] = l < d.L ? woff[JW_GLOBAL_COUNT + l * JB_BLOCK_COUNT + JB_C0_W] : 0;
-            F.ine[l] = l < d.L ? woff[JW_GLOBAL_COUNT + l * JB_BLOCK_COUNT + (A.rot ? JB_INEC_W : JB_INE_W)] : 0;
-        }
-        LAUNCH((wide::k_fold_coord<D, D / 16>), d.L * (D / 32) * (d.De / 4), 64, A, F, A.mfold, 0, A.mfold_s);
-        if (A.rot) {
-            for (int l = 0; l < d.L; ++l) F.ine[l] = woff[JW_GLOBAL_COUNT + l * JB_BLOCK_COUNT + JB_QT_W];
-            LAUNCH((wide::k_fold_coord<D, D / 8>), d.L * (D / 32) * (D / 8), 64, A, F, A.ffold, 1, A.ffold_s);
+            F.m.c0[l] = F.f.c0[l] = l < d.L ? woff[JW_GLOBAL_COUNT + l * JB_BLOCK_COUNT + JB_C0_W] : 0;
+            F.m.ine[l] = l < d.L ? woff[JW_GLOBAL_COUNT + l * JB_BLOCK_COUNT + (A.rot ? JB_INEC_W : JB_INE_W)] : 0;
+            F.f.ine[l] = l < d.L ? woff[JW_GLOBAL_COUNT + l * JB_BLOCK_COUNT + JB_QT_W] : 0;
+        }
+        const int n_m = d.L * (D / 32) * (d.De / 4), n_f = A.rot ? d.L * (D / 32) * (D / 8) : 0;
+        if (!mix) {
+            LAUNCH((wide::k_fold_coord<D, D / 16>), n_m, 64, A, F.m, A.mfold, 0, A.mfold_s);
+            if (A.rot) LAUNCH((wide::k_fold_coord<D, D / 8>), n_f, 64, A, F.f, A.ffold, 1, A.ffold_s);
+        } else {
+            F.n_m = n_m; F.n_f = n_f;
+            pos0_done = nblocks > 0 && (fuse_pre || ab_pre);
+            F.npos = pos0_done ? (p->Nn_pad + 63) / 64 : 0;
+            A.layer = 0;
+            LAUNCH((wide::k_fold_coord2<D>), n_f + n_m + F.npos, 64, A, F);
         }
     }
     pro.reset();
-    const int nblocks = (p->max_blocks >= 0 && p->max_blocks < d.L) ? p->max_blocks : d.L;
-    const bool fuse_pre = TUNED && p->opt[JODO_OPT_FUSE_NEXT_QKV] != 0 && nblocks > 1 && p->n_strips >= 1024;
-    const bool ab_pre = !fuse_pre && p->opt[JODO_OPT_AB_PRE] != 0 && nblocks > 1 && (!TUNED || (p->n_strips < 1024 && p->opt[JODO_OPT_NODE_POST_WAVES] == 0));
     int cur = 0;
     for (int l = 0; l < nblocks; ++l) {
         A.layer = l;
@@ -270,13 +300,13 @@
             if constexpr (TUNED) {
                 if (!fuse_pre && !ab_pre) {
                     A.pre_mode = 0;
-                    if (l == 0 && embed_merged) LAUNCH(k_pre_embed, p->n_strips * 3 + p->n_items, 64, A);
+                    if (l == 0 && embed_merged) { rc = launch_pre_embed(st, A, pmix, pre_ekq); if (rc) return rc; }
                     else LAUNCH(k_node_pre, p->n_strips * 3, 64, A);
                 } else {
-                    LAUNCH(k_pos_final, (p->Nn_pad + 255) / 256, 256, A);
+                    if (l > 0 || !pos0_done) LAUNCH(k_pos_final, (p->Nn_pad + 255) / 256, 256, A);
                     if (l == 0) {
                         A.pre_mode = 1;
-                        if (embed_merged) LAUNCH(k_pre_embed, p->n_strips * 3 + p->n_items, 64, A);
+                        if (embed_merged) { rc = launch_pre_embed(st, A, pmix, pre_ekq); if (rc) return rc; }
                         else LAUNCH(k_node_pre, p->n_strips * 3, 64, A);
                     }
                 }
@@ -285,7 +315,7 @@
                 if (l == 0 && embed_merged) LAUNCH((k_pre_embed_w<D>), p->n_strips * 3 + p->n_items, 64, A);
                 else LAUNCH((wide::k_node_pre<D>), p->n_strips * 3, 64, A);
             } else {
-                LAUNCH(k_pos_final, (p->Nn_pad + 255) / 256, 256, A);
+                if (l > 0 || !pos0_done) LAUNCH(k_pos_final, (p->Nn_pad + 255) / 256, 256, A);
                 if (l == 0) {
                     A.pre_mode = 1;
                     if (embed_merged) LAUNCH((k_pre_embed_w<D>), p->n_strips * 3 + p->n_items, 64, A);
@@ -341,7 +371,8 @@
     ProfScope epi(p, st, JODO_PROF_EPILOGUE);
     A.pos_in = posbuf[cur]; A.pos_out = posbuf[cur ^ 1];
     A.layer = nblocks;
-    LAUNCH(k_pos_final, (p->Nn_pad + 255) / 256, 256, A);
+    if (mix) A.pos_items = (p->Nn_pad + 63) / 64;
+    else LAUNCH(k_pos_final, (p->Nn_pad + 255) / 256, 256, A);
     p->last_pos_buf = cur ^ 1;
     const bool heads_mix = A.pin_sym == 1 && A.pd.n_ut_pad > 0 && p->opt[JODO_OPT_HEADS_MIX] != 0;
     switch (d.KEH / 32) {
@@ -360,10 +391,14 @@
         default: return jodo_set_error(JODO_ERR_UNSUPPORTED, "edge head width %d", d.KEH);
     }
     if (rc) return rc;
-    LAUNCH(k_finalize_nodes, (p->B * p->N + 255) / 256, 256, A);
     {
         const size_t tot = (size_t)p->B * p->N * p->N;
-        LAUNCH(k_finalize_edges, (unsigned)((tot + 255) / 256), 256, A);
+        if (mix) {
+            LAUNCH(k_finalize, (unsigned)((p->B * p->N + 255) / 256 + (tot + 255) / 256), 256, A);
+        } else {
+            LAUNCH(k_finalize_nodes, (p->B * p->N + 255) / 256, 256, A);
+            LAUNCH(k_finalize_edges, (unsigned)((tot + 255) / 256), 256, A);
+        }
     }
     return JODO_OK;
 }
@@ -394,7 +429,7 @@
     for (int i = 0; i < JB_BLOCK_COUNT; ++i) A.wb[i] = 0;
     A.mod_base = 0; A.layer = 0; A.force_directed = p->force_directed; A.pin_sym = p->force_directed ? 0 : p->opt[JODO_OPT_PIN_SYMMETRIC];
     A.half_rows = (A.pin_sym == 1 && p->n_pitems > 0 && p->opt[JODO_OPT_HALF_ROWS] != 0) ? 1 : 0;
-    A.pin_uni = p->opt[JODO_OPT_PIN_UNIFORM_T]; A.pre_mode = 0; A.strip0 = 0; A.item0 = 0; A.dir_split = 0; A.rot = 0; A.mix_nw = 0; A.ab0 = 0; A.ab1 = 0; A.g0 = 0; A.g1 = 0; A.fuse_next = 0; A.mod_base_next = 0;
+    A.pin_uni = p->opt[JODO_OPT_PIN_UNIFORM_T]; A.pre_mode = 0; A.strip0 = 0; A.item0 = 0; A.dir_split = 0; A.rot = 0; A.mix_nw = 0; A.ab0 = 0; A.ab1 = 0; A.g0 = 0; A.g1 = 0; A.fuse_next = 0; A.mod_base_next = 0; A.pos_items = 0;
     for (int i = 0; i < 6; ++i) A.wbn[i] = 0;
     fill_ws(A, p, workspace);
     if (p->opt[JODO_OPT_SPLIT_BF16] >= 1 && p->split_w && (d.D == 256 || d.D == 384) && d.cond_ch == 0 && !p->force_directed && p->n_pitems > 0 && p->pitems_single &&
@@ -421,8 +456,15 @@
     p->last_e_buf = 0;
     std::unique_ptr<ProfScope> pro(new ProfScope(p, st, JODO_PROF_PROLOGUE));
     LAUNCH(k_flags_init, 1, 256, A);
-    { const size_t tot = (size_t)p->B * p->N * p->N; LAUNCH(k_check_sym, (unsigned)((tot + 255) / 256), 256, A); }
-    LAUNCH(k_time1, p->B, 256, A);
+    {
+        const size_t tot = (size_t)p->B * p->N * p->N;
+        if (p->opt[JODO_OPT_FRAME_MIX] & 1) {
+            LAUNCH(k_frame_inputs, (unsigned)(p->B + (p->Nn_pad + 255) / 256 + (tot + 255) / 256), 256, A);
+        } else {
+            LAUNCH(k_check_sym, (unsigned)((tot + 255) / 256), 256, A);
+            LAUNCH(k_time1, p->B, 256, A);
+        }
+    }
     const int* uflag = d.cond_ch > 0 ? nullptr : flags_dev + FLAG_UNIFORM_T;
     float* tembs = ws_ptr<float>(workspace, p->ws.tembs);
     rc = rowgemm(st, A.hid1, d.T, A.temb, d.T, W + A.wg[JW_TIME_W3], W + A.wg[JW_TIME_B3], p->B, d.T, d.T / 32, 0, 0, uflag,
@@ -457,6 +499,9 @@
         case 3: src = ws + p->ws.hhat; n = (int64_t)p->Nn * p->amax_parts * p->dims.D; break;
         case 5: src = ws + p->ws.mods; n = p->dims.Mtot; break;
         case 6: src = ws + p->ws.q; n = (int64_t)p->Nn * p->dims.QKP; break;
+        case 7: src = ws + p->ws.mfold; n = (int64_t)p->dims.L * (p->dims.D / 32) * (p->dims.De / 4) * 256; break;
+        case 8: src = ws + p->ws.ffold; n = (int64_t)p->dims.L * (p->dims.D / 32) * (p->dims.D / 8) * 256; break;
+        case 9: src = ws + p->ws.ahid; n = (int64_t)p->Nn * p->dims.KNH; break;
         default: return jodo_set_error(JODO_ERR_ARG, "debug_fetch: unknown selector %d", what);
     }
     hipError_t e = hipMemcpyAsync(dst, src, (size_t)n * sizeof(float), hipMemcpyDeviceToDevice, (hipStream_t)stream);
diff --git a/jodo_amd/csrc/dgt_kernels_common.h b/jodo_amd/csrc/dgt_kernels_common.h
--- a/jodo_amd/csrc/dgt_kernels_common.h
+++ b/jodo_amd/csrc/dgt_kernels_common.h
@@ -23,6 +23,7 @@
     int64_t wbn[6];
     int64_t mod_base_next;
     int pre_mode;
+    int pos_items;
     float *hid1, *temb, *mods, *condh, *condh2;
     float *pos_in, *pos_out, *dpos, *cpos, *feat, *h, *hhat, *astat, *q, *k, *v, *n2e, *wrow, *wcol, *ua, *ub, *rmean, *mfold, *ffold, *ahid, *apred;
     int* eflag;
@@ -41,6 +42,7 @@
 };
 
 struct FoldOffs { int64_t c0[16], ine[16]; };
+struct FoldPair { FoldOffs m, f; int n_m, n_f, npos; };
 
 namespace jd {
 
@@ -113,6 +115,17 @@
     return p;
 }
 
+__device__ __forceinline__ void pos_final_body(const KArgs& A, int v) {
+    if (v >= A.pd.Nn_pad) return;
+    float4 p = reinterpret_cast<const float4*>(A.pos_in)[v];
+    if (v < A.pd.Nn) {
+        if (A.layer > 0)
+            p = advance_position(A, p, v, v >> 5, A.pd.node_n[v], A.pd.node_i[v], A.pd.node_eoff[v]);
+        if (isnan(p.x) || isnan(p.y) || isnan(p.z)) atomicOr(&A.flags[FLAG_NAN], 1);
+    }
+    reinterpret_cast<float4*>(A.pos_out)[v] = p;
+}
+
 __device__ __forceinline__ float gelu_erf(float x) { return 0.5f * x * (1.f + erff(x * 0.70710678118654752f)); }
 
 }
diff --git a/jodo_amd/csrc/dgt_kernels_node.h b/jodo_amd/csrc/dgt_kernels_node.h
--- a/jodo_amd/csrc/dgt_kernels_node.h
+++ b/jodo_amd/csrc/dgt_kernels_node.h
@@ -1,9 +1,10 @@
 #pragma once
 #include "dgt_kernels_attn.h"
+#include "dgt_kernels_wide.h"
 
 namespace jd {
 
-template <bool NEXT = false>
+template <bool NEXT = false, int EKQ = 0>
 __device__ __forceinline__ void node_pre_body(const KArgs& A, int blk) {
     const int lane = threadIdx.x & 63, j = lane & 31, half = lane >> 5;
     const int strip = blk / 3, piece = blk % 3;
@@ -15,7 +16,8 @@
     }
     const float* mr = mod_row(A, L.b) + (NEXT ? A.mod_base_next : A.mod_base);
     float hx[128];
-    load_nat<8>(A.h + (size_t)L.v * 256, half, hx);
+    if constexpr (EKQ > 0) wide::embed_nodes_body<256, EKQ, true>(A, strip, piece == 0, hx);
+    else load_nat<8>(A.h + (size_t)L.v * 256, half, hx);
     layer_norm<128>(hx);
     modulate<8>(hx, mr, mr + 256, half);
     const WSrc ws = make_wsrc(A.W, lane);
diff --git a/jodo_amd/csrc/dgt_kernels_post.h b/jodo_amd/csrc/dgt_kernels_post.h
--- a/jodo_amd/csrc/dgt_kernels_post.h
+++ b/jodo_amd/csrc/dgt_kernels_post.h
@@ -3,20 +3,10 @@
 
 namespace jd {
 
-__global__ void k_pos_final(KArgs A) {
-    const int v = blockIdx.x * blockDim.x + threadIdx.x;
-    if (v >= A.pd.Nn_pad) return;
-    float4 p = reinterpret_cast<const float4*>(A.pos_in)[v];
-    if (v < A.pd.Nn) {
-        if (A.layer > 0)
-            p = advance_position(A, p, v, v >> 5, A.pd.node_n[v], A.pd.node_i[v], A.pd.node_eoff[v]);
-        if (isnan(p.x) || isnan(p.y) || isnan(p.z)) atomicOr(&A.flags[FLAG_NAN], 1);
-    }
-    reinterpret_cast<float4*>(A.pos_out)[v] = p;
-}
+__global__ void k_pos_final(KArgs A) { pos_final_body(A, (int)(blockIdx.x * blockDim.x + threadIdx.x)); }
 
-__global__ void k_finalize_nodes(KArgs A) {
-    const int idx = blockIdx.x * blockDim.x + threadIdx.x;
+__device__ __forceinline__ void finalize_nodes_body(const KArgs& A, int blk) {
+    const int idx = blk * blockDim.x + threadIdx.x;
     if (idx >= A.pd.B * A.pd.N) return;
     if (idx == 0 && A.flags[FLAG_NAN] != 0) A.flags[FLAG_NAN_COUNT] += 1;
     if (idx == 0) {
@@ -47,9 +37,10 @@
     const float* ap = A.apred + (size_t)(v0 + i) * 32;
     for (int f = 0; f < nd; ++f) o[3 + f] = ap[f];
 }
+__global__ void k_finalize_nodes(KArgs A) { finalize_nodes_body(A, (int)blockIdx.x); }
 
-__global__ void k_finalize_edges(KArgs A) {
-    const size_t idx = (size_t)blockIdx.x * blockDim.x + threadIdx.x;
+__device__ __forceinline__ void finalize_edges_body(const KArgs& A, unsigned blk) {
+    const size_t idx = (size_t)blk * blockDim.x + threadIdx.x;
     const size_t NN = (size_t)A.pd.N * A.pd.N;
     if (idx >= (size_t)A.pd.B * NN) return;
     const int b = (int)(idx / NN);
@@ -66,5 +57,12 @@
     const float pp[4] = {p.x, p.y, p.z, p.w}, qq[4] = {q.x, q.y, q.z, q.w};
     for (int f = 0; f < ch; ++f) o[f] = 0.5f * (pp[f] + qq[f]);
 }
+__global__ void k_finalize_edges(KArgs A) { finalize_edges_body(A, blockIdx.x); }
+
+__global__ void k_finalize(KArgs A) {
+    const unsigned nn = (unsigned)(A.pd.B * A.pd.N + 255) / 256;
+    if (blockIdx.x < nn) finalize_nodes_body(A, (int)blockIdx.x);
+    else finalize_edges_body(A, blockIdx.x - nn);
+}
 
 }
diff --git a/jodo_amd/csrc/dgt_kernels_pre.h b/jodo_amd/csrc/dgt_kernels_pre.h
--- a/jodo_amd/csrc/dgt_kernels_pre.h
+++ b/jodo_amd/csrc/dgt_kernels_pre.h
@@ -21,8 +21,8 @@
     }
 }
 
-__global__ void k_check_sym(KArgs A) {
-    const size_t idx = (size_t)blockIdx.x * blockDim.x + threadIdx.x;
+__device__ __forceinline__ void check_sym_body(const KArgs& A, unsigned blk) {
+    const size_t idx = (size_t)blk * blockDim.x + threadIdx.x;
     const size_t NN = (size_t)A.pd.N * A.pd.N;
     if (idx >= (size_t)A.pd.B * NN) return;
     const int b = (int)(idx / NN);
@@ -41,9 +41,9 @@
     }
     if (diff) atomicOr(&A.flags[FLAG_ASYM], 1);
 }
+__global__ void k_check_sym(KArgs A) { check_sym_body(A, blockIdx.x); }
 
-__global__ void k_time1(KArgs A) {
-    const int b = blockIdx.x;
+__device__ __forceinline__ void time1_body(const KArgs& A, int b) {
     if (A.flags[FLAG_UNIFORM_T] && b > 0) return;
     __shared__ float ft[17];
     const float x = A.noise[b];
@@ -63,6 +63,7 @@
         A.hid1[(size_t)b * A.d.T + f] = gelu_erf(acc);
     }
 }
+__global__ void k_time1(KArgs A) { time1_body(A, (int)blockIdx.x); }
 
 __global__ void k_cond1(KArgs A) {
     const int row = blockIdx.x;
@@ -147,8 +148,8 @@
     }
 }
 
-__global__ void k_pack_nodes(KArgs A) {
-    const int v = blockIdx.x * blockDim.x + threadIdx.x;
+__device__ __forceinline__ void pack_nodes_body(const KArgs& A, int blk) {
+    const int v = blk * blockDim.x + threadIdx.x;
     if (v >= A.pd.Nn_pad) return;
     const int nd = A.d.nd, ndp = A.d.ndp, dims = 3 + nd;
     float4 p = make_float4(0.f, 0.f, 0.f, 0.f), cp = p;
@@ -170,5 +171,13 @@
     reinterpret_cast<float4*>(A.pos_in)[v] = p;
     reinterpret_cast<float4*>(A.cpos)[v] = cp;
 }
+__global__ void k_pack_nodes(KArgs A) { pack_nodes_body(A, (int)blockIdx.x); }
+
+__global__ void k_frame_inputs(KArgs A) {
+    const unsigned b = blockIdx.x, nt = (unsigned)A.pd.B, np = (unsigned)(A.pd.Nn_pad + 255) / 256;
+    if (b < nt) time1_body(A, (int)b);
+    else if (b < nt + np) pack_nodes_body(A, (int)(b - nt));
+    else check_sym_body(A, b - nt - np);
+}
 
 }
diff --git a/jodo_amd/csrc/dgt_kernels_wide.h b/jodo_amd/csrc/dgt_kernels_wide.h
--- a/jodo_amd/csrc/dgt_kernels_wide.h
+++ b/jodo_amd/csrc/dgt_kernels_wide.h
@@ -19,11 +19,11 @@
     static constexpr int M_WG = M_GBF + 32, M_BS = M_WG + D_;
 };
 
-template <int D, int KQ>
-__global__ __launch_bounds__(64) void k_embed_nodes(KArgs A) {
+template <int D, int KQ, bool KEEP>
+__device__ __forceinline__ void embed_nodes_body(const KArgs& A, int strip, bool write, float (&hx)[KEEP ? D / 2 : 1]) {
     using X = Dim<D>;
     const int lane = threadIdx.x & 63, j = lane & 31, half = lane >> 5;
-    const int v = blockIdx.x * 32 + j;
+    const int v = strip * 32 + j;
     float x[KQ * 4];
     const float4* src = reinterpret_cast<const float4*>(A.feat + (size_t)v * (KQ * 8) + half * (KQ * 4));
 #pragma unroll
@@ -38,9 +38,20 @@
         f32x16 acc = mfma_block<KQ>(w + (size_t)b * KQ * 64, x, zero16());
         float r[16];
         acc_bias(acc, bias + b * 32 + half * 16, r);
-        store16(A.h + (size_t)v * D + b * 32 + half * 16, r);
-        store16(A.ahid + (size_t)v * A.d.KNH + b * 32 + half * 16, r);
-    }
+        if (write) {
+            store16(A.h + (size_t)v * D + b * 32 + half * 16, r);
+            store16(A.ahid + (size_t)v * A.d.KNH + b * 32 + half * 16, r);
+        }
+        if constexpr (KEEP) {
+#pragma unroll
+            for (int s = 0; s < 16; ++s) hx[b * 16 + s] = r[s];
+        }
+    }
+}
+template <int D, int KQ>
+__global__ __launch_bounds__(64) void k_embed_nodes(KArgs A) {
+    float none[1];
+    embed_nodes_body<D, KQ, false>(A, (int)blockIdx.x, true, none);
 }
 
 template <int D>
@@ -359,11 +370,11 @@
 __global__ __launch_bounds__(64) void k_node_gram(KArgs A) { node_gram_body<D>(A, A.g0 + (int)blockIdx.x); }
 
 template <int D, int KQI>
-__global__ __launch_bounds__(64) void k_fold_coord(KArgs A, FoldOffs F, float* out, int need_rot, unsigned short* out_s = nullptr) {
+__device__ __forceinline__ void fold_coord_body(const KArgs& A, const FoldOffs& F, float* out, int need_rot, unsigned short* out_s, int blk) {
     if (!A.flags[FLAG_UNIFORM_T] || (need_rot && !rot_active(A))) return;
     using X = Dim<D>;
     constexpr int PER_L = X::ND * KQI;
-    const int l = blockIdx.x / PER_L, r = blockIdx.x % PER_L, nb = r / KQI, q = r % KQI;
+    const int l = blk / PER_L, r = blk % PER_L, nb = r / KQI, q = r % KQI;
     const int lane = threadIdx.x & 63, i = lane & 31, kh = lane >> 5;
     const float* sc = A.mods + 32 + (size_t)l * A.d.MB + X::M_EQUI + D;
     const float4* c0 = reinterpret_cast<const float4*>(A.W + F.c0[l]) + (size_t)nb * X::KQD * 64;
@@ -405,6 +416,17 @@
             *reinterpret_cast<uint2*>(dst) = make_uint2((unsigned)t[term][0] | ((unsigned)t[term][1] << 16), (unsigned)t[term][2] | ((unsigned)t[term][3] << 16));
         }
     }
+}
+template <int D, int KQI>
+__global__ __launch_bounds__(64) void k_fold_coord(KArgs A, FoldOffs F, float* out, int need_rot, unsigned short* out_s = nullptr) {
+    fold_coord_body<D, KQI>(A, F, out, need_rot, out_s, (int)blockIdx.x);
+}
+template <int D>
+__global__ __launch_bounds__(64) void k_fold_coord2(KArgs A, FoldPair F) {
+    const int b = (int)blockIdx.x;
+    if (b < F.n_f) fold_coord_body<D, D / 8>(A, F.f, A.ffold, 1, A.ffold_s, b);
+    else if (b < F.n_f + F.n_m) fold_coord_body<D, D / 16>(A, F.m, A.mfold, 0, A.mfold_s, b - F.n_f);
+    else pos_final_body(A, (b - F.n_f - F.n_m) * 64 + (int)threadIdx.x);
 }
 
 template <int D, int R>
@@ -1047,7 +1069,10 @@
     }
 }
 template <int D>
-__global__ __launch_bounds__(64, 1) void k_node_head(KArgs A) { node_head_body<D>(A, (int)blockIdx.x); }
+__global__ __launch_bounds__(64, 1) void k_node_head(KArgs A) {
+    if ((int)blockIdx.x < A.pd.n_strips) node_head_body<D>(A, (int)blockIdx.x);
+    else pos_final_body(A, ((int)blockIdx.x - A.pd.n_strips) * 64 + (int)threadIdx.x);
+}
 
 template <int D, int NBK, bool SYM>
 __device__ __forceinline__ void edge_head_body(const KArgs& A, int blk) {
@@ -1109,8 +1134,9 @@
 __global__ __launch_bounds__(64, 1) void k_heads_sym(KArgs A) {
     const int ns = A.pd.n_strips;
     if ((int)blockIdx.x < ns) node_head_body<D>(A, (int)blockIdx.x);
-    else edge_head_body<D, NBK, true>(A, (int)blockIdx.x - ns);
-}
-
-}
-}
+    else if ((int)blockIdx.x < ns + A.pos_items) pos_final_body(A, ((int)blockIdx.x - ns) * 64 + (int)threadIdx.x);
+    else edge_head_body<D, NBK, true>(A, (int)blockIdx.x - ns - A.pos_items);
+}
+
+}
+}
diff --git a/jodo_amd/csrc/dgt_plan.cpp b/jodo_amd/csrc/dgt_plan.cpp
--- a/jodo_amd/csrc/dgt_plan.cpp
+++ b/jodo_amd/csrc/dgt_plan.cpp
@@ -99,6 +99,7 @@
     p->B = B; p->N = N; p->max_blocks = -1; p->last_pos_buf = 0; p->last_e_buf = 0;
     p->opt[JODO_OPT_FUSE_NEXT_QKV] = 1; p->opt[JODO_OPT_DIR_SPLIT] = 1; p->opt[JODO_OPT_NODE_POST_WAVES] = 0; p->opt[JODO_OPT_ATTN_VARIANT] = 0; p->opt[JODO_OPT_HEADS_MIX] = 1; p->opt[JODO_OPT_HALF_ROWS] = 1; p->opt[JODO_OPT_PRE_EMBED] = 1; p->opt[JODO_OPT_AB_PRE] = 1; p->opt[JODO_OPT_Z_SPLIT] = 1;
     p->opt[JODO_OPT_PIN_SYMMETRIC] = 0; p->opt[JODO_OPT_PIN_UNIFORM_T] = 0; p->opt[JODO_OPT_ROT_STATS] = 1; p->opt[JODO_OPT_NODE_MIX] = 1;
+    p->opt[JODO_OPT_FRAME_MIX] = 7;
     p->opt[JODO_OPT_SPLIT_BF16] = 0; p->split_w = nullptr; p->split_bytes = 0;
     p->prof_enabled = 0; p->force_directed = 0; p->dbg_timing = nullptr;
 
@@ -409,7 +410,9 @@
     const double rowgroups = (uniform_t && d.cond_ch == 0) ? 1.0 : (double)((p->B + 31) / 32);
     cls[JODO_PROF_PROLOGUE] += rowgroups * (proj(d.T, d.T) + proj((int)d.Mtot, d.T));
     if (d.cond_ch > 0) cls[JODO_PROF_PROLOGUE] += (double)((p->B * d.cond_ch + 31) / 32) * proj(D, D) + (double)((p->B + 31) / 32) * proj(d.T, d.cond_ch * D);
-    cls[JODO_PROF_PROLOGUE] += strips * proj(D, d.ndp);
+    const bool pre_embed = p->n_items > 0 && p->opt[JODO_OPT_PRE_EMBED] != 0 && L > 0;
+    if (tuned && pre_embed && (p->opt[JODO_OPT_FRAME_MIX] & 3) == 3) cls[JODO_PROF_NODE_PRE] += 3 * strips * proj(D, d.ndp);
+    else cls[JODO_PROF_PROLOGUE] += strips * proj(D, d.ndp);
     double dir_iters = 0, pair_iters = 0;
     for (int i = 0; i < p->n_items; ++i) dir_iters += dsc[p->off_item_t1 + i] - dsc[p->off_item_t0 + i];
     for (int i = 0; i < p->n_pitems; ++i) pair_iters += dsc[p->off_pitem_t1 + i] - dsc[p->off_pitem_t0 + i];
@@ -491,9 +494,21 @@
         return jodo_set_error(JODO_ERR_ARG, "plan_set_option: the symmetric pin contradicts jodo_debug_set_force_directed");
     if ((option == JODO_OPT_PIN_SYMMETRIC || option == JODO_OPT_PIN_UNIFORM_T) && (value < 0 || value > 2))
         return jodo_set_error(JODO_ERR_ARG, "plan_set_option: a pin is 0 (none), 1 or 2, got %d", value);
+    if (option == JODO_OPT_FRAME_MIX && (value < 0 || value > 7))
+        return jodo_set_error(JODO_ERR_ARG, "plan_set_option: the frame mix is 0 (off) or 1 (merged launches) + 2 (node embedding in the q / k / v items) + 4 (interleaved edge embedding), got %d", value);
     if (option == JODO_OPT_ATTN_VARIANT && (value < 0 || value > 3))
         return jodo_set_error(JODO_ERR_ARG, "plan_set_option: attention variant must be 0..3, got %d", value);
     p->opt[option] = value;
+    return JODO_OK;
+}
+extern "C" int jodo_debug_frame_mix_map(int n_strips, int n_items, int32_t* out) {
+    if (n_strips < 1 || n_items < 0 || !out) return jodo_set_error(JODO_ERR_ARG, "frame_mix_map: n_strips %d, n_items %d", n_strips, n_items);
+    const int n_pre = 3 * n_strips;
+    for (int b = 0; b < n_pre + n_items; ++b) {
+        int emb = 0;
+        const int idx = jodo_frame_mix_map(b, n_pre, n_items, &emb);
+        out[b] = emb ? n_pre + idx : idx;
+    }
     return JODO_OK;
 }
 extern "C" int jodo_debug_attn_schedule(const jodo_plan* p, int64_t* o) {
diff --git a/jodo_amd/csrc/dgt_plan.h b/jodo_amd/csrc/dgt_plan.h
--- a/jodo_amd/csrc/dgt_plan.h
+++ b/jodo_amd/csrc/dgt_plan.h
@@ -100,4 +100,16 @@
     int gt_cache_full, gt_cache_count;
 };
 
+#if defined(__HIP__) || defined(__HIPCC__)
+#define JODO_HD __host__ __device__
+#else
+#define JODO_HD
+#endif
+JODO_HD inline int jodo_frame_mix_map(int b, int n_pre, int n_e, int* is_embed) {
+    const long long T = (long long)n_pre + n_e;
+    const int e0 = (int)((long long)b * n_e / T), e1 = (int)(((long long)b + 1) * n_e / T);
+    *is_embed = e1 > e0;
+    return e1 > e0 ? e0 : b - e0;
+}
+
 int dgt_dims_from_cfg(const jodo_cfg* cfg, DgtDims* d);
```

Result: no change. 174.7 (median of 6 runs) (+0.4%).
